# chenruduan/OAReactDiff

Measured on AMD Instinct MI355X. Metric: denoising_steps_per_sec, higher is better.
Workload: dtype f32; 1 GPU; EGNNDynamics.forward (LEFTNet H=196 R=96 L=6), B=64 reactions/GPU x 3 objects x 23 atoms, complete graph per reaction (N=4416, E=300288), T=1000 sampler step shape; batch_per_gpu=64, atoms_per_object=23, parallelism=replica x1 (no collective), launch=eager

## Files before the change

### oareactdiff_amd/_capi.py

```python
from __future__ import annotations

import ctypes as C
import os

from .build import LIB

OARD_MAX_OBJECTS = 8
ABI_VERSION = 2040
OARD_OK, OARD_EINVAL, OARD_ENOTCOMPLETE, OARD_EHIP, OARD_ENOMEM = 0, -1, -2, -3, -4
ERRORS = {OARD_EINVAL: "invalid argument / unsupported configuration", OARD_ENOTCOMPLETE: "topology is not complete-per-sample",
          OARD_EHIP: "HIP runtime error", OARD_ENOMEM: "workspace too small"}

PREC_GCL_BF16X3, PREC_EQUI_BF16X3, PREC_TRAIN_BF16X3 = 1, 2, 4
TAP_S, TAP_VEC, TAP_EDGE, TAP_POS_FRAME, TAP_DPOS, TAP_HOUT, TAP_LABELS, TAP_NE1 = 1, 2, 3, 4, 5, 6, 7, 8

EXPORTS = ["oard_version", "oard_supported", "oard_param_count", "oard_packed_bytes", "oard_pack_weights",
           "oard_topology_create", "oard_topology_destroy", "oard_topology_num_nodes", "oard_topology_num_edges",
           "oard_topology_num_inner_edges", "oard_topology_num_samples", "oard_topology_check_edge_index",
           "oard_workspace_bytes", "oard_forward", "oard_active_inner_edges", "oard_debug_lin3u_table", "oard_sampler_step", "oard_sampler_step_dev", "oard_tap", "oard_debug_stop_after", "oard_debug_option", "oard_timing_enable", "oard_timing_reset",
           "oard_timing_get",
           "oard_topology_create_parts", "oard_topology_export", "oard_tape_bytes", "oard_tape_entry", "oard_forward_train",
           "oard_packed_bwd_bytes", "oard_pack_weights_bwd", "oard_gcl_backward_dx", "oard_edge_node_sums",
           "oard_equi_backward_dx", "oard_scalarize_backward", "oard_equi_msg_backward", "oard_lin3u_forward", "oard_lin3u_backward", "oard_wgrad_scratch_bytes", "oard_wgrad",
           "oard_train_scratch_bytes", "oard_train_scratch_poison", "oard_train_scratch_entry", "oard_train_tail_backward",
           "oard_train_layer_backward", "oard_train_init_backward", "oard_train_stage_backward",
           "oard_loss_prepare", "oard_loss_terms", "oard_adamw_step", "oard_adamw_step_dev", "oard_nan_replace",
           "oard_graph_create", "oard_graph_destroy", "oard_graph_num_nodes", "oard_graph_num_edges", "oard_graph_object_rows",
           "oard_graph_is_complete", "oard_graph_workspace_bytes", "oard_graph_forward", "oard_library_stream"]
STAGE_RECOMPUTE, STAGE_UPDATE, STAGE_MESSAGE, STAGE_GCL_NODE, STAGE_NODE_PRE, STAGE_GCL_EDGE, STAGE_EQUI_EDGE = range(7)
SCRATCH_XH, SCRATCH_XQ, SCRATCH_CR, SCRATCH_DCD, SCRATCH_DCR = range(1, 6)

TOPO_NODE_REF, TOPO_NODE_OBJ, TOPO_NODE_ROW, TOPO_NODE_SAMPLE, TOPO_NODE_TIDX, TOPO_SAMPLE_PTR, TOPO_GROUP_PTR, \
    TOPO_INNER_SRC, TOPO_INNER_TGT, TOPO_ROW_SRC, TOPO_ROW_TGT = range(1, 12)
TAPE_HIN, TAPE_GEO, TAPE_RBF, TAPE_PP0, TAPE_X1 = 1, 2, 3, 4, 5
TAPE_S_IN, TAPE_VEC_IN, TAPE_EW, TAPE_AGG, TAPE_S_MID, TAPE_Z1, TAPE_Z2, TAPE_ATT, TAPE_Z3, TAPE_ZD1, TAPE_CD, TAPE_S_A, TAPE_VEC_A = range(16, 29)


class OardConfig(C.Structure):
    _fields_ = [
        ("hidden", C.c_int32), ("num_radial", C.c_int32), ("num_layers", C.c_int32), ("in_hidden", C.c_int32),
        ("n_obj", C.c_int32), ("node_nf", C.c_int32 * OARD_MAX_OBJECTS), ("enc_alias", C.c_int32 * OARD_MAX_OBJECTS),
        ("condition_nf", C.c_int32), ("condition_time", C.c_int32), ("pos_dim", C.c_int32), ("cutoff", C.c_float),
        ("reflect_equiv", C.c_int32), ("precision", C.c_int32),
    ]


class OardError(RuntimeError):
    pass


def check(rc: int, what: str) -> None:
    if rc != OARD_OK:
        raise OardError(f"{what} failed: {ERRORS.get(rc, rc)}")


def ptr_array(tensors, n=None):
    if tensors is None:
        return None
    ptrs = [None if t is None else t.data_ptr() for t in tensors]
    return (C.c_void_p * (len(ptrs) if n is None else n))(*ptrs)


_lib = None


def lib() -> C.CDLL:
    global _lib
    if _lib is not None:
        return _lib
    if not os.path.exists(LIB):
        raise OardError(f"{LIB} not found: build it with `python -m oareactdiff_amd.build` "
                        "(there is no CPU fallback for the HIP backend)")
    L = C.CDLL(LIB)
    vp, i32, i64, sz = C.c_void_p, C.c_int32, C.c_int64, C.c_size_t
    cfgp = C.POINTER(OardConfig)
    L.oard_version.restype = C.c_int
    got = L.oard_version()
    if got != ABI_VERSION:
        raise OardError(f"{LIB} has ABI version {got}, this package expects {ABI_VERSION}: rebuild it "
                        "(`python -m oareactdiff_amd.build --force`, or the script that made the OARD_LIB build)")
    L.oard_supported.argtypes = [cfgp]; L.oard_supported.restype = C.c_int
    L.oard_param_count.argtypes = [cfgp]; L.oard_param_count.restype = sz
    L.oard_packed_bytes.argtypes = [cfgp]; L.oard_packed_bytes.restype = sz
    L.oard_pack_weights.argtypes = [cfgp, C.POINTER(vp), sz, vp, sz, vp]; L.oard_pack_weights.restype = C.c_int
    L.oard_topology_create.argtypes = [cfgp, C.POINTER(i64), C.POINTER(i64), i64, C.POINTER(vp)]
    L.oard_topology_create.restype = C.c_int
    L.oard_topology_destroy.argtypes = [vp]; L.oard_topology_destroy.restype = None
    for f in ("oard_topology_num_nodes", "oard_topology_num_edges", "oard_topology_num_inner_edges",
              "oard_topology_num_samples"):
        getattr(L, f).argtypes = [vp]; getattr(L, f).restype = i64
    L.oard_topology_check_edge_index.argtypes = [vp, vp, i64, vp, vp]; L.oard_topology_check_edge_index.restype = C.c_int
    L.oard_workspace_bytes.argtypes = [cfgp, vp]; L.oard_workspace_bytes.restype = sz
    L.oard_forward.argtypes = [cfgp, vp, vp, C.POINTER(vp), vp, C.c_int, vp, C.POINTER(vp), vp, sz, vp, vp]
    L.oard_forward.restype = C.c_int
    L.oard_debug_lin3u_table.argtypes = [cfgp, vp, C.c_int, vp, vp]; L.oard_debug_lin3u_table.restype = C.c_int
    L.oard_active_inner_edges.argtypes = [cfgp, vp, vp, sz, C.POINTER(i64), vp]; L.oard_active_inner_edges.restype = C.c_int
    L.oard_sampler_step.argtypes = [cfgp, vp, C.c_int, C.POINTER(vp), C.POINTER(vp), C.POINTER(vp), C.POINTER(vp),
                                    C.c_float, C.c_float, C.c_float, C.c_int, C.POINTER(vp), vp]
    L.oard_sampler_step.restype = C.c_int
    L.oard_sampler_step_dev.argtypes = [cfgp, vp, C.c_int, C.POINTER(vp), C.POINTER(vp), C.POINTER(vp), C.POINTER(vp), vp, C.c_int,
                                        C.POINTER(vp), vp]
    L.oard_sampler_step_dev.restype = C.c_int
    L.oard_tap.argtypes = [cfgp, vp, vp, C.c_int, C.c_int, vp, vp]; L.oard_tap.restype = C.c_int
    ci = C.c_int
    L.oard_topology_create_parts.argtypes = [cfgp, C.POINTER(i64), C.POINTER(i64), i64, ci, C.POINTER(vp)]
    L.oard_topology_create_parts.restype = ci
    L.oard_topology_export.argtypes = [vp, ci, vp, i64, vp]; L.oard_topology_export.restype = ci
    L.oard_tape_bytes.argtypes = [cfgp, vp]; L.oard_tape_bytes.restype = sz
    L.oard_tape_entry.argtypes = [cfgp, vp, ci, ci, C.POINTER(sz), C.POINTER(i64), C.POINTER(i64)]; L.oard_tape_entry.restype = ci
    L.oard_forward_train.argtypes = [cfgp, vp, vp, C.POINTER(vp), vp, ci, vp, C.POINTER(vp), vp, sz, vp, sz, vp, vp]
    L.oard_forward_train.restype = ci
    L.oard_packed_bwd_bytes.argtypes = [cfgp]; L.oard_packed_bwd_bytes.restype = sz
    L.oard_pack_weights_bwd.argtypes = [cfgp, C.POINTER(vp), sz, vp, sz, vp]; L.oard_pack_weights_bwd.restype = ci
    L.oard_gcl_backward_dx.argtypes = [cfgp, vp, vp, ci, vp, vp, vp, vp, vp, vp, vp, vp, vp]; L.oard_gcl_backward_dx.restype = ci
    L.oard_edge_node_sums.argtypes = [cfgp, vp, vp, vp, vp, vp]; L.oard_edge_node_sums.restype = ci
    L.oard_equi_backward_dx.argtypes = [cfgp, vp, vp, ci, vp, vp, vp, vp, vp]; L.oard_equi_backward_dx.restype = ci
    L.oard_scalarize_backward.argtypes = [cfgp, vp, vp, vp, vp, ci, vp, vp, vp, vp]; L.oard_scalarize_backward.restype = ci
    L.oard_equi_msg_backward.argtypes = [cfgp, vp, vp, ci, vp, vp, vp, vp, vp, vp, vp, vp, vp]; L.oard_equi_msg_backward.restype = ci
    L.oard_lin3u_forward.argtypes = [cfgp, vp, ci, vp, i64, vp, vp]; L.oard_lin3u_forward.restype = ci
    L.oard_lin3u_backward.argtypes = [cfgp, vp, ci, vp, vp, i64, vp, vp, vp, vp, vp, vp, vp]; L.oard_lin3u_backward.restype = ci
    L.oard_wgrad_scratch_bytes.argtypes = [ci, ci, i64]; L.oard_wgrad_scratch_bytes.restype = sz
    L.oard_wgrad.argtypes = [vp, ci, ci, ci, ci, ci, vp, ci, ci, ci, ci, ci, ci, i64, vp, vp, vp, sz, vp]; L.oard_wgrad.restype = ci
    pvp = C.POINTER(vp)
    L.oard_train_scratch_bytes.argtypes = [cfgp, vp]; L.oard_train_scratch_bytes.restype = sz
    L.oard_train_scratch_poison.argtypes = [cfgp, vp, vp, sz, vp]; L.oard_train_scratch_poison.restype = ci
    L.oard_train_scratch_entry.argtypes = [cfgp, vp, ci, C.POINTER(sz), C.POINTER(i64), C.POINTER(i64)]; L.oard_train_scratch_entry.restype = ci
    L.oard_train_tail_backward.argtypes = [cfgp, vp, vp, vp, vp, pvp, vp, vp, pvp, pvp, vp, sz, vp]; L.oard_train_tail_backward.restype = ci
    L.oard_train_layer_backward.argtypes = [cfgp, vp, vp, vp, vp, ci, vp, vp, vp, pvp, pvp, vp, sz, vp]; L.oard_train_layer_backward.restype = ci
    L.oard_train_init_backward.argtypes = [cfgp, vp, vp, vp, vp, pvp, vp, vp, pvp, pvp, vp, sz, vp]; L.oard_train_init_backward.restype = ci
    L.oard_train_stage_backward.argtypes = [cfgp, vp, vp, vp, vp, ci, ci, vp, vp, vp, vp, vp, vp, pvp, pvp, vp, sz, vp]
    L.oard_train_stage_backward.restype = ci
    L.oard_nan_replace.argtypes = [cfgp, vp, vp, pvp, pvp, vp]; L.oard_nan_replace.restype = ci
    pf, cf = C.POINTER(C.c_float), C.c_float
    L.oard_loss_prepare.argtypes = [cfgp, vp, pvp, pvp, pvp, pvp, vp, vp, ci, pf, pf, ci, ci, pvp, pvp, vp]; L.oard_loss_prepare.restype = ci
    L.oard_loss_terms.argtypes = [cfgp, vp, pvp, pvp, pvp, pvp, pvp, vp, vp, ci, pf, pf, pf, ci, ci, vp, vp, pvp, vp]; L.oard_loss_terms.restype = ci
    cd = C.c_double
    L.oard_adamw_step.argtypes = [vp, vp, vp, vp, vp, i64, cd, cd, cd, cd, cd, i64, ci, cd, vp]; L.oard_adamw_step.restype = ci
    L.oard_adamw_step_dev.argtypes = [vp, vp, vp, vp, vp, i64, cd, cd, cd, cd, cd, ci, ci, vp, ci, vp, vp, vp, vp]; L.oard_adamw_step_dev.restype = ci
    L.oard_library_stream.argtypes = [ci, pvp]; L.oard_library_stream.restype = ci
    L.oard_graph_create.argtypes = [cfgp, vp, vp, i64, vp, i64, pvp]; L.oard_graph_create.restype = ci
    L.oard_graph_destroy.argtypes = [vp]; L.oard_graph_destroy.restype = None
    L.oard_graph_num_nodes.argtypes = [vp]; L.oard_graph_num_nodes.restype = i64
    L.oard_graph_num_edges.argtypes = [vp]; L.oard_graph_num_edges.restype = i64
    L.oard_graph_object_rows.argtypes = [vp, ci]; L.oard_graph_object_rows.restype = i64
    L.oard_graph_is_complete.argtypes = [vp]; L.oard_graph_is_complete.restype = ci
    L.oard_graph_workspace_bytes.argtypes = [cfgp, vp]; L.oard_graph_workspace_bytes.restype = sz
    L.oard_graph_forward.argtypes = [cfgp, vp, pvp, sz, pvp, vp, ci, vp, pvp, vp, sz, vp, vp]; L.oard_graph_forward.restype = ci
    L.oard_debug_stop_after.argtypes = [C.c_int]; L.oard_debug_stop_after.restype = C.c_int
    L.oard_debug_option.argtypes = [C.c_char_p, C.c_int]; L.oard_debug_option.restype = C.c_int
    L.oard_timing_enable.argtypes = [C.c_int]; L.oard_timing_enable.restype = C.c_int
    L.oard_timing_reset.argtypes = []; L.oard_timing_reset.restype = C.c_int
    L.oard_timing_get.argtypes = [C.c_char_p, C.POINTER(C.c_double), C.POINTER(i64)]; L.oard_timing_get.restype = C.c_int
    for env, opt in (("OARD_GCL_VARIANT", b"gcl_variant"), ("OARD_EQUI_VARIANT", b"equi_variant"),
                     ("OARD_NODE_VARIANT", b"node_variant"), ("OARD_GCL_SKIP", b"gcl_skip"), ("OARD_EQUI_SKIP", b"equi_skip"), ("OARD_EQUI_L0_SKIP", b"equi_l0_skip"), ("OARD_GCL_MSUM", b"gcl_msum"), ("OARD_GCL_PERSIST", b"gcl_persist"), ("OARD_GCL_GRID", b"gcl_grid"), ("OARD_PARTS", b"parts"), ("OARD_SEQUENTIAL", b"sequential"), ("OARD_POISON", b"poison"), ("OARD_AUTO_SMALL", b"auto_small"), ("OARD_AUTO_TINY", b"auto_tiny"), ("OARD_NPB", b"npb"),
                     ("OARD_WGRAD_WGS", b"wgrad_wgs"), ("OARD_WGRAD_LDS", b"wgrad_lds"), ("OARD_WGRAD_T16", b"wgrad_t16"), ("OARD_WGRAD_QUEUE", b"wgrad_queue"), ("OARD_GATE_FOLD", b"gate_fold"), ("OARD_WGRAD_SHAPES", b"wgrad_shapes"), ("OARD_TRAIN_DUAL", b"train_dual"), ("OARD_SMALL_SPLIT", b"small_split"),
                     ("OARD_SKIP_FAMILIES", b"skip_families")):
        if os.environ.get(env) not in (None, ""):
            check(L.oard_debug_option(opt, int(os.environ[env])), f"oard_debug_option({opt.decode()})")
    _lib = L
    return L


def timing_get(family: str):
    ms, n = C.c_double(0.0), C.c_int64(0)
    check(lib().oard_timing_get(family.encode(), C.byref(ms), C.byref(n)), "oard_timing_get")
    return ms.value, n.value
```

### oareactdiff_amd/csrc/oard_edge_v1.h

```cpp
#pragma once
#include "oard_kernels.h"

typedef __attribute__((address_space(3))) void* lds_ptr_t;
typedef const __attribute__((address_space(1))) void* gbl_ptr_t;
typedef int i4 __attribute__((ext_vector_type(4)));

OARD_DEV void glds16(const float* gsrc_lane, float* lds_chunk);
OARD_DEV void glds16u(const float* chunk_uniform, unsigned lane_byte_off, float* lds_chunk) {
    glds16(reinterpret_cast<const float*>(reinterpret_cast<const char*>(chunk_uniform) + lane_byte_off), lds_chunk);
}
OARD_DEV void glds16(const float* gsrc_lane, float* lds_chunk) {
#ifndef OARD_ABL_NODMA_INSTR
    __builtin_amdgcn_global_load_lds((gbl_ptr_t)gsrc_lane, (lds_ptr_t)lds_chunk, 16, 0, 0);
#else
    asm volatile("" :: "v"(gsrc_lane), "s"(lds_chunk));
#endif
}

OARD_DEV void phase_barrier() {
    asm volatile("s_waitcnt vmcnt(0)" ::: "memory");
#ifndef OARD_ABL_NOBARRIER
    __syncthreads();
#endif
}

#ifdef OARD_PHASE_PROBE
OARD_DEVVAR __device__ unsigned long long g_phase_probe[8];
#define PROBE_DECL long long pr_t0_ = clock64(), pr_wait_ = 0, pr_bar_ = 0, pr_n_ = 0;
#define PHASE_BARRIER() do { const long long a_ = clock64(); asm volatile("s_waitcnt vmcnt(0)" ::: "memory"); const long long b_ = clock64(); \
        __syncthreads(); const long long c_ = clock64(); pr_wait_ += b_ - a_; pr_bar_ += c_ - b_; ++pr_n_; } while (0)
#define PROBE_END(pf) do { if ((threadIdx.x & 63) == 0) { atomicAdd(&g_phase_probe[0], 1ull); atomicAdd(&g_phase_probe[1], (unsigned long long)(clock64() - pr_t0_)); \
        atomicAdd(&g_phase_probe[2], (unsigned long long)pr_wait_); atomicAdd(&g_phase_probe[3], (unsigned long long)pr_bar_); \
        atomicAdd(&g_phase_probe[4], (unsigned long long)(pf).dma_cyc); atomicAdd(&g_phase_probe[5], (unsigned long long)(pf).dma_n); \
        atomicAdd(&g_phase_probe[6], (unsigned long long)pr_n_); if ((threadIdx.x >> 6) < (blockDim.x >> 7)) atomicAdd(&g_phase_probe[7], (unsigned long long)pr_bar_); } } while (0)
#else
#define PROBE_DECL
#define PHASE_BARRIER() phase_barrier()
#define PROBE_END(pf) do {} while (0)
#endif

#ifdef OARD_TIMELINE
#define TL_MAX 1024
OARD_DEVVAR __device__ long long g_timeline[16][TL_MAX];
#define TL_DECL const bool tl_on_ = DO_S1 && DO_S3 && blockIdx.x == gridDim.x / 2 && (threadIdx.x & 63) == 0; int tl_n_ = 0;
#define TL(code) do { if (tl_on_ && tl_n_ < TL_MAX) g_timeline[threadIdx.x >> 6][tl_n_++] = (clock64() << 3) | (code); } while (0)
#define TL_END() do { if (tl_on_ && tl_n_ < TL_MAX) g_timeline[threadIdx.x >> 6][tl_n_] = 0; } while (0)
#else
#define TL_DECL
#define TL(code) do {} while (0)
#define TL_END() do {} while (0)
#endif

OARD_DEV void mma_pair(f4 a0, f4 b0, f4& c0, f4 a1, f4 b1, f4& c1) {
    c0 = __builtin_amdgcn_mfma_f32_16x16x4f32(a0.x, b0.x, c0, 0, 0, 0);
    c1 = __builtin_amdgcn_mfma_f32_16x16x4f32(a1.x, b1.x, c1, 0, 0, 0);
    c0 = __builtin_amdgcn_mfma_f32_16x16x4f32(a0.y, b0.y, c0, 0, 0, 0);
    c1 = __builtin_amdgcn_mfma_f32_16x16x4f32(a1.y, b1.y, c1, 0, 0, 0);
    c0 = __builtin_amdgcn_mfma_f32_16x16x4f32(a0.z, b0.z, c0, 0, 0, 0);
    c1 = __builtin_amdgcn_mfma_f32_16x16x4f32(a1.z, b1.z, c1, 0, 0, 0);
    c0 = __builtin_amdgcn_mfma_f32_16x16x4f32(a0.w, b0.w, c0, 0, 0, 0);
    c1 = __builtin_amdgcn_mfma_f32_16x16x4f32(a1.w, b1.w, c1, 0, 0, 0);
}

OARD_DEV void mma4_chunk(f4 a, f4 b, f4& c0, f4& c1) {
    c0 = __builtin_amdgcn_mfma_f32_4x4x1f32(a.x, b.x, c0, 0, 0, 0);
    c1 = __builtin_amdgcn_mfma_f32_4x4x1f32(a.y, b.y, c1, 0, 0, 0);
    c0 = __builtin_amdgcn_mfma_f32_4x4x1f32(a.z, b.z, c0, 0, 0, 0);
    c1 = __builtin_amdgcn_mfma_f32_4x4x1f32(a.w, b.w, c1, 0, 0, 0);
}
OARD_DEV f4 reduce_g(f4 v) {
    f4 r;
#pragma unroll
    for (int c = 0; c < 4; ++c) {
        float x = v[c];
        x += __shfl_xor(x, 16, 64);
        x += __shfl_xor(x, 32, 64);
        r[c] = x;
    }
    return r;
}

OARD_DEV f4 lds_a(const float* sl, int j) { return *reinterpret_cast<const f4*>(sl + j * 256); }

struct NoHook { OARD_DEV void operator()() const {} };
template <int KB, bool TAIL, class Hook>
OARD_DEV f4 chain_tile(const float* sl, int j0, const f4 (&in)[KB], f4 init, float tail, Hook hook) {
    static_assert(!TAIL || (KB & 1), "compact tail needs an odd number of chunks");
    f4 c0 = init, c1 = f4zero();
    f4 a0 = lds_a(sl, j0), a1 = KB > 1 ? lds_a(sl, j0 + 1) : f4zero();
#pragma unroll
    for (int b = 0; b + 1 < KB; b += 2) {
        f4 n0 = a0, n1 = a1;
        if (b + 2 < KB) n0 = lds_a(sl, j0 + b + 2);
        if (b + 3 < KB) n1 = lds_a(sl, j0 + b + 3);
        mma_pair(a0, in[b], c0, a1, in[b + 1], c1);
        hook();
        a0 = n0; a1 = n1;
    }
    if (KB & 1) {
        if (TAIL) c0 = __builtin_amdgcn_mfma_f32_16x16x4f32(a0.x, tail, c0, 0, 0, 0);
        else c0 = mma_chunk(a0, in[KB - 1], c0);
    }
    return c0 + c1;
}
template <int KB, class Hook = NoHook>
OARD_DEV f4 chain_tile(const float* sl, int j0, const f4 (&in)[KB], f4 init, Hook hook = Hook()) {
    return chain_tile<KB, false, Hook>(sl, j0, in, init, 0.f, hook);
}
template <int KB, class Hook = NoHook>
OARD_DEV f4 chain_tile4(const float* sl, int j0, const f4 (&in)[KB], f4 init, Hook hook = Hook()) {
    f4 c0 = init, c1 = f4zero();
    f4 a0 = lds_a(sl, j0), a1 = KB > 1 ? lds_a(sl, j0 + 1) : f4zero();
#pragma unroll
    for (int b = 0; b + 1 < KB; b += 2) {
        f4 n0 = a0, n1 = a1;
        if (b + 2 < KB) n0 = lds_a(sl, j0 + b + 2);
        if (b + 3 < KB) n1 = lds_a(sl, j0 + b + 3);
        mma4_chunk(a0, in[b], c0, c1);
        mma4_chunk(a1, in[b + 1], c0, c1);
        hook();
        a0 = n0; a1 = n1;
        __builtin_amdgcn_sched_barrier(0);
    }
    if (KB & 1) mma4_chunk(a0, in[KB - 1], c0, c1);
    return c0 + c1;
}
template <int MT, bool ROWS4, class Hook>
OARD_DEV void chain_kouter(const float* sl, int j0, f4 x, f4 (&acc)[MT], f4& extra, Hook hook) {
    static_assert(!ROWS4 || (MT & 1), "the 4-row tile must be the odd one");
    f4 a0 = lds_a(sl, j0), a1 = MT > 1 ? lds_a(sl, j0 + 1) : f4zero();
#pragma unroll
    for (int t = 0; t + 1 < MT; t += 2) {
        f4 n0 = a0, n1 = a1;
        if (t + 2 < MT) n0 = lds_a(sl, j0 + t + 2);
        if (t + 3 < MT) n1 = lds_a(sl, j0 + t + 3);
        mma_pair(a0, x, acc[t], a1, x, acc[t + 1]);
        hook();
        a0 = n0; a1 = n1;
    }
    if (MT & 1) {
        if (ROWS4) mma4_chunk(a0, x, acc[MT - 1], extra);
        else acc[MT - 1] = mma_chunk(a0, x, acc[MT - 1]);
    }
}
template <int MT, class Hook = NoHook>
OARD_DEV void chain_kouter(const float* sl, int j0, f4 x, f4 (&acc)[MT], Hook hook = Hook()) {
    f4 unused = f4zero();
    chain_kouter<MT, false, Hook>(sl, j0, x, acc, unused, hook);
}

#ifndef OARD_PF_HALF
#define OARD_PF_HALF 1
#endif
#ifndef OARD_PF_PERIOD
#define OARD_PF_PERIOD 1
#endif
template <int WAVES, int SLAB, int HALF = OARD_PF_HALF, int PERIOD = OARD_PF_PERIOD, int RING = 2>
struct SlabPrefetch {
    static constexpr int IW = (HALF && WAVES >= 8) ? WAVES / 2 : WAVES;
    static constexpr int KMAX = (SLAB + IW - 1) / IW;
    const float* src;
    float* dst;
    unsigned lane_off;
    int n, k, next, wave;
#ifdef OARD_PHASE_PROBE
    long long dma_cyc = 0, dma_n = 0;
#endif
    OARD_DEV void begin(const float* stream, float* smem, int phase, int first_chunk, int n_chunks) {
        src = stream + (size_t)first_chunk * 256;
        dst = smem + (size_t)(RING == 2 ? (phase & 1) : (phase % RING)) * SLAB * 256;
        n = wave < IW ? n_chunks : 0; k = 0; next = 1 + ((IW == WAVES && wave >= WAVES / 2) ? 1 : 0);
    }
    OARD_DEV void one() {
#ifdef OARD_ABL_NOHOOK
        k = KMAX;
        return;
#endif
        const int j = wave + k * IW;
#ifdef OARD_PHASE_PROBE
        if (j < n) { const long long a_ = clock64(); glds16u(src + (size_t)j * 256, lane_off, dst + j * 256); dma_cyc += clock64() - a_; ++dma_n; }
#else
        if (j < n) glds16u(src + (size_t)j * 256, lane_off, dst + j * 256);
#endif
        ++k;
    }
#ifdef OARD_ABL_BURST
    OARD_DEV void tick() {}
#else
#ifdef OARD_ABL_NOHOOK
    OARD_DEV void tick() {}
#else
    OARD_DEV void tick() { if (--next == 0) { one(); next = PERIOD; } }
#endif
#endif
    OARD_DEV void flush() { while (k < KMAX) one(); }
};

#ifdef OARD_ABL_NOEDGELOAD
OARD_DEV f4 ld_edge(const float* p) { return (f4){0.25f, -0.5f, 0.125f, 1.0f}; }
#else
OARD_DEV f4 ld_edge(const float* p) { return ld_f4(p); }
#endif

template <int CTRL>
OARD_DEV float dpp_row(float x) {
    return __builtin_bit_cast(float, __builtin_amdgcn_update_dpp(0, __builtin_bit_cast(int, x), CTRL, 0xf, 0xf, true));
}
template <int CTRL>
OARD_DEV int dpp_row_i(int x) { return __builtin_amdgcn_update_dpp(0, x, CTRL, 0xf, 0xf, true); }
struct SegLanes {
    float k1, k2, k4, k8;
    bool head;
};
OARD_DEV SegLanes seg_lanes(int key) {
    SegLanes s;
    s.k1 = dpp_row_i<0x101>(key) == key ? 1.f : 0.f; s.k2 = dpp_row_i<0x102>(key) == key ? 1.f : 0.f;
    s.k4 = dpp_row_i<0x104>(key) == key ? 1.f : 0.f; s.k8 = dpp_row_i<0x108>(key) == key ? 1.f : 0.f;
    const int prev = dpp_row_i<0x111>(key);
    s.head = key > 0 && prev != key;
    return s;
}
OARD_DEV f4 seg_sum(f4 v, const SegLanes& s) {
#define OARD_SEG_STEP(k, d) \
        "v_fmac_f32_dpp %0, %0, " k " row_shl:" d " row_mask:0xf bank_mask:0xf bound_ctrl:1\n\t" \
        "v_fmac_f32_dpp %1, %1, " k " row_shl:" d " row_mask:0xf bank_mask:0xf bound_ctrl:1\n\t" \
        "v_fmac_f32_dpp %2, %2, " k " row_shl:" d " row_mask:0xf bank_mask:0xf bound_ctrl:1\n\t" \
        "v_fmac_f32_dpp %3, %3, " k " row_shl:" d " row_mask:0xf bank_mask:0xf bound_ctrl:1\n\t"
    asm volatile("s_nop 4\n\t" OARD_SEG_STEP("%4", "1") OARD_SEG_STEP("%5", "2") OARD_SEG_STEP("%6", "4") OARD_SEG_STEP("%7", "8")
                 : "+v"(v.x), "+v"(v.y), "+v"(v.z), "+v"(v.w) : "v"(s.k1), "v"(s.k2), "v"(s.k4), "v"(s.k8));
#undef OARD_SEG_STEP
    return v;
}
template <class D>
OARD_DEV void st_msum(float* __restrict__ msum, long long col, int key, const f4 (&m)[D::HT], int lane) {
    const SegLanes s = seg_lanes(key);
#pragma unroll
    for (int t = 0; t < D::HT; ++t) {
        const f4 v = seg_sum(m[t], s);
        if (s.head) st_blk(msum, (size_t)col, D::HP, t, lane, v);
    }
}

template <class D, int GP>
struct GclStream {
    static constexpr int HT = D::HT, WB = D::WB, G1 = HT, G2 = HT + 1, NG2 = HT + 1;
    static constexpr bool TAIL1 = (D::H % 16) >= 1 && (D::H % 16) <= 4 && HT >= 3 && (HT & 1);
    static constexpr bool ROWS4 = TAIL1;
    static constexpr int SLAB = GP * G2;
    static constexpr int NP1 = (WB + GP - 1) / GP, NP2 = (NG2 + GP - 1) / GP, NP3 = NP1, NPH = NP1 + NP2 + NP3;
    static constexpr int C1 = WB * G1, C2 = NG2 * G2, C3 = WB * G2, CHUNKS = C1 + C2 + C3;
    static constexpr size_t LDS_BYTES = (size_t)2 * SLAB * 1024;
};

struct GclTape {
    float* z1;
    float* z2;
    float* att;
    float* z3;
};

OARD_DEV float tail_compact(f4 v, int lane) {
    const int e = lane & 15, g = lane >> 4;
    const float t0 = __shfl(v.x, e, 64), t1 = __shfl(v.y, e, 64), t2 = __shfl(v.z, e, 64), t3 = __shfl(v.w, e, 64);
// ... 201 lines not shown
            pf_begin(p + DIST);
            if (p3 + 1 < S::NP3) {
#pragma unroll
                for (int gg = 0; gg < GP; ++gg) {
                    const int t = (p3 + 1) * GP + gg;
                    if (t < WB)
                        onext[gg] = DO_S1 ? ld_edge(erow + 16 * t) : ld_f4(c0 + 16 * t + 4 * g);
                }
            }
        };
        auto hook = [&]() { if (RING == 3 && bar_left > 0 && --bar_left == 0) { PHASE_BARRIER(); post(); } pf.tick(); };
        if (RING == 2) { PHASE_BARRIER(); post(); } else bar_left = BAR_AT;
#pragma unroll
        for (int gg = 0; gg < GP; ++gg) {
            const int t = p3 * GP + gg;
            if (t < WB) {
                TL(2);
                const f4 z = chain_tile<HT, TAIL1>(SL(p), gg * G2 + 1, m, A(p, gg * G2), m_tail, hook);
                TL(3);
                if (TRAIN) pendz[gg] = z;
                pend[gg] = o[gg] + silu4(z);
            }
        }
        TL(4);
        if (RING == 3 && bar_left > 0) { bar_left = 0; PHASE_BARRIER(); post(); }
        if (MSUM && p3 == 0) st_msum<D>(mbuf, c, key, m, lane);
        pf.flush();
        ++p;
    };
    {
        int p3 = 0;
        for (; p3 + 1 < S::NP3; p3 += 2) { s3_phase(p3, on, om); s3_phase(p3 + 1, om, on); }
        if (p3 < S::NP3) s3_phase(p3, on, om);
    }
#pragma unroll
    for (int gg = 0; gg < GP; ++gg) {
        const int t = (S::NP3 - 1) * GP + gg;
        if (t < WB) {
            st_f4(orow + 16 * t, pend[gg]);
            if (TRAIN) st_f4(tape.z3 + e * D::WP + 4 * g + 16 * t, pendz[gg]);
        }
    }
    PROBE_END(pf);
    TL_END();
}

template <class D>
struct EquiStream {
    static constexpr int WB = D::WB, D1T = D::D1T, RB = D::RB, HT = D::HT;
    static constexpr int G1 = D1T, G2 = 1 + D1T + RB, NG2 = 3 * HT;
    static constexpr bool ROWS4 = (D::H % 16) >= 1 && (D::H % 16) <= 4;
    static constexpr int SLAB = G2 > G1 ? G2 : G1;
    static constexpr int NPH = WB + NG2;
    static constexpr int C1 = WB * G1, CHUNKS = C1 + NG2 * G2;
    static constexpr size_t LDS_BYTES = (size_t)2 * SLAB * 1024;
};

template <class D, int WAVES, bool TRAIN>
__global__ __launch_bounds__(WAVES * 64) void k_equi_edge_v1(TopoDev tp, const float* __restrict__ stream,
                                                             const float* __restrict__ dp0b,
                                                             const float* __restrict__ ew, const float* __restrict__ rbuf,
                                                             float* __restrict__ qbuf, float* __restrict__ zd1,
                                                             float* __restrict__ cdbuf, ActList al, int skip_mid) {
    extern __shared__ __attribute__((aligned(16))) float smem[];
    using S = EquiStream<D>;
    constexpr int WB = D::WB, D1T = D::D1T, RB = D::RB, HT = D::HT, G1 = S::G1, G2 = S::G2;
    const int lane = threadIdx.x & 63, g = lane >> 4;
    const int wave = __builtin_amdgcn_readfirstlane(threadIdx.x >> 6);

    SlabPrefetch<WAVES, S::SLAB, 0, 3> pf;
    pf.wave = wave;
    pf.lane_off = (unsigned)lane * 16u;
    const bool skip = !TRAIN && skip_mid != 0;
    auto pf_begin = [&](int ph) {
        pf.begin(stream, smem, ph, ph * G1, G1);
    };
    auto pf_begin_t2 = [&](int ph, int slot) {
        pf.begin(stream, smem, ph, S::C1 + slot * G2, slot < S::NG2 ? G2 : 0);
    };
    auto next_slot = [&](int i) -> int { return i + ((skip && i % 3 == 0) ? 2 : 1); };
    auto hook = [&]() { pf.tick(); };
    auto A = [&](int p, int j) -> f4 {
        return *reinterpret_cast<const f4*>(smem + ((size_t)(p & 1) * S::SLAB + j) * 256 + lane * 4);
    };
    auto SL = [&](int p) -> const float* { return smem + (size_t)(p & 1) * S::SLAB * 256 + lane * 4; };

    const long long n_cols = al.n != nullptr ? (long long)*al.n : tp.A;
    if ((long long)blockIdx.x * WAVES * 16 >= n_cols) return;
    const long long c = ((long long)blockIdx.x * WAVES + wave) * 16 + (lane & 15);
    const bool live = c < n_cols;
    const size_t a = (size_t)(live ? (al.rows != nullptr ? (long long)al.rows[c] : c) : tp.A);
    const float* erow = ew + (live ? a : (size_t)tp.E) * D::WP + 4 * g;
    f4 d1[D1T];
#pragma unroll
    for (int t = 0; t < D1T; ++t) d1[t] = ld_vec(dp0b, t, lane);
    f4 rb[RB];
#pragma unroll
    for (int b = 0; b < RB; ++b) rb[b] = ld_blk(rbuf, a, D::RP, b, lane);
    f4 xn = ld_f4(erow);
    pf_begin(0);
    pf.flush();

    int p = 0;
    for (int b = 0; b < WB; ++b, ++p) {
        phase_barrier();
        const f4 x = xn;
        if (b + 1 < WB) pf_begin(p + 1); else pf_begin_t2(p + 1, 0);
        if (b + 1 < WB) xn = ld_f4(erow + 16 * (b + 1));
        chain_kouter<D1T>(SL(p), 0, x, d1, hook);
        pf.flush();
    }
    if (TRAIN) {
#pragma unroll
        for (int t = 0; t < D1T; ++t) st_blk(zd1, a, D::D1P, t, lane, d1[t]);
    }
#pragma unroll
    for (int t = 0; t < D1T; ++t) d1[t] = silu4(d1[t]);

    float* qrow = qbuf + a * (size_t)(3 * D::HP) + 4 * g;
    float* cdrow = TRAIN ? cdbuf + a * (size_t)(3 * D::HP) + 4 * g : nullptr;
    f4 pend = f4zero(), pendc = f4zero();
    int pend_off = 0;
    auto t2_phase = [&](int i, auto rows4) {
        phase_barrier();
        if (i > 0) {
            st_f4(qrow + pend_off, pend);
            if (TRAIN) st_f4(cdrow + pend_off, pendc);
        }
        pf_begin_t2(p + 1, next_slot(i));
        const int tt = i / 3, th = i - 3 * tt;
        f4 cd, cr;
        if (decltype(rows4)::value) {
            cd = reduce_g(chain_tile4<D1T>(SL(p), 1, d1, A(p, 0), hook));
            cr = reduce_g(chain_tile4<RB>(SL(p), 1 + D1T, rb, f4zero(), hook));
            if (g != 0) { cd = f4zero(); cr = f4zero(); }
        } else {
            cd = chain_tile<D1T>(SL(p), 1, d1, A(p, 0), hook);
            cr = chain_tile<RB>(SL(p), 1 + D1T, rb, f4zero(), hook);
        }
        pf.flush();
        pend = cd * cr;
        if (TRAIN) pendc = cd;
        pend_off = th * D::HP + 16 * tt;
        ++p;
    };
    constexpr int N_FULL = S::ROWS4 ? S::NG2 - 3 : S::NG2;
    for (int i = 0; i < N_FULL; i = next_slot(i)) t2_phase(i, std::false_type{});
    for (int i = N_FULL; i < S::NG2; i = next_slot(i)) t2_phase(i, std::true_type{});
    st_f4(qrow + pend_off, pend);
    if (TRAIN) st_f4(cdrow + pend_off, pendc);
}

template <class D>
__global__ __launch_bounds__(256) void k_equi_agg_v1(TopoDev tp, const float* __restrict__ wb, LayerOff lo,
                                                     const float* __restrict__ qbuf, const float* __restrict__ xq,
                                                     const float* __restrict__ geo, const float* __restrict__ x1,
                                                     float* __restrict__ s, const float* __restrict__ vec_in,
                                                     float* __restrict__ vec_out, float* __restrict__ v2buf,
                                                     float* __restrict__ scal, float* __restrict__ vdot) {
    bool live; const ColId id = col_id(tp.N, live);
    if (!live) return;
    const int n = id.col, a0 = tp.act_ptr[n], cnt = tp.act_ptr[n + 1] - a0;
    const int mx = wave_max(cnt);
    const float inv_sqrt2 = 0.70710678118654752f, inv_sqrt3 = 0.57735026918962576f,
                inv_sqrt_h = 1.0f / sqrtf((float)D::H);
    f4 vx[3][D::HT], dx[D::HT];
#pragma unroll
    for (int t = 0; t < D::HT; ++t) { dx[t] = f4zero(); vx[0][t] = f4zero(); vx[1][t] = f4zero(); vx[2][t] = f4zero(); }
    for (int k = 0; k < mx; ++k)
        if (k < cnt) {
            const size_t a = (size_t)a0 + k;
            const int m = tp.act_src[a];
            const float* g = geo + a * GEO_STRIDE;
            const float ux = g[2], uy = g[3], uz = g[4];
            const float xc = lo.xcross ? 1.0f : 0.0f, cx = xc * g[5], cy = xc * g[6], cz = xc * g[7];
#pragma unroll
            for (int t = 0; t < D::HT; ++t) {
                const f4 q0 = ld_blk(qbuf, a, 3 * D::HP, t, id.lane);
                const f4 q1 = ld_blk(qbuf, a, 3 * D::HP, D::HT + t, id.lane);
                const f4 q2 = ld_blk(qbuf, a, 3 * D::HP, 2 * D::HT + t, id.lane);
                const f4 xs0 = ld_blk(xq, m, 3 * D::HP, t, id.lane) + ld_blk(xq, n, 3 * D::HP, t, id.lane);
                const f4 xs1 = ld_blk(xq, m, 3 * D::HP, D::HT + t, id.lane) + ld_blk(xq, n, 3 * D::HP, D::HT + t, id.lane);
                const f4 xs2 = ld_blk(xq, m, 3 * D::HP, 2 * D::HT + t, id.lane) + ld_blk(xq, n, 3 * D::HP, 2 * D::HT + t, id.lane);
                const f4 xm = xs0 * q0;
                dx[t] += xm;
                const f4 a2 = xs1 * q1 * inv_sqrt3, a3 = xs2 * q2;
                vx[0][t] += (ld_blk(vec_in, (size_t)m * 3 + 0, D::HP, t, id.lane) * a2 + a3 * ux + xm * cx) * inv_sqrt_h;
                vx[1][t] += (ld_blk(vec_in, (size_t)m * 3 + 1, D::HP, t, id.lane) * a2 + a3 * uy + xm * cy) * inv_sqrt_h;
                vx[2][t] += (ld_blk(vec_in, (size_t)m * 3 + 2, D::HP, t, id.lane) * a2 + a3 * uz + xm * cz) * inv_sqrt_h;
            }
        }
#pragma unroll
    for (int t = 0; t < D::HT; ++t) {
        const f4 sn = (ld_blk(s, n, D::HP, t, id.lane) + dx[t]) * inv_sqrt2;
        if (id.valid) st_blk(s, n, D::HP, t, id.lane, sn);
#pragma unroll
        for (int x = 0; x < 3; ++x) {
            vx[x][t] += ld_blk(vec_in, (size_t)n * 3 + x, D::HP, t, id.lane);
            if (id.valid) st_blk(vec_out, (size_t)n * 3 + x, D::HP, t, id.lane, vx[x][t]);
        }
    }
    const float fx = x1[n * 3], fy = x1[n * 3 + 1], fz = x1[n * 3 + 2];
    const float* l3 = wb + lo.l3u;
    for (int t = 0; t < D::HT; ++t) {
        f4 v1[3] = {f4zero(), f4zero(), f4zero()}, v2[3] = {f4zero(), f4zero(), f4zero()};
        const float* w1 = wb + lo.vp + ((size_t)t * D::HT * 64 + id.lane) * 4;
        const float* w2 = wb + lo.vp + ((size_t)(D::HT + t) * D::HT * 64 + id.lane) * 4;
#pragma unroll
        for (int b = 0; b < D::HT; ++b) {
            const f4 c1 = ld_f4(w1 + (size_t)b * 256), c2 = ld_f4(w2 + (size_t)b * 256);
#pragma unroll
            for (int x = 0; x < 3; ++x) {
                v1[x] = mma_chunk(c1, vx[x][b], v1[x]);
                v2[x] = mma_chunk(c2, vx[x][b], v2[x]);
            }
        }
        const f4 sc = v1[0] * fx + v1[1] * fy + v1[2] * fz;
        const f4 vd = (v1[0] * v2[0] + v1[1] * v2[1] + v1[2] * v2[2]) * inv_sqrt_h;
        f4 sca;
        const int f0 = 16 * t + 4 * id.g;
        sca.x = f0 + 0 < D::H ? lin3u(l3, sc.x) : 0.f;
        sca.y = f0 + 1 < D::H ? lin3u(l3, sc.y) : 0.f;
        sca.z = f0 + 2 < D::H ? lin3u(l3, sc.z) : 0.f;
        sca.w = f0 + 3 < D::H ? lin3u(l3, sc.w) : 0.f;
        if (id.valid) {
            st_blk(scal, n, D::HP, t, id.lane, sca);
            st_blk(vdot, n, D::HP, t, id.lane, vd);
            st_blk(v2buf, (size_t)n * 3 + 0, D::HP, t, id.lane, v2[0]);
            st_blk(v2buf, (size_t)n * 3 + 1, D::HP, t, id.lane, v2[1]);
            st_blk(v2buf, (size_t)n * 3 + 2, D::HP, t, id.lane, v2[2]);
        }
    }
}
```

### oareactdiff_amd/csrc/oard_hip.hip

```cpp
#include <algorithm>
#include <cmath>
#include <cstdio>
#include <cstring>
#include <map>
#include <string>
#include <vector>
#include <mutex>
#include <chrono>
#include <utility>

#include "oard_kernels.h"
#include "oard_edge_v1.h"
#include "oard_edge_p.h"
#include "oard_wgrad_t16.h"
#include "oard_edge_b3.h"
#ifdef OARD_EXPERIMENTS
#include "oard_edge_fp.h"
#endif
#include "oard_node_v1.h"
#include "oard_edge_small.h"
#include "oard_edge_bwd.h"
#include "oard_node_bwd.h"
#include "oard_rows.h"
#include "oard_inst.h"

#define OARD_VERSION 2040
#ifdef OARD_EXPERIMENTS
static constexpr bool kV0 = true;
#else
static constexpr bool kV0 = false;
#endif

#define HIP_TRY(x) do { hipError_t e_ = (x); if (e_ != hipSuccess) { \
    fprintf(stderr, "liboard_hip: %s failed: %s (%s:%d)\n", #x, hipGetErrorString(e_), __FILE__, __LINE__); \
    return OARD_EHIP; } } while (0)

namespace {
enum Family { F_GCL_EDGE = 0, F_EQUI_EDGE, F_NODE, F_INIT, F_OTHER, F_GCL_BWD, F_EQUI_BWD, F_WGRAD, F_COUNT };
const char* kFamilyNames[F_COUNT] = {"gcl_edge", "equi_edge", "node", "init", "other", "gcl_edge_bwd", "equi_edge_bwd", "wgrad"};
struct TimingRec { hipEvent_t a, b; int fam; };
struct Timing {
    bool on = false;
    std::vector<TimingRec> recs;
    std::vector<hipEvent_t> pool;
    double total_ms[F_COUNT] = {0};
    long long launches[F_COUNT] = {0};
    hipEvent_t get() {
        if (!pool.empty()) { hipEvent_t e = pool.back(); pool.pop_back(); return e; }
        hipEvent_t e; (void)hipEventCreate(&e); return e;
    }
    void flush() {
        for (auto& r : recs) {
            (void)hipEventSynchronize(r.b);
            float ms = 0.f;
            (void)hipEventElapsedTime(&ms, r.a, r.b);
            total_ms[r.fam] += ms; launches[r.fam] += 1;
            pool.push_back(r.a); pool.push_back(r.b);
        }
        recs.clear();
    }
} g_timing;
int g_stop_after = 0;
int g_gcl_variant = 2;
int g_equi_variant = 2;
int g_sequential = 0;
int g_auto_tiny = 8;
int g_auto_small = 4;
int g_npb = 0;
int g_poison = 0;
int g_equi_l0_skip = 1;
int g_gcl_msum = 1;
int g_gcl_msum_taken = 0;
int g_equi_l0_taken = 0;
int g_parts = 0;
int g_small_split = 128;
int g_wgrad_shapes = 3;
int g_wgrad_t16 = 256;
int g_wgrad_lds = 256;
int g_wgrad_wgs = 512;
int g_gcl_persist = 1;
int g_gcl_grid = 0;
int g_equi_skip = 1;
int g_gcl_skip = 1;
int g_node_variant = 1;
int g_skip_families = 0;

struct ScopedLaunch {
    hipStream_t st; hipEvent_t a; int fam; bool on;
    ScopedLaunch(int f, hipStream_t s) : st(s), fam(f), on(g_timing.on) {
        if (on) { a = g_timing.get(); (void)hipEventRecord(a, st); }
    }
    ~ScopedLaunch() {
        if (on) { hipEvent_t b = g_timing.get(); (void)hipEventRecord(b, st); g_timing.recs.push_back({a, b, fam}); }
    }
};
#define LAUNCH(fam, kern, grid, block, stream, ...) do { ScopedLaunch sl_(fam, stream); if (!((g_skip_families >> (fam)) & 1)) \
    hipLaunchKernelGGL(kern, dim3((unsigned)(grid)), dim3(block), 0, stream, __VA_ARGS__); } while (0)
#define LAUNCH2(fam, kern, gx, gy, block, stream, ...) do { ScopedLaunch sl_(fam, stream); if (!((g_skip_families >> (fam)) & 1)) \
    hipLaunchKernelGGL(kern, dim3((unsigned)(gx), (unsigned)(gy)), dim3(block), 0, stream, __VA_ARGS__); } while (0)

#ifndef OARD_DIMS_LIST
#define OARD_DIMS_LIST X(196, 96) X(32, 8) X(32, 32)
#endif

inline size_t align_up(size_t x, size_t a) { return (x + a - 1) / a * a; }
inline long long cdiv(long long a, long long b) { return (a + b - 1) / b; }

bool config_ok(const oard_config* c) {
    if (!c) return false;
    bool dims = false;
#define X(h, r) dims = dims || (c->hidden == (h) && c->num_radial == (r));
    OARD_DIMS_LIST
#undef X
    if (!dims) return false;
    if (c->num_layers < 1 || c->num_layers > OARD_MAX_LAYERS) return false;
    if (c->in_hidden < 1 || c->in_hidden > 16) return false;
    if (c->n_obj < 1 || c->n_obj > OARD_MAX_OBJECTS) return false;
    if (c->pos_dim != 3 || (c->reflect_equiv != 0 && c->reflect_equiv != 1)) return false;
    if (c->precision & ~(OARD_PREC_GCL_BF16X3 | OARD_PREC_EQUI_BF16X3 | OARD_PREC_TRAIN_BF16X3)) return false;
    const int emb = c->in_hidden - (c->condition_time ? 1 : 0) - (c->condition_nf > 0 ? c->condition_nf : 0);
    if (emb < 1) return false;
    for (int k = 0; k < c->n_obj; ++k) {
        const int d = c->node_nf[k] - 3;
        if (d < 1 || d > 16) return false;
        const int a = c->enc_alias[k];
        if (a < 0 || a >= c->n_obj || c->node_nf[a] != c->node_nf[k]) return false;
    }
    return true;
}
int embed_dim(const oard_config* c) {
    return c->in_hidden - (c->condition_time ? 1 : 0) - (c->condition_nf > 0 ? c->condition_nf : 0);
}

PackOff make_layout(const oard_config* c) {
    const RDims d(c->hidden, c->num_radial);
    PackOff po;
    memset(&po, 0, sizeof(po));
    size_t cur = 0;
    auto take = [&](size_t n) { size_t o = cur; cur = align_up(cur + n, 64); return o; };
    auto mat = [&](int MT, int KB) { return take((size_t)MT * KB * 256); };
    const int emb = embed_dim(c);
    po.emb = mat(d.HT, 1); po.emb_b = take(d.HP);
    po.nbemb = mat(d.HT, 1); po.nbemb_b = take(d.HP);
    po.s2v = mat(d.HT, d.HT); po.s2v_b = take(d.HP);
    po.rl0 = mat(d.HT, d.RB); po.rl0_b = take(d.HP);
    po.rl2 = mat(d.HT, d.HT); po.rl2_b = take(d.HP);
    po.lin3 = take((size_t)d.H4 * 5 + 1);
    po.pe0 = take((size_t)d.H2 * 3);
    po.pe1 = mat(d.HT, d.PB);
    po.embout = mat(1, d.HT); po.embout_b = take(16);
    po.v1p = mat(d.HT, d.HT); po.v2p = take(d.HP);
    po.un0 = mat(d.HT, 2 * d.HT); po.un0_b = take(d.HP);
    po.un2 = mat(1, d.HT); po.un2_b = take(16);
    po.c0row = take(d.WP);
    po.u0 = take(d.HP);
    po.rbf_means = take(d.RP); po.rbf_betas = take(d.RP);
    for (int k = 0; k < c->n_obj; ++k) {
        const int dd = c->node_nf[k] - 3;
        po.enc[k] = take((size_t)2 * dd * dd + 2 * dd + (size_t)emb * 2 * dd + emb);
        po.dec[k] = take((size_t)2 * dd * emb + 2 * dd + (size_t)dd * 2 * dd + dd);
    }
    for (int l = 0; l < c->num_layers; ++l) {
        LayerOff& lo = po.layer[l];
        lo.ln_g_w = take(d.HP); lo.ln_g_b = take(d.HP);
        lo.W1a = mat(d.HT, d.HT); lo.b1 = take(d.HP);
        lo.W1b = mat(d.HT, d.HT);
        lo.W1c = mat(d.HT, d.WB);
        lo.W2 = mat(d.HT, d.HT); lo.b2 = take(d.HP);
        lo.watt = take(d.HP); lo.batt = take(1);
        lo.W3 = mat(d.WB, d.HT); lo.b3 = take(d.WP);
        lo.nm0 = mat(d.HT, 2 * d.HT); lo.nm0b = take(d.HP);
        lo.nm1 = mat(d.HT, d.HT); lo.nm1b = take(d.HP);
        lo.ln_q_w = take(d.HP); lo.ln_q_b = take(d.HP);
        lo.xp0 = mat(d.HT, d.HT);
        lo.xp2 = mat(3 * d.HT, d.HT);
        lo.dp0 = mat(d.D1T, d.WB); lo.dp0b = take(d.D1P);
        lo.dp2 = mat(3 * d.HT, d.D1T); lo.dp2b = take(3 * d.HP);
        lo.rbfp = mat(3 * d.HT, d.RB);
        lo.vp = mat(2 * d.HT, d.HT);
        lo.xv0 = mat(d.HT, 2 * d.HT);
        lo.xv2 = mat(3 * d.HT, d.HT);
        lo.l3u = take(593);
        lo.l3t = take(L3T_FLOATS);
        lo.gcl_stream = take((size_t)(d.WB * d.HT + (d.HT + 1) * (d.HT + 1) + d.WB * (d.HT + 1)) * 256);
        lo.equi_stream = take((size_t)(d.WB * d.D1T + 3 * d.HT * (1 + d.D1T + d.RB)) * 256);
        {
            const int nbh = (d.HT + 1) / 2, nbw = (d.WB + 1) / 2;
            lo.gcl_b3 = take((size_t)(nbw * 3 * d.HT + (d.HT + 1) * (1 + 3 * nbh) + d.WB * (1 + 3 * nbh)) * 256);
            lo.equi_b3 = take((size_t)(nbw * 3 * d.D1T + ((d.RB + 1) / 2 + (d.D1T + 1) / 2) * 9 * d.HT) * 256);
        }
    }
    po.total = cur;
    po.signed_scal = c->reflect_equiv ? 0 : 1;
    for (int l = 0; l < c->num_layers; ++l) po.layer[l].xcross = c->reflect_equiv ? 0 : 1;
    return po;
}

struct ParamIdx {
    int emb_w, emb_b, embout_w, embout_b, means, betas, nbemb_w, nbemb_b, s2v_w, s2v_b, rl0_w, rl0_b, rl2_w, rl2_b,
        lin30_w, lin30_b, lin32_w, lin32_b, pe0_w, pe1_w;
    int gcl0, msg0, upd0, out0, enc0, dec0, count;
    explicit ParamIdx(const oard_config* c) {
        int i = 0;
        emb_w = i++; emb_b = i++; embout_w = i++; embout_b = i++; means = i++; betas = i++;
        nbemb_w = i++; nbemb_b = i++; s2v_w = i++; s2v_b = i++; rl0_w = i++; rl0_b = i++; rl2_w = i++; rl2_b = i++;
        lin30_w = i++; lin30_b = i++; lin32_w = i++; lin32_b = i++; pe0_w = i++; pe1_w = i++;
        i += 2;
        gcl0 = i; i += 14 * c->num_layers;
        msg0 = i; i += 9 * c->num_layers;
        upd0 = i; i += 9 * c->num_layers;
        i += 2;
        out0 = i; i += 6;
        enc0 = i; i += 4 * c->n_obj;
        dec0 = i; i += 4 * c->n_obj;
        count = i;
    }
};

struct Packer {
    const float* const* p; float* blob; hipStream_t st;
    std::vector<GenJob> jobs;
    long long blocks = 0;
    void push(GenJob j, size_t work) {
        j.block0 = blocks;
        blocks += cdiv((long long)std::max<size_t>(work, 1), 256);
        jobs.push_back(j);
    }
    void matrix(int src, int src_ld, int col_off, int msl, int msp, int ms, int ksl, int ksp, int ks, int MT, int KB,
                size_t dst, size_t tstride = 0, size_t bstride = 256, int perm_ht = 0, int transpose = 0, int tail_compact = 0,
                int rows4 = 0) {
        if (tstride == 0) tstride = (size_t)KB * 256;
        GenJob j;
        memset(&j, 0, sizeof(j));
        j.type = 0;
        j.m = PackJob{p[src], src_ld, col_off, msl, msp, ms, ksl, ksp, ks, MT, KB, dst, tstride, bstride, perm_ht, transpose, rows4, tail_compact};
        push(j, (size_t)MT * KB * 256);
    }
    void nat(int src, int src_ld, int col_off, int M, int K, int MT, int KB, size_t dst) {
        matrix(src, src_ld, col_off, M, MT * 16, 1, K, KB * 16, 1, MT, KB, dst);
    }
    void vec(int src, int sect_len, int sect_pad, int sects, int n_dst, size_t dst) {
        GenJob j;
        memset(&j, 0, sizeof(j));
        j.type = 1; j.src = src >= 0 ? p[src] : nullptr; j.dst = dst; j.sect_len = sect_len; j.sect_pad = sect_pad; j.sects = sects; j.n = n_dst;
        push(j, (size_t)n_dst);
    }
    void bias_chunks(int src, int sect_len, int sect_pad, int sects, int n_tiles, size_t dst, size_t tstride,
                     int perm_ht = 0) {
        GenJob j;
        memset(&j, 0, sizeof(j));
        j.type = 2; j.src = p[src]; j.dst = dst; j.sect_len = sect_len; j.sect_pad = sect_pad; j.sects = sects; j.n = n_tiles * 256;
        j.tstride = tstride; j.perm_ht = perm_ht;
        push(j, (size_t)n_tiles * 256);
    }
    void raw(int src, int n, size_t dst) {
        GenJob j;
        memset(&j, 0, sizeof(j));
        j.type = 3; j.src = p[src]; j.dst = dst; j.n = n;
        push(j, (size_t)n);
    }
    int flush() {
        if (jobs.empty()) return OARD_OK;
        struct Cached { std::vector<GenJob> host; GenJob* dev = nullptr; size_t cap = 0; };
        static std::mutex mu;
        static std::map<std::pair<const void*, int>, Cached> cache;
        int devid = 0;
        (void)hipGetDevice(&devid);
        const GenJob* table = nullptr;
        {
            std::lock_guard<std::mutex> lk(mu);
            Cached& c = cache[{(const void*)blob, devid}];
            const bool same = c.host.size() == jobs.size() && memcmp(c.host.data(), jobs.data(), jobs.size() * sizeof(GenJob)) == 0;
            if (!same) {
                HIP_TRY(hipStreamSynchronize(st));
                if (c.cap < jobs.size()) {
                    if (c.dev) (void)hipFree(c.dev);
                    HIP_TRY(hipMalloc((void**)&c.dev, jobs.size() * sizeof(GenJob)));
                    c.cap = jobs.size();
                }
                HIP_TRY(hipMemcpy(c.dev, jobs.data(), jobs.size() * sizeof(GenJob), hipMemcpyHostToDevice));
                c.host = jobs;
            }
            table = c.dev;
        }
        hipLaunchKernelGGL(k_pack_all, dim3((unsigned)blocks), dim3(256), 0, st, table, (int)jobs.size(), blob);
        jobs.clear();
        blocks = 0;
        return OARD_OK;
    }
};
#define OARD_SMALL_MAX_EDGES (512 * 16 * 16)
struct SmallScratch { float* a; float* b; };
static thread_local SmallScratch t_small = {nullptr, nullptr};
static WsOff make_ws(const oard_config* c, const TopoDev& td) {
    const RDims d(c->hidden, c->num_radial);
    const size_t N = td.N, E = td.E + 1, A = td.A + 1;
    WsOff w;
    size_t cur = 0;
    auto take = [&](size_t bytes) { size_t o = cur; cur = align_up(cur + bytes, 256); return o; };
    w.pos = take(N * 3 * 4); w.pf64 = take(N * 3 * 8); w.pf32 = take(N * 3 * 4); w.x1 = take(N * 3 * 4);
    w.pp0 = take(N * 4); w.labels = take(N * 4); w.hin = take(N * 16 * 4);
    w.zemb = take(N * d.HP * 4); w.nb = take(N * d.HP * 4); w.s = take(N * d.HP * 4); w.s1 = take(N * d.HP * 4);
    w.ne1 = take(N * 3 * d.HP * 4); w.xh = take(N * d.HP * 4); w.P = take(N * d.HP * 4); w.Q = take(N * d.HP * 4);
    w.xq = take(N * 3 * d.HP * 4); w.vec = take(N * 3 * d.HP * 4); w.vec2 = take(N * 3 * d.HP * 4); w.v2buf = take(N * 3 * d.HP * 4);
    w.sc0 = take(N * d.HP * 4); w.vdot = take(N * d.HP * 4);
    w.geo = take(A * GEO_STRIDE * 4); w.d64 = take(A * 8); w.rbuf = take(A * d.RP * 4);
    w.ew = take(E * d.WP * 4); w.mbuf = take(std::max(E, (size_t)(td.CI + td.CX) + 1) * d.HP * 4);
    w.xmsg = take(A * d.HP * 4); w.vmsg = take(A * 3 * d.HP * 4);
    w.dpos = take(N * 3 * 4); w.hout = take(N * 16 * 4);
    w.al_rows = take(A * 4); w.al_src = take(A * 4); w.al_pre = take(A * 4); w.al_cnt = take((size_t)cdiv((long long)td.A, 256) * 4 + 4); w.al_n = take(4);
    w.d1s = take((size_t)cdiv((long long)td.A, 128) * 8 * d.D1T * 1024);
    w.small_a = w.small_b = 0;
    if (E <= (size_t)OARD_SMALL_MAX_EDGES) {
        w.small_a = take(A * d.D1P * 4);
    }
    w.total = cur;
    return w;
}



template <class K>
int set_lds(K kernel, size_t bytes) {
    HIP_TRY(hipFuncSetAttribute((const void*)kernel, hipFuncAttributeMaxDynamicSharedMemorySize, (int)bytes));
    return OARD_OK;
}

#define LAUNCH_LDS(fam, kern, grid, block, lds, stream, ...) do { \
    static bool attr_done_[64] = {}; \
    int dev_ = 0; (void)hipGetDevice(&dev_); dev_ &= 63; \
    if (!attr_done_[dev_]) { int rc_ = set_lds(kern, lds); if (rc_ != OARD_OK) return rc_; attr_done_[dev_] = true; } \
    ScopedLaunch sl_(fam, stream); if (!((g_skip_families >> (fam)) & 1)) \
    hipLaunchKernelGGL(kern, dim3((unsigned)(grid)), dim3(block), lds, stream, __VA_ARGS__); } while (0)

#define GCL_CASE(id, WV_, GP_) case id: { \
        LAUNCH_LDS(F_GCL_EDGE, (k_gcl_edge_v1<D, WV_, GP_, S1, S3, false>), cdiv(r1 - r0, 16 * WV_), WV_ * 64, \
                   (GclStream<D, GP_>::LDS_BYTES), st, tp, stream, P, Q, u0, c0, r0, r1, ew_in, ew_out, mbuf, GclTape{}); return OARD_OK; }
#define GCL_RING3(TRAIN_, tape_) do { \
        LAUNCH_LDS(F_GCL_EDGE, (k_gcl_edge_v1<D, 8, 2, S1, S3, TRAIN_, false, 2, 3>), cdiv(r1 - r0, 16 * 8), 8 * 64, \
                   (GclStream<D, 2>::LDS_BYTES / 2 * 3), st, tp, stream, P, Q, u0, c0, r0, r1, ew_in, ew_out, mbuf, tape_); return OARD_OK; } while (0)
static int device_cus() {
    static int cus[64] = {};
    int d = 0;
    (void)hipGetDevice(&d);
    d &= 63;
    if (!cus[d]) {
        int n = 0;
        if (hipDeviceGetAttribute(&n, hipDeviceAttributeMultiprocessorCount, d) != hipSuccess || n < 1) { (void)hipGetLastError(); n = 256; }
        cus[d] = n;
    }
    return cus[d];
}
static bool gcl_v1_throughput(int prec, int variant, int conc, long long cols) {
    if (variant == 2 && cdiv(cols, 16) * conc <= 1024LL * g_auto_small) variant = 3;
    if ((variant == 2 || variant == 3) && cdiv(cols, 16) * conc <= 512LL * g_auto_tiny) variant = 6;
    return variant == 2 && !(prec & OARD_PREC_GCL_BF16X3);
}
template <class D, bool S1, bool S3>
int launch_gcl_v1s(int prec, int variant, int conc, const TopoDev& tp, const float* wb, const LayerOff& lo, const float* stream, const float* P, const float* Q, const float* u0,
                   const float* c0, long long r0, long long r1, const float* ew_in, float* ew_out, float* mbuf, const GclTape* tape, hipStream_t st,
                   bool msum = false) {
    if (r1 <= r0) return OARD_OK;
    if (msum && (tape || !gcl_v1_throughput(prec, variant, conc, r1 - r0))) return OARD_EINVAL;
    if (tape && (prec & OARD_PREC_TRAIN_BF16X3)) {
        LAUNCH_LDS(F_GCL_EDGE, (k_gcl_edge_b3<D, S1, S3, true>), cdiv(r1 - r0, 16 * 8), 8 * 64, (GclB3Stream<D>::LDS_BYTES), st, tp,
                   wb + lo.gcl_b3, P, Q, u0, c0, r0, r1, ew_in, ew_out, mbuf, *tape);
        return OARD_OK;
    }
    if (tape) {
#ifdef OARD_EXPERIMENTS
        if (variant == 7) {
            LAUNCH_LDS(F_GCL_EDGE, (k_gcl_edge_v1<D, 8, 2, S1, S3, true>), cdiv(r1 - r0, 16 * 8), 8 * 64,
                       (GclStream<D, 2>::LDS_BYTES), st, tp, stream, P, Q, u0, c0, r0, r1, ew_in, ew_out, mbuf, *tape);
            return OARD_OK;
        }
#endif
        if (g_gcl_persist) {
            const long long nhalf = cdiv(cdiv(r1 - r0, 16), 4);
            const long long want = g_gcl_grid > 0 ? g_gcl_grid : (g_gcl_grid < 0 ? cdiv(nhalf, 2LL * -g_gcl_grid) : device_cus());
            LAUNCH_LDS(F_GCL_EDGE, (k_gcl_edge_p<D, S1, S3, true>), std::min(nhalf, want), 8 * 64, (GclStream<D, 2>::LDS_BYTES / 2 * 3), st,
                       tp, stream, P, Q, u0, c0, r0, r1, ew_in, ew_out, mbuf, *tape);
            return OARD_OK;
        }
        GCL_RING3(true, *tape);
    }
    if (variant == 2 && cdiv(r1 - r0, 16) * conc <= 1024LL * g_auto_small) variant = 3;
    if ((variant == 2 || variant == 3) && cdiv(r1 - r0, 16) * conc <= 512LL * g_auto_tiny) variant = 6;
    if (variant == 6) {
        LAUNCH_LDS(F_GCL_EDGE, (k_gcl_edge_small<D, 8, S1, S3>), cdiv(r1 - r0, 16), 512, (GclSmall<D>::LDS_BYTES), st,
                   tp, wb, lo, P, Q, u0, c0, r0, r1, ew_out, mbuf);
        return OARD_OK;
    }
    switch (variant) {
        case 2:
            if (prec & OARD_PREC_GCL_BF16X3) {
                LAUNCH_LDS(F_GCL_EDGE, (k_gcl_edge_b3<D, S1, S3>), cdiv(r1 - r0, 16 * 8), 8 * 64, (GclB3Stream<D>::LDS_BYTES), st, tp,
                           wb + lo.gcl_b3, P, Q, u0, c0, r0, r1, ew_in, ew_out, mbuf, GclTape{});
                return OARD_OK;
            }
            if (g_gcl_persist > 1 || (g_gcl_persist == 1 && conc == 1)) {
                const long long nhalf = cdiv(cdiv(r1 - r0, 16), 4);
                const long long want = g_gcl_grid > 0 ? g_gcl_grid : (g_gcl_grid < 0 ? cdiv(nhalf, 2LL * -g_gcl_grid) : (conc > 1 ? std::max(1, device_cus() / 2) : device_cus()));
                if (msum) {
                    LAUNCH_LDS(F_GCL_EDGE, (k_gcl_edge_p<D, S1, S3, false, true>), std::min(nhalf, want), 8 * 64, (GclStream<D, 2>::LDS_BYTES / 2 * 3), st,
                               tp, stream, P, Q, u0, c0, r0, r1, ew_in, ew_out, mbuf, GclTape{});
                    return OARD_OK;
                }
                LAUNCH_LDS(F_GCL_EDGE, (k_gcl_edge_p<D, S1, S3>), std::min(nhalf, want), 8 * 64, (GclStream<D, 2>::LDS_BYTES / 2 * 3), st,
                           tp, stream, P, Q, u0, c0, r0, r1, ew_in, ew_out, mbuf, GclTape{});
                return OARD_OK;
            }
            if (msum) {
                LAUNCH_LDS(F_GCL_EDGE, (k_gcl_edge_v1<D, 8, 2, S1, S3, false, true, 2, 3>), cdiv(r1 - r0, 16 * 8), 8 * 64,
                           (GclStream<D, 2>::LDS_BYTES / 2 * 3), st, tp, stream, P, Q, u0, c0, r0, r1, ew_in, ew_out, mbuf, GclTape{});
                return OARD_OK;
            }
            GCL_RING3(false, GclTape{});
        GCL_CASE(3, 4, 2)
#ifdef OARD_EXPERIMENTS
        GCL_CASE(7, 8, 2)
        case 4: {
            LAUNCH_LDS(F_GCL_EDGE, (k_gcl_edge_fp<D, 8, 2, S1, S3, false>), cdiv(r1 - r0, 16 * 8), 8 * 64,
                       (GclRing<D, 2, 4>::LDS_BYTES), st, tp, stream, P, Q, u0, c0, r0, r1, ew_in, ew_out, mbuf, GclTape{}); return OARD_OK; }
        case 5: {
            LAUNCH_LDS(F_GCL_EDGE, (k_gcl_edge_fp<D, 8, 2, S1, S3, false, 3>), cdiv(r1 - r0, 16 * 8), 8 * 64,
                       (GclRing<D, 2, 3>::LDS_BYTES), st, tp, stream, P, Q, u0, c0, r0, r1, ew_in, ew_out, mbuf, GclTape{}); return OARD_OK; }
        GCL_CASE(8, 8, 3)
        GCL_CASE(9, 8, 4)
        case 10: { LAUNCH_LDS(F_GCL_EDGE, (k_gcl_edge_v1<D, 12, 1, S1, S3, false, false, 3>), cdiv(r1 - r0, 16 * 12), 12 * 64,
                              (GclStream<D, 1>::LDS_BYTES), st, tp, stream, P, Q, u0, c0, r0, r1, ew_in, ew_out, mbuf, GclTape{}); return OARD_OK; }
        case 11: { LAUNCH_LDS(F_GCL_EDGE, (k_gcl_edge_v1<D, 12, 2, S1, S3, false, false, 3>), cdiv(r1 - r0, 16 * 12), 12 * 64,
                              (GclStream<D, 2>::LDS_BYTES), st, tp, stream, P, Q, u0, c0, r0, r1, ew_in, ew_out, mbuf, GclTape{}); return OARD_OK; }
        case 12: { LAUNCH_LDS(F_GCL_EDGE, (k_gcl_edge_v1<D, 4, 1, S1, S3, false, false, 3>), cdiv(r1 - r0, 16 * 4), 4 * 64,
                              (GclStream<D, 1>::LDS_BYTES), st, tp, stream, P, Q, u0, c0, r0, r1, ew_in, ew_out, mbuf, GclTape{}); return OARD_OK; }
#endif
        default: return OARD_EINVAL;
    }
}
template <class D>
int launch_gcl_v1(int prec, int variant, int conc, const TopoDev& tp, const float* wb, const LayerOff& lo, const float* stream, const float* P, const float* Q, const float* u0,
                  const float* c0, bool first, bool last, const float* ew_in, float* ew_out, float* mbuf, const GclTape* tape, hipStream_t st,
                  bool msum = false) {
    const long long A = tp.A, E = tp.E;
    int rc;
    const bool skip = g_gcl_skip || tape;
    if (msum) {
        const long long c_in = tp.CI, c_all = tp.CI + tp.CX;
        const bool s1 = !(skip && first), s3 = !(skip && last);
        if (s1 && s3) return launch_gcl_v1s<D, true, true>(prec, variant, conc, tp, wb, lo, stream, P, Q, u0, c0, 0, c_all, ew_in, ew_out, mbuf, tape, st, true);
        rc = launch_gcl_v1s<D, true, true>(prec, variant, conc, tp, wb, lo, stream, P, Q, u0, c0, 0, c_in, ew_in, ew_out, mbuf, tape, st, true);
        if (rc != OARD_OK) return rc;
        if (s1) return launch_gcl_v1s<D, true, false>(prec, variant, conc, tp, wb, lo, stream, P, Q, u0, c0, c_in, c_all, ew_in, ew_out, mbuf, tape, st, true);
        if (s3) return launch_gcl_v1s<D, false, true>(prec, variant, conc, tp, wb, lo, stream, P, Q, u0, c0, c_in, c_all, ew_in, ew_out, mbuf, tape, st, true);
        return launch_gcl_v1s<D, false, false>(prec, variant, conc, tp, wb, lo, stream, P, Q, u0, c0, c_in, c_all, ew_in, ew_out, mbuf, tape, st, true);
    }
    if (!skip || (!first && !last)) return launch_gcl_v1s<D, true, true>(prec, variant, conc, tp, wb, lo, stream, P, Q, u0, c0, 0, E, ew_in, ew_out, mbuf, tape, st);
    rc = launch_gcl_v1s<D, true, true>(prec, variant, conc, tp, wb, lo, stream, P, Q, u0, c0, 0, A, ew_in, ew_out, mbuf, tape, st);
    if (rc != OARD_OK) return rc;
    if (first && last) return launch_gcl_v1s<D, false, false>(prec, variant, conc, tp, wb, lo, stream, P, Q, u0, c0, A, E, ew_in, ew_out, mbuf, tape, st);
    if (first) return launch_gcl_v1s<D, false, true>(prec, variant, conc, tp, wb, lo, stream, P, Q, u0, c0, A, E, ew_in, ew_out, mbuf, tape, st);
    return launch_gcl_v1s<D, true, false>(prec, variant, conc, tp, wb, lo, stream, P, Q, u0, c0, A, E, ew_in, ew_out, mbuf, tape, st);
}
static int equi_v1_shape(int prec, int variant, int conc, long long A, const float* d1s) {
    if (variant == 2 && cdiv(A, 16) * conc <= 512LL * g_auto_small) variant = 1;
    if ((variant == 2 || variant == 1) && cdiv(A, 16) * conc <= 512LL * g_auto_tiny) variant = 4;
    if (variant == 2 && (prec & OARD_PREC_EQUI_BF16X3) && d1s) variant = 5;
    return variant;
}
#define EQUI_CASE(id, WV_, SKIP_) case id: { \
        LAUNCH_LDS(F_EQUI_EDGE, (k_equi_edge_v1<D, WV_, false>), cdiv(tp.A, 16 * WV_), WV_ * 64, (EquiStream<D>::LDS_BYTES), st, \
                   tp, stream, dp0b, ew, rbuf, qbuf, nullptr, nullptr, al, SKIP_); return OARD_OK; }
template <class D>
int launch_equi_v1(int prec, int variant, int conc, const TopoDev& tp, const float* wb, const LayerOff& lo, const float* stream, const float* dp0b, const float* ew,
                   const float* rbuf, float* qbuf, float* zd1, float* cd, hipStream_t st, float* d1s = nullptr, ActList al = ActList{}, bool skip_mid = false) {
    if (zd1 && (prec & OARD_PREC_TRAIN_BF16X3) && d1s) {
        LAUNCH_LDS(F_EQUI_EDGE, (k_equi_edge_b3<D, true>), cdiv(tp.A, 16 * 8), 8 * 64, (EquiB3Stream<D>::LDS_BYTES), st, tp, wb + lo.equi_b3,
                   dp0b, wb + lo.dp2b, ew, rbuf, qbuf, d1s, zd1, cd, ActList{});
        return OARD_OK;
    }
    if (zd1) {
        LAUNCH_LDS(F_EQUI_EDGE, (k_equi_edge_v1<D, 8, true>), cdiv(tp.A, 16 * 8), 8 * 64, (EquiStream<D>::LDS_BYTES), st,
                   tp, stream, dp0b, ew, rbuf, qbuf, zd1, cd, ActList{}, 0);
        return OARD_OK;
    }
    variant = equi_v1_shape(prec, variant, conc, tp.A, d1s);
    if (skip_mid && variant != 2) return OARD_EINVAL;
    if (variant == 4) {
        if (t_small.a && cdiv(tp.A, 16) * conc <= g_small_split) {
            const long long tiles = cdiv(tp.A, 16);
            LAUNCH_LDS(F_EQUI_EDGE, (k_equi_small_s1<D, 8>), tiles * cdiv(D::D1T, 8), 512, (size_t)D::WB * 1024, st,
                       tp, wb, lo, ew, t_small.a);
            LAUNCH_LDS(F_EQUI_EDGE, (k_equi_small_s2<D, 8>), tiles * cdiv(3 * D::HT, 8), 512, (size_t)(D::D1T + D::RB) * 1024, st,
                       tp, wb, lo, (const float*)t_small.a, rbuf, qbuf);
            return OARD_OK;
        }
        LAUNCH_LDS(F_EQUI_EDGE, (k_equi_edge_small<D, 8>), cdiv(tp.A, 16), 512, (EquiSmall<D>::LDS_BYTES), st,
                   tp, wb, lo, ew, rbuf, qbuf);
        return OARD_OK;
    }
    if (variant == 5) {
        LAUNCH_LDS(F_EQUI_EDGE, (k_equi_edge_b3<D>), cdiv(tp.A, 16 * 8), 8 * 64, (EquiB3Stream<D>::LDS_BYTES), st, tp, wb + lo.equi_b3,
                   dp0b, wb + lo.dp2b, ew, rbuf, qbuf, d1s, nullptr, nullptr, al);
        return OARD_OK;
    }
    switch (variant) {
        EQUI_CASE(1, 4, 0)
        EQUI_CASE(2, 8, skip_mid ? 1 : 0)
        default: return OARD_EINVAL;
    }
}

struct TapeOff {
    size_t hin, geo, rbuf, pp0, x1;
    size_t s_in[OARD_MAX_LAYERS + 1], vec_in[OARD_MAX_LAYERS + 1];
    size_t agg[OARD_MAX_LAYERS], s_mid[OARD_MAX_LAYERS];
    size_t s_a[OARD_MAX_LAYERS], vec_a[OARD_MAX_LAYERS];
    size_t ew[OARD_MAX_LAYERS + 1];
    size_t z1[OARD_MAX_LAYERS], z2[OARD_MAX_LAYERS], att[OARD_MAX_LAYERS], z3[OARD_MAX_LAYERS];
    size_t zd1[OARD_MAX_LAYERS], cd[OARD_MAX_LAYERS];
    size_t total;
};
static TapeOff make_tape(const oard_config* c, const TopoDev& td) {
    const RDims d(c->hidden, c->num_radial);
    const size_t N = td.N, E = td.E + 1, A = td.A + 1;
    TapeOff t;
    memset(&t, 0, sizeof(t));
    size_t cur = 0;
    auto take = [&](size_t bytes) { size_t o = cur; cur = align_up(cur + bytes, 256); return o; };
    t.hin = take(N * 16 * 4); t.geo = take(A * GEO_STRIDE * 4); t.rbuf = take(A * d.RP * 4); t.pp0 = take(N * 4); t.x1 = take(N * 3 * 4);
    for (int l = 0; l <= c->num_layers; ++l) {
        t.s_in[l] = take(N * d.HP * 4); t.vec_in[l] = take(N * 3 * d.HP * 4); t.ew[l] = take(E * d.WP * 4);
        if (l == c->num_layers) break;
        t.agg[l] = take(N * d.HP * 4); t.s_mid[l] = take(N * d.HP * 4);
        t.s_a[l] = take(N * d.HP * 4); t.vec_a[l] = take(N * 3 * d.HP * 4);
        t.z1[l] = take(E * d.HP * 4); t.z2[l] = take(E * d.HP * 4); t.att[l] = take(E * 4); t.z3[l] = take(E * d.WP * 4);
        t.zd1[l] = take(A * d.D1P * 4); t.cd[l] = take(A * 3 * d.HP * 4);
    }
    t.total = cur;
    return t;
}

template <class D>
static int forward_impl(const oard_config* c, const TopoPart* topo, const float* wb, const float* const* xh,
                        const float* t, int t_scalar, const float* cond, float* const* out, char* ws, char* tape,
                        int* status, hipStream_t st) {
    const TopoDev& tp = topo->d;
    const PackOff po = make_layout(c);
    const WsOff w = make_ws(c, tp);
    const bool train = tape != nullptr;
    const TapeOff to = train ? make_tape(c, tp) : TapeOff{};
    const int emb = embed_dim(c);
    float* pos = (float*)(ws + w.pos); double* pf64 = (double*)(ws + w.pf64); float* pf32 = (float*)(ws + w.pf32);
    auto slot = [&](size_t ws_off, size_t tape_off) -> float* { return train ? (float*)(tape + tape_off) : (float*)(ws + ws_off); };
    float* x1 = slot(w.x1, to.x1); float* pp0 = slot(w.pp0, to.pp0); int* labels = (int*)(ws + w.labels);
    float* hin = slot(w.hin, to.hin); float* zemb = (float*)(ws + w.zemb); float* nb = (float*)(ws + w.nb);
    float* s = (float*)(ws + w.s); float* s1 = (float*)(ws + w.s1); float* ne1 = (float*)(ws + w.ne1);
    float* xhb = (float*)(ws + w.xh); float* P = (float*)(ws + w.P); float* Q = (float*)(ws + w.Q);
    float* xq = (float*)(ws + w.xq); float* vec = slot(w.vec, to.vec_in[0]); float* v2buf = (float*)(ws + w.v2buf);
    float* scal = (float*)(ws + w.sc0); float* vdot = (float*)(ws + w.vdot);
    float* geo = slot(w.geo, to.geo); double* d64 = (double*)(ws + w.d64); float* rbuf = slot(w.rbuf, to.rbuf);
    float* mbuf = (float*)(ws + w.mbuf); float* xmsg = (float*)(ws + w.xmsg);
    float* vmsg = (float*)(ws + w.vmsg); float* dpos = (float*)(ws + w.dpos); float* hout = (float*)(ws + w.hout);
    t_small = (w.small_a && !train) ? SmallScratch{(float*)(ws + w.small_a), (float*)(ws + w.small_b)} : SmallScratch{nullptr, nullptr};
    auto ew_at = [&](int l) -> float* { return train ? (float*)(tape + to.ew[l]) : (float*)(ws + w.ew); };
    float* ew = ew_at(0);
    auto s_at = [&](int l) -> float* { return train ? (float*)(tape + to.s_in[l]) : s; };
    auto s_mid_at = [&](int l) -> float* { return train ? (float*)(tape + to.s_mid[l]) : s; };

    ObjPtrs op;
    memset(&op, 0, sizeof(op));
    for (int k = 0; k < c->n_obj; ++k) {
        op.xh[k] = xh[k]; op.out[k] = out[k]; op.node_nf[k] = c->node_nf[k]; op.enc[k] = po.enc[k]; op.dec[k] = po.dec[k];
    }
    const long long N = tp.N, E = tp.E, A = tp.A;
    const unsigned gN = (unsigned)cdiv(N, 64), gE = (unsigned)cdiv(E, 64), gA = (unsigned)cdiv(A, 64);
    const double cutoff = (double)c->cutoff;
    const int gcl_variant = train ? 2 : g_gcl_variant, equi_variant = train ? 2 : g_equi_variant;
    const int node_variant = train ? 1 : g_node_variant;
    const bool gcl_skip = train || g_gcl_skip;
    const int stop_after = train ? 0 : g_stop_after;
    const bool use_al = !train && g_equi_skip && A > 0 && equi_variant != 0 && node_variant == 1;
    int* al_cnt = (int*)(ws + w.al_cnt);
    const ActList al = use_al ? ActList{(const int*)(ws + w.al_rows), (const int*)(ws + w.al_src), (const int*)(ws + w.al_pre), (const int*)(ws + w.al_n)}
                              : ActList{nullptr, nullptr, nullptr, nullptr};
    if (!use_al) HIP_TRY(hipMemsetAsync(ws + w.al_n, 0xff, sizeof(int), st));
    LAUNCH(F_OTHER, k_prep, cdiv(N, 128), 128, st, tp, op, wb, pos, hin, t, t_scalar, cond,
           c->condition_nf > 0 ? c->condition_nf : 0, c->condition_time, emb);
    LAUNCH(F_INIT, k_geom, tp.n_groups, 64, st, tp, (const float*)pos, cutoff, pf64, pf32, x1, pp0, labels);
    if (!(gcl_skip && gcl_variant != 0) || stop_after == 1)
        LAUNCH(F_INIT, k_fill_edges, std::min<long long>(cdiv((E - A + 1) * (D::WP / 4), 256), 8192), 256, st,
               wb + po.c0row, ew + (size_t)A * D::WP, E - A + 1, D::WP);
    if (A > 0) {
        LAUNCH(F_INIT, k_edge_geo, cdiv(A, 256), 256, st, tp, (const float*)pos, (const double*)pf64, cutoff, geo, d64, use_al ? al_cnt : nullptr);
        if (use_al) LAUNCH(F_INIT, k_active_list, cdiv(A, 256), 256, st, tp, (const float*)geo, (const int*)al_cnt, (int*)al.rows, (int*)al.src, (int*)al.pre, (int*)al.n);
        LAUNCH(F_INIT, k_rbf, cdiv(A * D::RP, 256), 256, st, tp, (const double*)d64, (const float*)geo,
               wb + po.rbf_means, wb + po.rbf_betas, cutoff, rbuf, ew, D::R, D::RP, D::H, D::WP);
    }
    LAUNCH(F_INIT, (k_node_embed<D>), gN, 256, st, tp, wb, po, (const float*)hin, zemb, nb);
    if (A > 0) LAUNCH(F_INIT, (k_radial_lin<D>), gA, 256, st, tp, wb, po, (const float*)rbuf, (const float*)geo, ew);
    constexpr int NW = D::HT <= 16 ? D::HT : 8;
    const unsigned gNb = (unsigned)cdiv(N, tp.npb);
    if (node_variant >= 1) {
        LAUNCH(F_INIT, (k_neighbor_v1<D, NW>), gNb, NW * 64, st, tp, wb, po, (const float*)zemb, (const float*)nb, (const float*)ew, s_at(0), s1);
        LAUNCH(F_INIT, (k_s2v_agg_v1<D, NW>), gNb, NW * 64, st, tp, (const float*)s1, (const float*)ew, (const float*)geo, ne1);
    } else if constexpr (kV0) {
        LAUNCH(F_INIT, (k_neighbor<D>), gN, 256, st, tp, wb, po, (const float*)zemb, (const float*)nb, (const float*)ew, s_at(0), s1);
        LAUNCH(F_INIT, (k_s2v_agg<D>), gN, 256, st, tp, (const float*)s1, (const float*)ew, (const float*)geo, ne1);
    } else return OARD_EINVAL;
    if (A > 0) LAUNCH2(F_INIT, (k_scalarize<D>), gA, (gA * topo->conc <= 2048 ? D::HT : 1), 256, st, tp, wb, po, (const float*)ne1, (const float*)geo, ew);
    HIP_TRY(hipMemsetAsync(vec, 0, (size_t)N * 3 * D::HP * sizeof(float), st));
    if (stop_after == 1) return OARD_OK;

    float* vec2 = (float*)(ws + w.vec2);
    float* vcur = vec;
    float* vnext = vec2;
    const bool msum = !train && g_gcl_msum && E > 0 && gcl_variant == 2 && node_variant == 1 && equi_variant != 0 && tp.npb > 4 &&
                      (tp.CI == 0 || gcl_v1_throughput(c->precision, gcl_variant, topo->conc, tp.CI)) &&
                      (tp.CX == 0 || gcl_v1_throughput(c->precision, gcl_variant, topo->conc, tp.CX));
    g_gcl_msum_taken = msum;
    for (int l = 0; l < c->num_layers; ++l) {
        const LayerOff lo = po.layer[l];
        const bool nv1 = node_variant == 1 && equi_variant != 0;
        const unsigned gN16 = (unsigned)cdiv(N, tp.npb);
        float* ew_in = ew_at(l);
        float* ew_out = ew_at(l + 1);
        if (train) vnext = (float*)(tape + to.vec_in[l + 1]);

        if (nv1) LAUNCH(F_NODE, (k_node_pre_v1<D, NW>), gN16, NW * 64, st, tp, wb, po, lo, (const float*)s_at(l), (const float*)pp0, xhb, P, Q);
        else if constexpr (kV0) LAUNCH(F_NODE, (k_node_pre<D>), gN, 256, st, tp, wb, po, lo, (const float*)s, (const float*)pp0, xhb, P, Q);
        else return OARD_EINVAL;
        if (E > 0) {
            if (gcl_variant == 0) {
                if constexpr (kV0) LAUNCH(F_GCL_EDGE, (k_gcl_edge<D>), gE, 256, st, tp, wb, lo, (const float*)P, (const float*)Q, ew_in, mbuf);
                else return OARD_EINVAL;
            } else {
                GclTape gt{};
                if (train) gt = GclTape{(float*)(tape + to.z1[l]), (float*)(tape + to.z2[l]), (float*)(tape + to.att[l]), (float*)(tape + to.z3[l])};
                int rc = launch_gcl_v1<D>(c->precision, gcl_variant, topo->conc, tp, wb, lo, wb + lo.gcl_stream, P, Q, wb + po.u0, wb + po.c0row, l == 0,
                                          l == c->num_layers - 1, ew_in, ew_out, mbuf, train ? &gt : nullptr, st, msum);
                if (rc != OARD_OK) return rc;
            }
        }
        const bool rows = tp.npb <= 4;
        if (nv1 && rows) LAUNCH(F_NODE, (k_gcl_node_v1<D, NW, true>), gN16, NW * 64, st, tp, wb, lo, (const float*)xhb, (const float*)mbuf, s_mid_at(l), xq,
                                train ? (float*)(tape + to.agg[l]) : nullptr);
        else if (nv1 && msum) LAUNCH(F_NODE, (k_gcl_node_v1<D, NW, false, true>), gN16, NW * 64, st, tp, wb, lo, (const float*)xhb, (const float*)mbuf, s_mid_at(l), xq,
                                     (float*)nullptr);
        else if (nv1) LAUNCH(F_NODE, (k_gcl_node_v1<D, NW, false>), gN16, NW * 64, st, tp, wb, lo, (const float*)xhb, (const float*)mbuf, s_mid_at(l), xq,
                             train ? (float*)(tape + to.agg[l]) : nullptr);
        else if constexpr (kV0) LAUNCH(F_NODE, (k_gcl_node<D>), gN, 256, st, tp, wb, lo, (const float*)xhb, (const float*)mbuf, s, xq);
        else return OARD_EINVAL;
        if (stop_after == 100 + 10 * l + 1) { topo->vec_final = (size_t)((char*)vcur - ws); return OARD_OK; }
        if (equi_variant == 0) {
            if constexpr (kV0) {
                if (A > 0) LAUNCH(F_EQUI_EDGE, (k_equi_edge<D>), gA, 256, st, tp, wb, lo, (const float*)ew_out, (const float*)rbuf,
                                  (const float*)geo, (const float*)xq, (const float*)vcur, xmsg, vmsg);
                LAUNCH(F_NODE, (k_equi_agg<D>), gN, 256, st, tp, wb, lo, (const float*)xmsg, (const float*)vmsg, (const float*)x1,
                       s, vcur, v2buf, scal, vdot);
            } else return OARD_EINVAL;
        } else {
            const bool l0_skip = l == 0 && !train && g_equi_l0_skip && A > 0 && nv1 && !rows &&
                                 equi_v1_shape(c->precision, equi_variant, topo->conc, A, (const float*)(ws + w.d1s)) == 2;
            if (l == 0) g_equi_l0_taken = l0_skip;
            if (A > 0) {
                int rc = launch_equi_v1<D>(c->precision, equi_variant, topo->conc, tp, wb, lo, wb + lo.equi_stream, wb + lo.dp0b, ew_out, rbuf, vmsg,
                                           train ? (float*)(tape + to.zd1[l]) : nullptr, train ? (float*)(tape + to.cd[l]) : nullptr, st,
                                           (float*)(ws + w.d1s), al, l0_skip);
                if (rc != OARD_OK) return rc;
            }
#define EQUI_NODE_V1(D_, ROWS_, XC_) LAUNCH(F_NODE, (k_equi_node_v1<D_, NW, ROWS_, XC_>), gN16, NW * 64, st, tp, wb, lo, (const float*)vmsg, \
                       (const float*)xq, (const float*)geo, (const float*)x1, (const float*)s_mid_at(l), s_at(l + 1), (const float*)vcur, vnext, \
                       train ? (float*)(tape + to.s_a[l]) : nullptr, train ? (float*)(tape + to.vec_a[l]) : nullptr, al)
            if (nv1 && rows) {
                if (lo.xcross) EQUI_NODE_V1(D, true, true); else EQUI_NODE_V1(D, true, false);
            } else if (nv1 && l0_skip) {
                if (lo.xcross) EQUI_NODE_V1(Layer0<D>, false, true); else EQUI_NODE_V1(Layer0<D>, false, false);
            } else if (nv1) {
                if (lo.xcross) EQUI_NODE_V1(D, false, true); else EQUI_NODE_V1(D, false, false);
            } else if constexpr (kV0) {
                LAUNCH(F_NODE, (k_equi_agg_v1<D>), gN, 256, st, tp, wb, lo, (const float*)vmsg, (const float*)xq,
                       (const float*)geo, (const float*)x1, s, (const float*)vcur, vnext, v2buf, scal, vdot);
            } else return OARD_EINVAL;
            std::swap(vcur, vnext);
        }
        if constexpr (kV0) {
            if (!nv1) LAUNCH(F_NODE, (k_equi_upd<D>), gN, 256, st, tp, wb, lo, (const float*)scal, (const float*)vdot,
                             (const float*)v2buf, s, vcur);
        }
        if (stop_after == 100 + 10 * l + 2) { topo->vec_final = (size_t)((char*)vcur - ws); return OARD_OK; }
    }
    if (!train) topo->vec_final = (size_t)((char*)vcur - ws);
    if (train) {
        ZeroRows z;
        z.count = 0;
        auto add = [&](size_t off, size_t row, int ld) {
            if (z.count == 64) { LAUNCH(F_OTHER, k_zero_rows, 64, 256, st, z); z.count = 0; }
            z.p[z.count] = (float*)(tape + off) + row * (size_t)ld; z.n[z.count] = ld; ++z.count;
        };
        for (int l = 0; l <= c->num_layers; ++l) {
            add(to.ew[l], (size_t)E, D::WP);
            if (l == c->num_layers) break;
            add(to.z1[l], (size_t)E, D::HP); add(to.z2[l], (size_t)E, D::HP); add(to.att[l], (size_t)E, 1); add(to.z3[l], (size_t)E, D::WP);
            add(to.zd1[l], (size_t)A, D::D1P); add(to.cd[l], (size_t)A, 3 * D::HP);
        }
        add(to.geo, (size_t)A, GEO_STRIDE); add(to.rbuf, (size_t)A, D::RP);
        if (z.count > 0) LAUNCH(F_OTHER, k_zero_rows, z.count, 256, st, z);
    }
    if (node_variant >= 1)
        LAUNCH(F_NODE, (k_out_v1<D, NW>), gNb, NW * 64, st, tp, wb, po, (const float*)s_at(c->num_layers), (const float*)vcur, dpos, hout, status);
    else if constexpr (kV0)
        LAUNCH(F_NODE, (k_out<D>), gN, 256, st, tp, wb, po, (const float*)s, (const float*)vcur, dpos, hout, status);
    else return OARD_EINVAL;
    LAUNCH(F_OTHER, k_post, cdiv(N, 128), 128, st, tp, op, wb, (const float*)dpos, (const float*)hout, emb);
    HIP_TRY(hipGetLastError());
    return OARD_OK;
}

template <class F> static int dispatch_dims(const oard_config* c, F&& f) {
#define X(h, r) if (c->hidden == (h) && c->num_radial == (r)) { f(Dims<(h), (r)>{}); return 0; }
    OARD_DIMS_LIST
#undef X
    return OARD_EINVAL;
}
#define DISPATCH_DIMS(c, CALL)                                                                         \
    do {                                                                                               \
        if (dispatch_dims((c), [&](auto d_) { using D = decltype(d_); CALL; }) != 0) return OARD_EINVAL; \
    } while (0)

struct BwdLayerOff { size_t gcl, equi, watt; };
struct BwdOff { BwdLayerOff layer[OARD_MAX_LAYERS]; size_t total; };
static BwdOff make_bwd_layout(const oard_config* c) {
    const RDims d(c->hidden, c->num_radial);
    BwdOff b;
    memset(&b, 0, sizeof(b));
    size_t cur = 0;
    auto take = [&](size_t n) { size_t o = cur; cur = align_up(cur + n, 64); return o; };
    for (int l = 0; l < c->num_layers; ++l) {
        b.layer[l].gcl = take((size_t)(2 * d.WB * d.HT + d.HT * d.HT) * 256);
        b.layer[l].equi = take((size_t)(3 * d.HT * d.D1T + d.WB * d.D1T) * 256);
        b.layer[l].watt = take(d.HP);
    }
    b.total = cur;
    return b;
}
template <class D>
static int gcl_backward_impl(const oard_config* c, const TopoDev& tp, const float* pb, const BwdLayerOff& bl, int layer,
                             const char* tape, const TapeOff& to, const float* dagg, float* dew, float* dz3, float* mout,
                             float* dz2, float* da, float* dz1, hipStream_t st, float* gate_part = nullptr, long long* gate_rows = nullptr) {
    GclBwdArgs a;
    a.gate_part = gate_part;
    a.z1 = (const float*)(tape + to.z1[layer]); a.z2 = (const float*)(tape + to.z2[layer]);
    a.att = (const float*)(tape + to.att[layer]); a.z3 = (const float*)(tape + to.z3[layer]);
    a.dagg = dagg; a.watt = pb + bl.watt; a.dew = dew; a.dz3 = dz3; a.mout = mout; a.dz2 = dz2; a.da = da; a.dz1 = dz1;
    const float* stream = pb + bl.gcl;
    const bool last = layer == c->num_layers - 1;
    const long long r_full = last ? tp.A : tp.E;
    long long rows = 0;
    if (r_full > 0) {
        LAUNCH_LDS(F_GCL_BWD, (k_gcl_edge_bwd<D, 8, 2, true>), cdiv(r_full, 128), 512, (GclBwdStream<D, 2>::LDS_BYTES), st,
                   tp, stream, 0LL, r_full, a);
        rows += cdiv(r_full, 128) * 8;
    }
    if (last && tp.E > tp.A) {
        if (a.gate_part) a.gate_part += (size_t)rows * D::HP;
        LAUNCH_LDS(F_GCL_BWD, (k_gcl_edge_bwd<D, 8, 2, false>), cdiv(tp.E - tp.A, 128), 512, (GclBwdStream<D, 2>::LDS_BYTES), st,
                   tp, stream, tp.A, tp.E, a);
        rows += cdiv(tp.E - tp.A, 128) * 8;
    }
    if (gate_rows) *gate_rows = rows;
    HIP_TRY(hipGetLastError());
    return OARD_OK;
}

template <class D>
static int equi_backward_impl(const TopoDev& tp, const float* stream, const float* dcd, const float* zd1, float* dew,
                              float* dzd1, hipStream_t st) {
    LAUNCH_LDS(F_EQUI_BWD, (k_equi_edge_bwd<D, 8>), cdiv(tp.A, 128), 512, (EquiBwdStream<D>::LDS_BYTES), st, tp, stream, dcd,
               zd1, dew, dzd1);
    HIP_TRY(hipGetLastError());
    return OARD_OK;
}

#ifndef OARD_SCAL_BWD_WAVES
#define OARD_SCAL_BWD_WAVES 2
#endif
template <class D>
static int scalarize_backward_impl(const oard_config* c, const TopoDev& tp, const float* wb, const char* tape, const TapeOff& to,
                                   const float* ne1, int ld, const float* dew, float* dne1, float* part, hipStream_t st) {
    const PackOff po = make_layout(c);
    constexpr int NW = OARD_SCAL_BWD_WAVES;
    if (po.signed_scal)
        LAUNCH(F_INIT, (k_scalarize_bwd<D, NW, true>), tp.N, NW * 64, st, tp, wb + po.lin3, ne1, ld, (const float*)(tape + to.geo), dew, dne1, part);
    else
        LAUNCH(F_INIT, (k_scalarize_bwd<D, NW, false>), tp.N, NW * 64, st, tp, wb + po.lin3, ne1, ld, (const float*)(tape + to.geo), dew, dne1, part);
    HIP_TRY(hipGetLastError());
    return OARD_OK;
}

template <class D>
static int equi_msg_backward_impl(const oard_config* c, const TopoDev& tp, const char* tape, const TapeOff& to, int layer, const float* xq, const float* cr,
                                  const float* gs, const float* gv, float* dcd, float* dcr, float* dxq, float* dvec, hipStream_t st) {
    const Strided3 xq3{xq, 3 * D::H, D::H}, vec3{(const float*)(tape + to.vec_in[layer]), 3 * D::HP, D::HP}, cr3{cr, 3 * D::H, D::H},
        gv3{gv, 3 * D::H, D::H};
    LAUNCH(F_NODE, (k_equi_msg_bwd<D>), tp.N, 256, st, tp, (const float*)(tape + to.geo), xq3, vec3, (const float*)(tape + to.cd[layer]), cr3,
           gs, D::H, gv3, dcd, dcr, dxq, dvec, D::H, c->reflect_equiv ? 0 : 1);
    HIP_TRY(hipGetLastError());
    return OARD_OK;
}

struct WgradPlan { int transposed, NT, nPB, nQG, PP, QP, gy; long long rpc; int n_chunks; int lds, PBW, QGW; };
struct WglShape { int NT, PBW, QGW; };
static const WglShape kWglShapes[2] = {{7, 4, 2}, {8, 4, 2}};
static WgradPlan wgrad_plan(int ncY, int ncX, long long rows) {
    WgradPlan p;
    p.transposed = ncX > ncY ? 1 : 0;
    const int ncP = p.transposed ? ncX : ncY, ncQ = p.transposed ? ncY : ncX;
    const int nQT = (int)cdiv(ncQ, 16);
    p.NT = (cdiv(nQT, 7) * 7 <= cdiv(nQT, 8) * 8) ? 7 : 8;
    p.nPB = (int)cdiv(ncP, 64); p.nQG = (int)cdiv(nQT, p.NT);
    p.PP = p.nPB * 64; p.QP = p.nQG * p.NT * 16;
    p.gy = (int)cdiv((long long)p.nPB * p.nQG, 4);
    long long want = std::max<long long>(1, g_wgrad_wgs / p.gy);
    want = std::min(want, std::max<long long>(1, cdiv(rows, rows < 16384 ? 128 : 64)));
    p.rpc = align_up((size_t)cdiv(std::max<long long>(rows, 1), want), 4 * OARD_WG_PD);
    p.n_chunks = (int)cdiv(std::max<long long>(rows, 1), p.rpc);
    p.lds = 0; p.PBW = 4; p.QGW = 2;
// ... 273 lines not shown
        fl.erase(fl.begin());
    }
    void* p = nullptr;
    *cap = align_up(bytes + bytes / 8, (size_t)1 << 16);
    const hipError_t e = kind == 0 ? hipMalloc(&p, *cap) : hipHostMalloc(&p, *cap, hipHostMallocDefault);
    if (e != hipSuccess) { (void)hipGetLastError(); return nullptr; }
    return p;
}
static void pool_release(void* p, size_t cap, const hipStream_t* streams, int n_streams, bool sync_device, int kind = 0) {
    if (!p) return;
    TablePool& tp = table_pool();
    std::lock_guard<std::mutex> lk(tp.m);
    if (sync_device) { (void)hipDeviceSynchronize(); tp.free_[kind].push_back({p, cap}); return; }
    TablePool::Pending q{p, cap, {}, 0, kind};
    hipStream_t all[5] = {device_streams()[2]};
    int n = 1;
    for (int k = 0; k < n_streams && k < 4; ++k) if (streams[k] != all[0]) all[n++] = streams[k];
    for (int k = 0; k < n && q.n_ev < 4; ++k) {
        hipEvent_t e = nullptr;
        if (!tp.spare_events.empty()) { e = tp.spare_events.back(); tp.spare_events.pop_back(); }
        else if (hipEventCreateWithFlags(&e, hipEventDisableTiming) != hipSuccess) { (void)hipDeviceSynchronize(); tp.free_[kind].push_back({p, cap}); return; }
        (void)hipEventRecord(e, all[k]);
        q.ev[q.n_ev++] = e;
    }
    if (n > 4) { (void)hipDeviceSynchronize(); }
    tp.pending.push_back(q);
}
struct UploadItem { const void* src; size_t bytes; size_t off; };
static int pool_upload(void* dev, const std::vector<UploadItem>& items, size_t total, void** stage_out, size_t* stage_cap) {
    char* stage = (char*)pool_alloc(total, stage_cap, 1);
    if (!stage) return OARD_EHIP;
    for (const UploadItem& it : items) memcpy(stage + it.off, it.src, it.bytes);
    if (hipMemcpyAsync(dev, stage, total, hipMemcpyHostToDevice, device_streams()[2]) != hipSuccess) {
        (void)hipGetLastError();
        pool_release(stage, *stage_cap, nullptr, 0, true, 1);
        return OARD_EHIP;
    }
    *stage_out = stage;
    return OARD_OK;
}
static void topo_touch(const oard_topology* tp, hipStream_t st) {
    if (!tp) return;
    for (int i = 0; i < tp->n_used; ++i) if (tp->used_on[i] == st) return;
    if (tp->ready) (void)hipStreamWaitEvent(st, tp->ready, 0);
    if (tp->n_used < 4) tp->used_on[tp->n_used++] = st; else tp->used_many = true;
}

static int build_part(const oard_config* c, const int64_t* cm, const int64_t* nfs, int N_all, const std::vector<int>& obj_start,
                      const std::vector<int>& dense, const std::vector<long long>& ref_ptr_ref, int lo, int hi,
                      TopoPart& part, int& max_group, int& max_ns) {
    const int n_obj = c->n_obj, B = hi - lo;
    std::vector<int> order;
    for (int i = 0; i < N_all; ++i) if (dense[i] >= lo && dense[i] < hi) order.push_back(i);
    std::stable_sort(order.begin(), order.end(), [&](int a, int b) {
        if (dense[a] != dense[b]) return dense[a] < dense[b];
        return nfs[a] < nfs[b];
    });
    const int N = (int)order.size();
    if (N < 1) return OARD_EINVAL;
    std::vector<int> node_obj(N), node_row(N), node_ref(N), node_tidx(N), node_sample(N), sample_ptr(B + 1, 0),
        grp_ptr((size_t)B * n_obj + 1, 0), edge_ptr(N), act_ptr(N + 1, 0);
    for (int n = 0; n < N; ++n) {
        const int r = order[n], sb = dense[r] - lo;
        node_ref[n] = r; node_obj[n] = (int)nfs[r]; node_row[n] = r - obj_start[nfs[r]];
        node_tidx[n] = (int)cm[r]; node_sample[n] = sb;
        sample_ptr[sb + 1]++;
        grp_ptr[(size_t)sb * n_obj + nfs[r] + 1]++;
    }
    for (int b = 0; b < B; ++b) sample_ptr[b + 1] += sample_ptr[b];
    for (size_t q = 0; q < (size_t)B * n_obj; ++q) grp_ptr[q + 1] += grp_ptr[q];
    long long E = 0, A = 0;
    for (int b = 0; b < B; ++b) {
        const long long ns = sample_ptr[b + 1] - sample_ptr[b];
        max_ns = std::max(max_ns, (int)ns);
        for (int n = sample_ptr[b]; n < sample_ptr[b + 1]; ++n) { edge_ptr[n] = (int)E; E += ns - 1; }
        if (E > 0x7fffffffLL) return OARD_EINVAL;
    }
    for (size_t q = 0; q < (size_t)B * n_obj; ++q) {
        const long long ng = grp_ptr[q + 1] - grp_ptr[q];
        max_group = std::max(max_group, (int)ng);
        A += ng * (ng - 1);
    }
    if (max_group > OARD_MAX_GROUP || A > 0x7fffffffLL) return OARD_EINVAL;
    std::vector<int> edge_src((size_t)E + 1, 0), edge_tgt((size_t)E + 1, 0);
    for (int b = 0; b < B; ++b) {
        const int s0 = sample_ptr[b], s1 = sample_ptr[b + 1];
        for (int n = s0; n < s1; ++n) {
            size_t e = (size_t)edge_ptr[n];
            for (int m = s0; m < s1; ++m) if (m != n) { edge_src[e] = n; edge_tgt[e] = m; ++e; }
        }
    }
    std::vector<int> act_src((size_t)A + 1, 0), act_tgt((size_t)A + 1, 0), act_edge((size_t)A + 1, (int)E);
    {
        size_t a = 0;
        for (int n = 0; n < N; ++n) {
            const int q = node_sample[n] * n_obj + node_obj[n];
            const int g0 = grp_ptr[q], g1 = grp_ptr[q + 1], s0 = sample_ptr[node_sample[n]];
            act_ptr[n] = (int)a;
            for (int m = g0; m < g1; ++m) if (m != n) {
                act_src[a] = m; act_tgt[a] = n;
                act_edge[a] = edge_ptr[m] + (n - s0) - (n > m ? 1 : 0);
                ++a;
            }
        }
        act_ptr[N] = (int)a;
    }
    std::vector<int> edge_row((size_t)std::max<long long>(E, 1), -1), row_src((size_t)E + 1, 0), row_tgt((size_t)E + 1, 0),
        row_eid((size_t)E + 1, (int)E);
    {
        for (long long a = 0; a < A; ++a) {
            edge_row[act_edge[a]] = (int)a; row_src[a] = act_src[a]; row_tgt[a] = act_tgt[a]; row_eid[a] = act_edge[a];
        }
        long long r = A;
        for (long long e = 0; e < E; ++e)
            if (edge_row[e] < 0) { edge_row[e] = (int)r; row_src[r] = edge_src[e]; row_tgt[r] = edge_tgt[e]; row_eid[r] = (int)e; ++r; }
    }
    std::vector<long long> ref_edge_ptr(N);
    for (int n = 0; n < N; ++n) ref_edge_ptr[n] = ref_ptr_ref[node_ref[n]];
    std::vector<int> col_row, col_info, node_cols((size_t)N * 4, 0);
    long long CI = 0, CX = 0;
    {
        auto pad16 = [&]() { while (col_row.size() % 16) col_row.push_back((int)E); };
        for (int b = 0; b < B; ++b) {
            for (int n = sample_ptr[b]; n < sample_ptr[b + 1]; ++n) {
                const int q = node_sample[n] * n_obj + node_obj[n];
                const int g0 = grp_ptr[q], g1 = grp_ptr[q + 1];
                node_cols[4 * (size_t)n + 0] = (int)col_row.size();
                for (int m = g0; m < g1; ++m) if (m != n) col_row.push_back(act_ptr[m] + (n - g0) - (n > m ? 1 : 0));
                node_cols[4 * (size_t)n + 1] = (int)col_row.size();
            }
            pad16();
        }
        CI = (long long)col_row.size();
        for (int b = 0; b < B; ++b) {
            const int ns = sample_ptr[b + 1] - sample_ptr[b];
            for (int n = sample_ptr[b]; n < sample_ptr[b + 1]; ++n) {
                node_cols[4 * (size_t)n + 2] = (int)col_row.size();
                for (long long e = edge_ptr[n]; e < (long long)edge_ptr[n] + ns - 1; ++e) if (edge_row[e] >= A) col_row.push_back(edge_row[e]);
                node_cols[4 * (size_t)n + 3] = (int)col_row.size();
            }
            pad16();
        }
        CX = (long long)col_row.size() - CI;
        if (CI + CX > 0x7fffffffLL - 256) return OARD_EINVAL;
        if (col_row.empty()) col_row.push_back((int)E);
        col_info.resize(col_row.size() * 4);
        for (size_t k = 0; k < col_row.size(); ++k) {
            const int r = col_row[k];
            col_info[4 * k] = r; col_info[4 * k + 1] = row_src[r]; col_info[4 * k + 2] = row_tgt[r];
            col_info[4 * k + 3] = r == (int)E ? -1 : row_src[r] + 1;
        }
    }

    std::vector<UploadItem> items;
    size_t cur = 0;
    auto add = [&](const void* p, size_t bytes) { UploadItem it{p, bytes, cur}; cur = align_up(cur + bytes, 256); items.push_back(it); return it.off; };
    const size_t o_obj = add(node_obj.data(), N * 4), o_row = add(node_row.data(), N * 4), o_ref = add(node_ref.data(), N * 4),
                 o_tidx = add(node_tidx.data(), N * 4), o_smp = add(node_sample.data(), N * 4),
                 o_sptr = add(sample_ptr.data(), (B + 1) * 4), o_eptr = add(edge_ptr.data(), N * 4),
                 o_esrc = add(edge_src.data(), edge_src.size() * 4), o_etgt = add(edge_tgt.data(), edge_tgt.size() * 4),
                 o_gptr = add(grp_ptr.data(), grp_ptr.size() * 4), o_aptr = add(act_ptr.data(), (N + 1) * 4),
                 o_asrc = add(act_src.data(), act_src.size() * 4), o_atgt = add(act_tgt.data(), act_tgt.size() * 4),
                 o_aedge = add(act_edge.data(), act_edge.size() * 4), o_rptr = add(ref_edge_ptr.data(), N * 8),
                 o_erow = add(edge_row.data(), edge_row.size() * 4), o_rsrc = add(row_src.data(), row_src.size() * 4),
                 o_rtgt = add(row_tgt.data(), row_tgt.size() * 4), o_reid = add(row_eid.data(), row_eid.size() * 4),
                 o_crow = add(col_info.data(), col_info.size() * 4), o_ncol = add(node_cols.data(), node_cols.size() * 4);
    size_t cap = 0;
    char* dev = (char*)pool_alloc(cur, &cap);
    if (!dev) return OARD_EHIP;
    if (int rc = pool_upload(dev, items, cur, &part.stage, &part.stage_cap)) { pool_release(dev, cap, nullptr, 0, false); return rc; }
    part.dev_cap = cap;
    part.dev_block = dev;
    TopoDev& d = part.d;
    d.N = N; d.B = B; d.n_obj = n_obj; d.n_groups = B * n_obj; d.E = E; d.A = A;
    d.node_obj = (const int*)(dev + o_obj); d.node_row = (const int*)(dev + o_row); d.node_ref = (const int*)(dev + o_ref);
    d.node_tidx = (const int*)(dev + o_tidx); d.node_sample = (const int*)(dev + o_smp); d.sample_ptr = (const int*)(dev + o_sptr);
    d.edge_ptr = (const int*)(dev + o_eptr); d.edge_src = (const int*)(dev + o_esrc); d.edge_tgt = (const int*)(dev + o_etgt);
    d.grp_ptr = (const int*)(dev + o_gptr); d.act_ptr = (const int*)(dev + o_aptr); d.act_src = (const int*)(dev + o_asrc);
    d.act_tgt = (const int*)(dev + o_atgt); d.act_edge = (const int*)(dev + o_aedge);
    d.ref_edge_ptr = (const long long*)(dev + o_rptr);
    d.edge_row = (const int*)(dev + o_erow); d.row_src = (const int*)(dev + o_rsrc); d.row_tgt = (const int*)(dev + o_rtgt);
    d.row_eid = (const int*)(dev + o_reid);
    d.CI = CI; d.CX = CX; d.col_info = (const int*)(dev + o_crow); d.node_cols = (const int*)(dev + o_ncol);
    return OARD_OK;
}

int oard_topology_create(const oard_config* c, const int64_t* cm, const int64_t* nfs, int64_t n_nodes,
                         oard_topology** out) {
    return oard_topology_create_parts(c, cm, nfs, n_nodes, g_parts, out);
}

int oard_topology_create_parts(const oard_config* c, const int64_t* cm, const int64_t* nfs, int64_t n_nodes,
                               int parts, oard_topology** out) {
    if (!config_ok(c) || !cm || !nfs || !out || n_nodes < 1 || n_nodes > (1 << 24)) return OARD_EINVAL;
    const int N = (int)n_nodes, n_obj = c->n_obj;
    std::vector<int> obj_start(n_obj + 1, 0);
    for (int i = 0; i < N; ++i) {
        if (nfs[i] < 0 || nfs[i] >= n_obj) return OARD_EINVAL;
        if (i > 0 && nfs[i] < nfs[i - 1]) return OARD_EINVAL;
        obj_start[nfs[i] + 1]++;
    }
    for (int k = 0; k < n_obj; ++k) obj_start[k + 1] += obj_start[k];
    std::vector<int64_t> samples(cm, cm + N);
    std::sort(samples.begin(), samples.end());
    samples.erase(std::unique(samples.begin(), samples.end()), samples.end());
    const int B = (int)samples.size();
    if (samples.front() < 0 || samples.back() > (1 << 30)) return OARD_EINVAL;
    std::vector<int> dense(N), ns_of(B, 0);
    for (int i = 0; i < N; ++i) {
        dense[i] = (int)(std::lower_bound(samples.begin(), samples.end(), cm[i]) - samples.begin());
        ns_of[dense[i]]++;
    }
    std::vector<long long> ref_ptr_ref(N);
    long long E_all = 0;
    for (int r = 0; r < N; ++r) { ref_ptr_ref[r] = E_all; E_all += ns_of[dense[r]] - 1; }

    int n_parts = parts > 0 ? parts : (B >= 32 ? 4 : (B >= 16 ? 2 : 1));
    n_parts = std::max(1, std::min(std::min(n_parts, OARD_MAX_PARTS), B));
    oard_topology* tp = new oard_topology();
    (void)hipGetDevice(&tp->device);
    tp->n_obj = n_obj; tp->B = B; tp->n_parts = n_parts;
    {
        std::vector<int> tab(2 * (size_t)N), seen(B, 0);
        for (int r = 0; r < N; ++r) { tab[r] = dense[r]; tab[(size_t)N + r] = seen[dense[r]]++; }
        const size_t b_int = 2 * (size_t)N * sizeof(int), b_all = align_up(b_int, 8) + (size_t)N * sizeof(long long);
        tp->ref_block = pool_alloc(b_all, &tp->ref_cap);
        if (!tp->ref_block) { delete tp; return OARD_EHIP; }
        const std::vector<UploadItem> ref_items = {{tab.data(), b_int, 0}, {ref_ptr_ref.data(), (size_t)N * sizeof(long long), align_up(b_int, 8)}};
        if (int rc = pool_upload(tp->ref_block, ref_items, b_all, &tp->ref_stage, &tp->ref_stage_cap)) { oard_topology_destroy(tp); return rc; }
        tp->ref_sample = (const int*)tp->ref_block; tp->ref_rank = tp->ref_sample + N;
        tp->ref_ptr = (const long long*)((char*)tp->ref_block + align_up(b_int, 8));
        tp->N_ref = N;
    }
    for (int k = 0; k <= n_obj && k <= OARD_MAX_OBJECTS; ++k) tp->obj_start[k] = obj_start[k];
    for (int p = 0; p < n_parts; ++p) {
        const int lo = (int)((long long)B * p / n_parts), hi = (int)((long long)B * (p + 1) / n_parts);
        int rc = build_part(c, cm, nfs, N, obj_start, dense, ref_ptr_ref, lo, hi, tp->parts[p], tp->max_group, tp->max_ns);
        if (rc != OARD_OK) { oard_topology_destroy(tp); return rc; }
        tp->N += tp->parts[p].d.N; tp->E += tp->parts[p].d.E; tp->A += tp->parts[p].d.A;
        tp->parts[p].conc = n_parts;
    }
    {
        const int npb = g_npb > 0 ? g_npb : (int)std::max<long long>(1, std::min<long long>(16, cdiv(tp->N, 256)));
        for (int p = 0; p < n_parts; ++p) tp->parts[p].d.npb = npb;
    }
    if (n_parts > 1) {
        HIP_TRY(hipEventCreateWithFlags(&tp->ev_fork, hipEventDisableTiming));
        for (int p = 1; p < n_parts; ++p) {
            tp->side[p] = device_streams()[(p - 1) % 3];
            if (!tp->side[p]) { oard_topology_destroy(tp); return OARD_EHIP; }
            HIP_TRY(hipEventCreateWithFlags(&tp->ev_join[p], hipEventDisableTiming));
        }
    }
    HIP_TRY(hipEventCreateWithFlags(&tp->ready, hipEventDisableTiming));
    HIP_TRY(hipEventRecord(tp->ready, device_streams()[2]));
    *out = tp;
    return OARD_OK;
}

void oard_topology_destroy(oard_topology* tp) {
    if (!tp) return;
    int cur = tp->device;
    (void)hipGetDevice(&cur);
    if (cur != tp->device) (void)hipSetDevice(tp->device);
    struct Restore { int cur, dev; ~Restore() { if (cur != dev) (void)hipSetDevice(cur); } } restore_{cur, tp->device};
    for (int p = 0; p < OARD_MAX_PARTS; ++p) {
        pool_release(tp->parts[p].dev_block, tp->parts[p].dev_cap, tp->used_on, tp->n_used, tp->used_many);
        pool_release(tp->parts[p].stage, tp->parts[p].stage_cap, nullptr, 0, false, 1);
        if (tp->ev_join[p]) (void)hipEventDestroy(tp->ev_join[p]);
    }
    if (tp->ev_fork) (void)hipEventDestroy(tp->ev_fork);
    pool_release(tp->ref_block, tp->ref_cap, tp->used_on, tp->n_used, tp->used_many);
    pool_release(tp->ref_stage, tp->ref_stage_cap, nullptr, 0, false, 1);
    if (tp->ready) (void)hipEventDestroy(tp->ready);
    delete tp;
}
int64_t oard_topology_num_nodes(const oard_topology* tp) { return tp ? tp->N : 0; }
int64_t oard_topology_num_edges(const oard_topology* tp) { return tp ? tp->E : 0; }
int64_t oard_topology_num_inner_edges(const oard_topology* tp) { return tp ? tp->A : 0; }
int64_t oard_topology_num_samples(const oard_topology* tp) { return tp ? tp->B : 0; }

int oard_topology_check_edge_index(const oard_topology* tp, const int64_t* ei, int64_t n_edges, int32_t* ok,
                                   oard_stream_t stream) {
    topo_touch(tp, (hipStream_t)stream);
    if (!tp || !ok) return OARD_EINVAL;
    hipStream_t st = (hipStream_t)stream;
    const int one = (n_edges == tp->E) ? 1 : 0;
    HIP_TRY(hipMemcpyAsync(ok, &one, sizeof(int), hipMemcpyHostToDevice, st));
    HIP_TRY(hipStreamSynchronize(st));
    if (one && tp->E > 0) {
        if (!ei) return OARD_EINVAL;
        unsigned* bitmap = nullptr;
        const size_t words = (size_t)cdiv(tp->E, 32);
        HIP_TRY(hipMalloc(&bitmap, words * sizeof(unsigned)));
        hipError_t e1 = hipMemsetAsync(bitmap, 0, words * sizeof(unsigned), st);
        if (e1 == hipSuccess) {
            hipLaunchKernelGGL(k_check_edge_set, dim3((unsigned)cdiv(n_edges, 256)), dim3(256), 0, st, tp->ref_sample, tp->ref_rank,
                               tp->ref_ptr, tp->N_ref, (const long long*)ei, (long long)n_edges, bitmap, (int*)ok);
            e1 = hipGetLastError();
        }
        const hipError_t e2 = hipStreamSynchronize(st);
        (void)hipFree(bitmap);
        HIP_TRY(e1);
        HIP_TRY(e2);
    }
    return OARD_OK;
}

static size_t ws_total(const oard_config* c, const oard_topology* tp) {
    size_t cur = 0;
    for (int p = 0; p < tp->n_parts; ++p) {
        const_cast<TopoPart&>(tp->parts[p]).ws_off = cur;
        cur = align_up(cur + make_ws(c, tp->parts[p].d).total, 4096);
    }
    return cur;
}
size_t oard_workspace_bytes(const oard_config* c, const oard_topology* tp) {
    if (!config_ok(c) || !tp) return 0;
    return ws_total(c, tp);
}

int oard_debug_lin3u_table(const oard_config* c, const void* packed, int layer, float* out, oard_stream_t stream) {
    static_assert(OARD_L3T_FLOATS == L3T_FLOATS, "include/oard.h and csrc/oard_layout.h disagree on the table size");
    if (!config_ok(c) || !packed || !out || layer < 0 || layer >= c->num_layers) return OARD_EINVAL;
    const PackOff po = make_layout(c);
    HIP_TRY(hipMemcpyAsync(out, (const float*)packed + po.layer[layer].l3t, (size_t)L3T_FLOATS * sizeof(float), hipMemcpyDeviceToDevice,
                           (hipStream_t)stream));
    return OARD_OK;
}

int oard_active_inner_edges(const oard_config* c, const oard_topology* topo, const void* ws, size_t ws_bytes, int64_t* n_active,
                            oard_stream_t stream) {
    if (!config_ok(c) || !topo || !ws || !n_active) return OARD_EINVAL;
    if (ws_bytes < ws_total(c, topo)) return OARD_ENOMEM;
    hipStream_t st = (hipStream_t)stream;
    long long total = 0;
// ... 652 lines not shown
    NanPtrs np;
    memset(&np, 0, sizeof(np));
    for (int k = 0; k < c->n_obj; ++k) { np.noise[k] = noise[k]; np.out[k] = out[k]; np.node_nf[k] = c->node_nf[k]; }
    for (int p = 0; p < topo->n_parts; ++p)
        LAUNCH(F_OTHER, k_nan_replace, cdiv(topo->parts[p].d.N, 128), 128, (hipStream_t)stream, topo->parts[p].d, np, (const int*)status);
    HIP_TRY(hipGetLastError());
    return OARD_OK;
}

static LossCfg make_loss_cfg(const oard_config* c, const float* norm_values, const float* norm_biases, const float* scales, int pos_only,
                             int fixed_mask, int T) {
    LossCfg lc;
    memset(&lc, 0, sizeof(lc));
    for (int i = 0; i < 3; ++i) { lc.norm_value[i] = norm_values ? norm_values[i] : 1.0f; lc.norm_bias[i] = norm_biases ? norm_biases[i] : 0.0f; }
    for (int k = 0; k < c->n_obj; ++k) lc.scale[k] = scales ? scales[k] : 1.0f;
    lc.pos_only = pos_only; lc.fixed_mask = fixed_mask; lc.T = T;
    return lc;
}
int oard_loss_prepare(const oard_config* c, const oard_topology* topo, const float* const* pos, const int64_t* const* one_hot,
                      const int64_t* const* charge, const float* const* noise, const float* t_int, const float* gamma, int T,
                      const float* norm_values, const float* norm_biases, int pos_only, int fixed_mask, float* const* z,
                      float* const* eps, oard_stream_t stream) {
    topo_touch(topo, (hipStream_t)stream);
    if (!config_ok(c) || !topo || topo->n_parts != 1 || !pos || !one_hot || !charge || !noise || !t_int || !gamma || !z || !eps)
        return OARD_EINVAL;
    LossPtrs lp;
    memset(&lp, 0, sizeof(lp));
    for (int k = 0; k < c->n_obj; ++k) {
        if (c->node_nf[k] < 5 || c->node_nf[k] - 4 > 16) return OARD_EINVAL;
        lp.pos[k] = pos[k]; lp.one_hot[k] = (const long long*)one_hot[k]; lp.charge[k] = (const long long*)charge[k];
        lp.noise[k] = noise[k]; lp.z[k] = z[k]; lp.eps[k] = eps[k]; lp.node_nf[k] = c->node_nf[k];
    }
    const TopoDev& tp = topo->parts[0].d;
    LAUNCH(F_OTHER, k_loss_prep, cdiv(tp.N, 128), 128, (hipStream_t)stream, tp, lp,
           make_loss_cfg(c, norm_values, norm_biases, nullptr, pos_only, fixed_mask, T), t_int, gamma);
    HIP_TRY(hipGetLastError());
    return OARD_OK;
}
int oard_loss_terms(const oard_config* c, const oard_topology* topo, const float* const* eps, const float* const* net,
                    const float* const* z, const int64_t* const* one_hot, const int64_t* const* charge, const float* t_int,
                    const float* gamma, int T, const float* norm_values, const float* norm_biases, const float* scales, int pos_only,
                    int B, float* nll, float* terms, float* const* dnet, oard_stream_t stream) {
    topo_touch(topo, (hipStream_t)stream);
    if (!config_ok(c) || !topo || topo->n_parts != 1 || !eps || !net || !z || !one_hot || !charge || !t_int || !gamma || !nll || !terms ||
        !dnet || B < 1)
        return OARD_EINVAL;
    LossPtrs lp;
    memset(&lp, 0, sizeof(lp));
    for (int k = 0; k < c->n_obj; ++k) {
        if (c->node_nf[k] < 5 || c->node_nf[k] - 4 > 16) return OARD_EINVAL;
        lp.eps[k] = (float*)eps[k]; lp.net[k] = net[k]; lp.z[k] = (float*)z[k]; lp.one_hot[k] = (const long long*)one_hot[k];
        lp.charge[k] = (const long long*)charge[k]; lp.dnet[k] = dnet[k]; lp.node_nf[k] = c->node_nf[k];
    }
    const TopoDev& tp = topo->parts[0].d;
    LAUNCH(F_OTHER, k_loss_terms, tp.B, 64, (hipStream_t)stream, tp, lp, make_loss_cfg(c, norm_values, norm_biases, scales, pos_only, 0, T),
           t_int, gamma, B, nll, terms);
    HIP_TRY(hipGetLastError());
    return OARD_OK;
}
int oard_adamw_step(float* param, const float* grad, float* exp_avg, float* exp_avg_sq, float* max_exp_avg_sq, int64_t n, double lr,
                    double beta1, double beta2, double eps, double weight_decay, int64_t step, int amsgrad, double grad_scale,
                    oard_stream_t stream) {
    if (!param || !grad || !exp_avg || !exp_avg_sq || (amsgrad && !max_exp_avg_sq) || n < 0 || step < 1) return OARD_EINVAL;
    if (n == 0) return OARD_OK;
    const double bc1 = 1.0 - pow(beta1, (double)step), bc2 = 1.0 - pow(beta2, (double)step);
    LAUNCH(F_OTHER, k_adamw, cdiv(n, 256), 256, (hipStream_t)stream, param, grad, exp_avg, exp_avg_sq, max_exp_avg_sq, (long long)n,
           (float)(1.0 - lr * weight_decay), (float)(1.0 - beta1), (float)beta2, (float)(1.0 - beta2), (float)eps, (float)(lr / bc1),
           (float)(1.0 / sqrt(bc2)), amsgrad, (float)grad_scale);
    HIP_TRY(hipGetLastError());
    return OARD_OK;
}

int oard_adamw_step_dev(float* param, const float* grad, float* exp_avg, float* exp_avg_sq, float* max_exp_avg_sq, int64_t n, double lr,
                        double beta1, double beta2, double eps, double weight_decay, int amsgrad, int clip, double* clip_state,
                        int capacity, const float* grad_norm, const float* flag, float* out4, oard_stream_t stream) {
    if (!param || !grad || !exp_avg || !exp_avg_sq || (amsgrad && !max_exp_avg_sq) || n < 0 || !clip_state || capacity < 1 || capacity > 64 ||
        !grad_norm || !flag || !out4)
        return OARD_EINVAL;
    LAUNCH(F_OTHER, k_clip_decide, 1, 64, (hipStream_t)stream, clip_state, capacity, grad_norm, flag, clip, lr, beta1, beta2, eps, weight_decay, out4);
    if (n > 0)
        LAUNCH(F_OTHER, k_adamw_dev, cdiv(n, 256), 256, (hipStream_t)stream, param, grad, exp_avg, exp_avg_sq, max_exp_avg_sq, (long long)n, amsgrad,
               reinterpret_cast<const AdamScal*>(clip_state + 4 + capacity));
    HIP_TRY(hipGetLastError());
    return OARD_OK;
}

int oard_train_scratch_entry(const oard_config* c, const oard_topology* topo, int which, size_t* offset_bytes, int64_t* rows,
                             int64_t* row_floats) {
    if (!config_ok(c) || !topo || topo->n_parts != 1 || !offset_bytes || !rows || !row_floats) return OARD_EINVAL;
    const TopoDev& d = topo->parts[0].d;
    const TrainWs w = make_train_ws(c, d);
    const RDims r(c->hidden, c->num_radial);
    switch (which) {
        case OARD_SCRATCH_XH: *offset_bytes = w.xh; *rows = d.N; *row_floats = r.HP; break;
        case OARD_SCRATCH_XQ: *offset_bytes = w.xq; *rows = d.N; *row_floats = 3 * r.HP; break;
        case OARD_SCRATCH_CR: *offset_bytes = w.cr; *rows = d.A + 1; *row_floats = 3 * r.HP; break;
        case OARD_SCRATCH_DCD: *offset_bytes = w.dcd; *rows = d.A + 1; *row_floats = 3 * r.HP; break;
        case OARD_SCRATCH_DCR: *offset_bytes = w.dcr; *rows = d.A + 1; *row_floats = 3 * r.HP; break;
        default: return OARD_EINVAL;
    }
    return OARD_OK;
}

int oard_tap(const oard_config* c, const oard_topology* topo, const void* ws_, int which, int layer, float* dst,
             oard_stream_t stream) {
    topo_touch(topo, (hipStream_t)stream);
    if (!config_ok(c) || !topo || !ws_ || !dst || layer != 0) return OARD_EINVAL;
    const RDims d(c->hidden, c->num_radial);
    ws_total(c, topo);
    hipStream_t st = (hipStream_t)stream;
    for (int p = 0; p < topo->n_parts; ++p) {
        const TopoDev& tp = topo->parts[p].d;
        const WsOff w = make_ws(c, tp);
        const char* ws = (const char*)ws_ + topo->parts[p].ws_off;
        auto nodes = [&](const float* src, int ld, int sections, int sect_pad, int sect_len) {
            const long long tot = (long long)tp.N * sections * sect_len;
            hipLaunchKernelGGL(k_tap_nodes, dim3((unsigned)cdiv(tot, 256)), dim3(256), 0, st, tp, src, ld, sections, sect_pad, sect_len, dst);
        };
        switch (which) {
            case OARD_TAP_S: nodes((const float*)(ws + w.s), d.HP, 1, d.HP, d.H); break;
            case OARD_TAP_VEC: nodes((const float*)(ws + topo->parts[p].vec_final), 3 * d.HP, 3, d.HP, d.H); break;
            case OARD_TAP_NE1: nodes((const float*)(ws + w.ne1), 3 * d.HP, 3, d.HP, d.H); break;
            case OARD_TAP_POS_FRAME: nodes((const float*)(ws + w.pf32), 3, 1, 3, 3); break;
            case OARD_TAP_DPOS: nodes((const float*)(ws + w.dpos), 3, 1, 3, 3); break;
            case OARD_TAP_HOUT: nodes((const float*)(ws + w.hout), 16, 1, 16, c->in_hidden); break;
            case OARD_TAP_LABELS:
                hipLaunchKernelGGL(k_tap_labels, dim3((unsigned)cdiv(tp.N, 256)), dim3(256), 0, st, tp, (const int*)(ws + w.labels), dst);
                break;
            case OARD_TAP_EDGE:
                if (tp.E > 0)
                    hipLaunchKernelGGL(k_tap_edges, dim3((unsigned)cdiv(tp.E * d.W, 256)), dim3(256), 0, st, tp,
                                       (const float*)(ws + w.ew), d.WP, d.W, dst);
                break;
            default: return OARD_EINVAL;
        }
    }
    HIP_TRY(hipGetLastError());
    return OARD_OK;
}

int oard_debug_stop_after(int code) { g_stop_after = code; return OARD_OK; }
int oard_debug_option(const char* name, int value) {
    if (!name) return OARD_EINVAL;
    if (!kV0 && value == 0 && (strcmp(name, "gcl_variant") == 0 || strcmp(name, "equi_variant") == 0 || strcmp(name, "node_variant") == 0))
        return OARD_EINVAL;
    if (strcmp(name, "gcl_variant") == 0) { g_gcl_variant = value; return OARD_OK; }
    if (strcmp(name, "equi_variant") == 0) { g_equi_variant = value; return OARD_OK; }
    if (strcmp(name, "node_variant") == 0) { g_node_variant = value; return OARD_OK; }
    if (strcmp(name, "experiments") == 0) return kV0 ? OARD_OK : OARD_EINVAL;
    if (strcmp(name, "gcl_skip") == 0) { g_gcl_skip = value; return OARD_OK; }
    if (strcmp(name, "equi_skip") == 0) { g_equi_skip = value; return OARD_OK; }
    if (strcmp(name, "equi_l0_skip") == 0) { g_equi_l0_skip = value; return OARD_OK; }
    if (strcmp(name, "gcl_msum") == 0) { g_gcl_msum = value; return OARD_OK; }
    if (strcmp(name, "gcl_msum_taken") == 0) return g_gcl_msum_taken ? OARD_OK : OARD_EINVAL;
    if (strcmp(name, "equi_l0_taken") == 0) return g_equi_l0_taken ? OARD_OK : OARD_EINVAL;
    if (strcmp(name, "gcl_persist") == 0) { g_gcl_persist = value; return OARD_OK; }
    if (strcmp(name, "gcl_grid") == 0) { g_gcl_grid = value; return OARD_OK; }
    if (strcmp(name, "skip_families") == 0) { g_skip_families = value; return OARD_OK; }
    if (strcmp(name, "parts") == 0) { g_parts = value; return OARD_OK; }
    if (strcmp(name, "sequential") == 0) { g_sequential = value; return OARD_OK; }
    if (strcmp(name, "poison") == 0) { g_poison = value; return OARD_OK; }
    if (strcmp(name, "auto_small") == 0) { g_auto_small = value; return OARD_OK; }
    if (strcmp(name, "auto_tiny") == 0) { g_auto_tiny = value; return OARD_OK; }
    if (strcmp(name, "npb") == 0) { g_npb = value; return OARD_OK; }
    if (strcmp(name, "wgrad_wgs") == 0) { g_wgrad_wgs = value; return OARD_OK; }
    if (strcmp(name, "wgrad_t16") == 0) { g_wgrad_t16 = value; return OARD_OK; }
    if (strcmp(name, "wgrad_queue") == 0) { g_wgrad_queue = value; return OARD_OK; }
    if (strcmp(name, "gate_fold") == 0) { g_gate_fold = value; return OARD_OK; }
    if (strcmp(name, "wgrad_lds") == 0) { g_wgrad_lds = value; return OARD_OK; }
    if (strcmp(name, "wgrad_shapes") == 0) { g_wgrad_shapes = value & 3; return OARD_OK; }
    if (strcmp(name, "train_dual") == 0) { g_train_dual = value; return OARD_OK; }
    if (strcmp(name, "small_split") == 0) { g_small_split = value; return OARD_OK; }
    return OARD_EINVAL;
}
#ifdef OARD_PHASE_PROBE
int oard_debug_probe_read(unsigned long long* out8) {
    if (!out8) return OARD_EINVAL;
    HIP_TRY(hipDeviceSynchronize());
    HIP_TRY(hipMemcpyFromSymbol(out8, HIP_SYMBOL(g_phase_probe), 8 * sizeof(unsigned long long)));
    unsigned long long z[8] = {};
    HIP_TRY(hipMemcpyToSymbol(HIP_SYMBOL(g_phase_probe), z, sizeof(z)));
    return OARD_OK;
}
#endif
#ifdef OARD_TIMELINE
int oard_debug_timeline_read(long long* out, int waves) {
    if (!out || waves < 1 || waves > 16) return OARD_EINVAL;
    HIP_TRY(hipDeviceSynchronize());
    HIP_TRY(hipMemcpyFromSymbol(out, HIP_SYMBOL(g_timeline), (size_t)waves * TL_MAX * sizeof(long long)));
    return OARD_OK;
}
#endif
#ifdef OARD_EXPERIMENTS
int oard_debug_fp_timeouts(unsigned int* out) {
    if (!out) return OARD_EINVAL;
    HIP_TRY(hipDeviceSynchronize());
    HIP_TRY(hipMemcpyFromSymbol(out, HIP_SYMBOL(g_fp_timeouts), sizeof(unsigned int)));
    return OARD_OK;
}
#endif
int oard_timing_enable(int on) { g_timing.on = on != 0; return OARD_OK; }
int oard_timing_reset(void) {
    g_timing.flush();
    for (int f = 0; f < F_COUNT; ++f) { g_timing.total_ms[f] = 0; g_timing.launches[f] = 0; }
    return OARD_OK;
}
int oard_timing_get(const char* family, double* total_ms, int64_t* launches) {
    if (!family || !total_ms || !launches) return OARD_EINVAL;
    g_timing.flush();
    for (int f = 0; f < F_COUNT; ++f)
        if (strcmp(family, kFamilyNames[f]) == 0) { *total_ms = g_timing.total_ms[f]; *launches = g_timing.launches[f]; return OARD_OK; }
    return OARD_EINVAL;
}

}
```

### oareactdiff_amd/csrc/oard_inst.h

```cpp
#pragma once
#if !defined(OARD_EXPERIMENTS) && !defined(OARD_SINGLE_TU)

#define OARD_UNPAREN(...) __VA_ARGS__
#ifdef OARD_INST_DEFINE
#define OARD_INST(K, ARGS) template __global__ void OARD_UNPAREN K ARGS;
#else
#define OARD_INST(K, ARGS) extern template __global__ void OARD_UNPAREN K ARGS;
#endif
#ifndef OARD_DIMS_LIST
#define OARD_DIMS_LIST X(196, 96) X(32, 8) X(32, 32)
#endif
#define OARD_BOOL4(M, D) M(D, true, true) M(D, false, true) M(D, true, false) M(D, false, false)

#define OARD_NW(h) (((h) + 15) / 16 <= 16 ? ((h) + 15) / 16 : 8)
#define OARD_A_GCL (TopoDev, const float*, const float*, const float*, const float*, const float*, long long, long long, const float*, float*, float*, GclTape)

#if !defined(OARD_INST_DEFINE) || defined(OARD_INST_UNIT_GCL_P)
#define OARD_I_GCL_P(D, S1, S3) OARD_INST((k_gcl_edge_p<OARD_UNPAREN D, S1, S3, false>), OARD_A_GCL) OARD_INST((k_gcl_edge_p<OARD_UNPAREN D, S1, S3, true>), OARD_A_GCL) \
    OARD_INST((k_gcl_edge_p<OARD_UNPAREN D, S1, S3, false, true>), OARD_A_GCL)
#define X(h, r) OARD_BOOL4(OARD_I_GCL_P, (Dims<h, r>))
OARD_DIMS_LIST
#undef X
#endif

#if !defined(OARD_INST_DEFINE) || defined(OARD_INST_UNIT_GCL_V1)
#define OARD_I_GCL_V1(D, S1, S3) \
    OARD_INST((k_gcl_edge_v1<OARD_UNPAREN D, 8, 2, S1, S3, false, false, 2, 3>), OARD_A_GCL) OARD_INST((k_gcl_edge_v1<OARD_UNPAREN D, 8, 2, S1, S3, true, false, 2, 3>), OARD_A_GCL) \
    OARD_INST((k_gcl_edge_v1<OARD_UNPAREN D, 8, 2, S1, S3, false, true, 2, 3>), OARD_A_GCL) \
    OARD_INST((k_gcl_edge_v1<OARD_UNPAREN D, 4, 2, S1, S3, false, false, 2, 2>), OARD_A_GCL) \
    OARD_INST((k_gcl_edge_small<OARD_UNPAREN D, 8, S1, S3>), (TopoDev, const float*, LayerOff, const float*, const float*, const float*, const float*, long long, long long, float*, float*))
#define X(h, r) OARD_BOOL4(OARD_I_GCL_V1, (Dims<h, r>))
OARD_DIMS_LIST
#undef X
#endif

#if !defined(OARD_INST_DEFINE) || defined(OARD_INST_UNIT_B3)
#define OARD_A_EQUI_B3 (TopoDev, const float*, const float*, const float*, const float*, const float*, float*, float*, float*, float*, ActList)
#define OARD_I_GCL_B3(D, S1, S3) OARD_INST((k_gcl_edge_b3<OARD_UNPAREN D, S1, S3, false>), OARD_A_GCL) OARD_INST((k_gcl_edge_b3<OARD_UNPAREN D, S1, S3, true>), OARD_A_GCL)
#define X(h, r) OARD_BOOL4(OARD_I_GCL_B3, (Dims<h, r>)) OARD_INST((k_equi_edge_b3<Dims<h, r>, false>), OARD_A_EQUI_B3) OARD_INST((k_equi_edge_b3<Dims<h, r>, true>), OARD_A_EQUI_B3)
OARD_DIMS_LIST
#undef X
#endif

#if !defined(OARD_INST_DEFINE) || defined(OARD_INST_UNIT_EQUI)
#define OARD_A_EQUI (TopoDev, const float*, const float*, const float*, const float*, float*, float*, float*, ActList, int)
#define OARD_A_EQUI_NODE (TopoDev, const float*, LayerOff, const float*, const float*, const float*, const float*, const float*, float*, const float*, float*, float*, float*, ActList)
#define X(h, r) \
    OARD_INST((k_equi_edge_v1<Dims<h, r>, 8, false>), OARD_A_EQUI) OARD_INST((k_equi_edge_v1<Dims<h, r>, 8, true>), OARD_A_EQUI) \
    OARD_INST((k_equi_edge_v1<Dims<h, r>, 4, false>), OARD_A_EQUI) \
    OARD_INST((k_equi_node_v1<Dims<h, r>, OARD_NW(h), false, false>), OARD_A_EQUI_NODE) OARD_INST((k_equi_node_v1<Dims<h, r>, OARD_NW(h), false, true>), OARD_A_EQUI_NODE) \
    OARD_INST((k_equi_node_v1<Dims<h, r>, OARD_NW(h), true, false>), OARD_A_EQUI_NODE) OARD_INST((k_equi_node_v1<Dims<h, r>, OARD_NW(h), true, true>), OARD_A_EQUI_NODE) \
    OARD_INST((k_equi_node_v1<Layer0<Dims<h, r> >, OARD_NW(h), false, false>), OARD_A_EQUI_NODE) OARD_INST((k_equi_node_v1<Layer0<Dims<h, r> >, OARD_NW(h), false, true>), OARD_A_EQUI_NODE) \
    OARD_INST((k_gcl_edge_bwd<Dims<h, r>, 8, 2, true>), (TopoDev, const float*, long long, long long, GclBwdArgs)) \
    OARD_INST((k_gcl_edge_bwd<Dims<h, r>, 8, 2, false>), (TopoDev, const float*, long long, long long, GclBwdArgs)) \
    OARD_INST((k_equi_edge_bwd<Dims<h, r>, 8>), (TopoDev, const float*, const float*, const float*, float*, float*))
OARD_DIMS_LIST
#undef X
#endif

#if !defined(OARD_INST_DEFINE) || defined(OARD_INST_UNIT_NODE)
#define OARD_A_GCL_NODE (TopoDev, const float*, LayerOff, const float*, const float*, float*, float*, float*)
#define OARD_A_OUT (TopoDev, const float*, PackOff, const float*, const float*, float*, float*, int*)
#define OARD_A_SCAL_BWD (TopoDev, const float*, const float*, int, const float*, const float*, float*, float*)
#define OARD_A_MSG_BWD (TopoDev, const float*, Strided3, Strided3, const float*, Strided3, const float*, int, Strided3, float*, float*, float*, float*, int, int, int)
#define X(h, r) \
    OARD_INST((k_gcl_node_v1<Dims<h, r>, OARD_NW(h), false>), OARD_A_GCL_NODE) OARD_INST((k_gcl_node_v1<Dims<h, r>, OARD_NW(h), true>), OARD_A_GCL_NODE) \
    OARD_INST((k_gcl_node_v1<Dims<h, r>, OARD_NW(h), false, true>), OARD_A_GCL_NODE) \
    OARD_INST((k_out_v1<Dims<h, r>, OARD_NW(h)>), OARD_A_OUT) \
    OARD_INST((k_scalarize_bwd<Dims<h, r>, 2, false>), OARD_A_SCAL_BWD) OARD_INST((k_scalarize_bwd<Dims<h, r>, 2, true>), OARD_A_SCAL_BWD) \
    OARD_INST((k_equi_msg_bwd<Dims<h, r> >), OARD_A_MSG_BWD)
OARD_DIMS_LIST
#undef X
OARD_INST((k_lin3u_bwd_fused<4>), (const float*, const float*, const float*, long long, float*, float*))
#define OARD_I_ROWS(KB, EPI) OARD_INST((k_rows_dense<KB, EPI, 8>), (RowsDense)) OARD_INST((k_rows_dense_long<KB, EPI, 8, 4>), (RowsDense))
OARD_I_ROWS(13, 0) OARD_I_ROWS(13, 2) OARD_I_ROWS(13, 3) OARD_I_ROWS(7, 3) OARD_I_ROWS(6, 0) OARD_I_ROWS(6, 1) OARD_I_ROWS(4, 1) OARD_I_ROWS(4, 3)
OARD_INST((k_rows_dense<26, 1, 8>), (RowsDense)) OARD_INST((k_rows_dense<26, 3, 8>), (RowsDense))
OARD_INST((k_rows_dense2<13, 1, 8, 13>), (RowsDense2)) OARD_INST((k_rows_dense2<13, 2, 8, 13>), (RowsDense2))
OARD_INST((k_rows_dense2<26, 1, 8, 13>), (RowsDense2)) OARD_INST((k_rows_dense2<39, 2, 8, 13>), (RowsDense2))
#endif

#if !defined(OARD_INST_DEFINE) || defined(OARD_INST_UNIT_WGRAD)
#define OARD_A_WG (const float*, int, int, const float*, int, int, long long, long long, long long, int, int, float*, float*, float*)
OARD_INST((k_wgrad_t16<4, 7, false>), (WgtArgs)) OARD_INST((k_wgrad_t16<4, 7, true>), (WgtArgs)) OARD_INST((k_wgrad_t16<5, 3, false>), (WgtArgs))
OARD_INST((k_wgrad_t16<5, 5, true>), (WgtArgs)) OARD_INST((k_wgrad_t16<5, 7, true>), (WgtArgs)) OARD_INST((k_wgrad_t16<6, 5, false>), (WgtArgs))
OARD_INST((k_wgrad_t16<6, 7, false>), (WgtArgs))
OARD_INST((k_wgrad<false, 7>), OARD_A_WG) OARD_INST((k_wgrad<false, 8>), OARD_A_WG) OARD_INST((k_wgrad<true, 7>), OARD_A_WG) OARD_INST((k_wgrad<true, 8>), OARD_A_WG)
OARD_INST((k_wgrad_lds<false, 7, 4, 2>), OARD_A_WG) OARD_INST((k_wgrad_lds<false, 8, 4, 2>), OARD_A_WG)
OARD_INST((k_wgrad_lds<true, 7, 4, 2>), OARD_A_WG) OARD_INST((k_wgrad_lds<true, 8, 4, 2>), OARD_A_WG)
#endif

#endif
```

### oareactdiff_amd/csrc/oard_layout.h

```cpp
#pragma once
#include <hip/hip_runtime.h>
#include <stdint.h>
#include <stddef.h>
#include "../../include/oard.h"

#define OARD_MAX_LAYERS 16
#define OARD_MAX_GROUP 1024

template <int H_, int R_>
struct Dims {
    static constexpr int H = H_, R = R_;
    static constexpr int HT = (H + 15) / 16, HP = HT * 16;
    static constexpr int W = 3 * H + R, WB = (W + 15) / 16, WP = WB * 16;
    static constexpr int RB = (R + 15) / 16, RP = RB * 16;
    static constexpr int H2 = H / 2, PB = (H2 + 15) / 16, PP = PB * 16;
    static constexpr int D1T = (3 * H + 15) / 16, D1P = D1T * 16;
    static constexpr int H4 = H / 4;
    static_assert(H % 4 == 0 && R % 4 == 0, "feature widths must be multiples of 4");
};

struct RDims {
    int H, R, HT, HP, W, WB, WP, RB, RP, H2, PB, PP, D1T, D1P, H4;
    explicit RDims(int h, int r) {
        H = h; R = r; HT = (H + 15) / 16; HP = HT * 16; W = 3 * H + R; WB = (W + 15) / 16; WP = WB * 16;
        RB = (R + 15) / 16; RP = RB * 16; H2 = H / 2; PB = (H2 + 15) / 16; PP = PB * 16;
        D1T = (3 * H + 15) / 16; D1P = D1T * 16; H4 = H / 4;
    }
};

#define L3T_X 16.0f
#define L3T_H 0.03125f
#define L3T_N 1024
#define L3T_FLOATS (2 * (L3T_N + 1) + 4)

struct LayerOff {
    size_t ln_g_w, ln_g_b, W1a, b1, W1b, W1c, W2, b2, watt, batt, W3, b3, nm0, nm0b, nm1, nm1b;
    size_t ln_q_w, ln_q_b, xp0, xp2, dp0, dp0b, dp2, dp2b, rbfp;
    size_t vp, xv0, xv2, l3u;
    size_t l3t;
    size_t gcl_stream, equi_stream;
    size_t gcl_b3, equi_b3;
    int xcross;
};
struct PackOff {
    size_t emb, emb_b, nbemb, nbemb_b, s2v, s2v_b, rl0, rl0_b, rl2, rl2_b;
    size_t lin3;
    size_t pe0;
    size_t pe1, embout, embout_b, v1p, v2p, un0, un0_b, un2, un2_b;
    size_t c0row;
    size_t u0;
    size_t rbf_means, rbf_betas;
    size_t enc[OARD_MAX_OBJECTS], dec[OARD_MAX_OBJECTS];
    LayerOff layer[OARD_MAX_LAYERS];
    size_t total;
    int signed_scal;
};

struct TopoDev {
    int N, B, n_obj, n_groups;
    int npb;
    long long E, A;
    const int *node_obj, *node_row, *node_ref, *node_tidx, *node_sample, *sample_ptr;
    const int *edge_ptr, *edge_src, *edge_tgt;
    const int *edge_row;
    const int *row_src, *row_tgt;
    const int *row_eid;
    const int *grp_ptr;
    const int *act_ptr, *act_src, *act_tgt, *act_edge;
    const long long *ref_edge_ptr;
    long long CI, CX;
    const int *col_info;
    const int *node_cols;
};

struct ActList {
    const int* rows;
    const int* src;
    const int* pre;
    const int* n;
};

#define OARD_MAX_PARTS 8
struct TopoPart {
    TopoDev d;
    void* dev_block = nullptr;
    size_t dev_cap = 0;
    void* stage = nullptr;
    size_t stage_cap = 0;
    size_t ws_off = 0;
    int conc = 1;
    mutable size_t vec_final = 0;
};
struct oard_topology {
    int device = 0;
    int n_parts = 0;
    TopoPart parts[OARD_MAX_PARTS];
    int n_obj = 0, B = 0;
    long long N = 0, E = 0, A = 0;
    int max_group = 0, max_ns = 0;
    int obj_start[OARD_MAX_OBJECTS + 1] = {};
    hipStream_t side[OARD_MAX_PARTS] = {};
    hipEvent_t ev_fork = nullptr, ev_join[OARD_MAX_PARTS] = {};
    void* ref_block = nullptr;
    size_t ref_cap = 0;
    void* ref_stage = nullptr;
    size_t ref_stage_cap = 0;
    hipEvent_t ready = nullptr;
    mutable hipStream_t used_on[4] = {};
    mutable int n_used = 0;
    mutable bool used_many = false;
    const int *ref_sample = nullptr, *ref_rank = nullptr;
    const long long* ref_ptr = nullptr;
    int N_ref = 0;
};

struct WsOff {
    size_t pos, pf64, pf32, x1, pp0, labels, hin, zemb, nb, s, s1, ne1, xh, P, Q, xq, vec, vec2, v2buf, sc0, vdot,
        geo, d64, rbuf, ew, mbuf, xmsg, vmsg, dpos, hout, total;
    size_t al_rows, al_src, al_pre, al_cnt, al_n;
    size_t d1s;
    size_t small_a, small_b;
};
```

### oareactdiff_amd/csrc/oard_node_v1.h

```cpp
#pragma once
#include "oard_kernels.h"

OARD_DEV f4 lds_blk(const float* v, int b, int lane) { return *reinterpret_cast<const f4*>(v + b * 256 + lane * 4); }
OARD_DEV void lds_st(float* v, int t, int lane, f4 x) { *reinterpret_cast<f4*>(v + t * 256 + lane * 4) = x; }

#ifndef OARD_NODE_PF
#define OARD_NODE_PF 13
#endif
template <int KB>
OARD_DEV f4 dense_tile_lds(const float* __restrict__ wp, int t, const float* in, int lane, f4 init) {
    const float* base = wp + ((size_t)t * KB * 64 + lane) * 4;
    f4 c0 = init, c1 = f4zero();
    constexpr int G = OARD_NODE_PF;
#pragma unroll
    for (int b0 = 0; b0 < KB; b0 += G) {
        f4 a[G];
#pragma unroll
        for (int i = 0; i < G; ++i)
            if (b0 + i < KB) a[i] = ld_f4(base + (size_t)(b0 + i) * 256);
        __builtin_amdgcn_sched_barrier(0);
#pragma unroll
        for (int i = 0; i < G; ++i)
            if (b0 + i < KB) {
                const f4 x = lds_blk(in, b0 + i, lane);
// ... 296 lines not shown
        if (ROWS) {
            const RowLanes rl = row_lanes(tp.N, tp.npb, nb.lane);
            const int nn = min(blockIdx.x * tp.npb + rl.node, tp.N - 1);
            const int smp2 = tp.node_sample[nn];
            const int deg2 = rl.live ? tp.sample_ptr[smp2 + 1] - tp.sample_ptr[smp2] - 1 : 0;
            const size_t e2 = (size_t)tp.edge_ptr[nn];
            const int mx2 = wave_max(deg2), last2 = max(deg2 - 1, 0);
            for (int k = 0; k < mx2; k += 2 * rl.L) {
                const int k0 = k + rl.slot, k1 = k0 + rl.L;
                const f4 r0 = ld_blk(mbuf, e2 + min(k0, last2), D::HP, t, nb.lane), r1 = ld_blk(mbuf, e2 + min(k1, last2), D::HP, t, nb.lane);
                if (k0 < deg2) a0 += r0;
                if (k1 < deg2) a1 += r1;
            }
            a0 = rows_total4(a0 + a1, rl, nb.lane);
            a1 = f4zero();
        }
        const int last = max(deg - 1, 0);
        for (int k = 0; MSUM && k < mxp; k += 8) {
            f4 r[8];
#pragma unroll
            for (int i = 0; i < 8; ++i) r[i] = ld_blk(mbuf, pc(min(k + i, max(cnt - 1, 0))), D::HP, t, nb.lane);
#pragma unroll
            for (int i = 0; i < 8; ++i) {
                const f4 v = k + i < cnt ? r[i] : f4zero();
                if (i & 1) a1 += v; else a0 += v;
            }
        }
        for (int k = 0; !ROWS && !MSUM && k < mx; k += 8) {
            f4 r[8];
#pragma unroll
            for (int i = 0; i < 8; ++i) r[i] = ld_blk(mbuf, e0 + min(k + i, last), D::HP, t, nb.lane);
#pragma unroll
            for (int i = 0; i < 8; ++i) {
                const f4 v = k + i < deg ? r[i] : f4zero();
                if (i & 1) a1 += v; else a0 += v;
            }
        }
        lds_st(in, D::HT + t, nb.lane, (a0 + a1) * inv);
        if (agg_out != nullptr && nb.valid) st_blk(agg_out, nb.n, D::HP, t, nb.lane, (a0 + a1) * inv);
    }
    __syncthreads();
    constexpr int TPW = (D::HT + WAVES - 1) / WAVES, TPW3 = (3 * D::HT + WAVES - 1) / WAVES;
    int tw[TPW];
#pragma unroll
    for (int i = 0; i < TPW; ++i) tw[i] = min(nb.wave + i * WAVES, D::HT - 1);
    {
        TileJob job[TPW];
        f4 acc[TPW];
#pragma unroll
        for (int i = 0; i < TPW; ++i) { job[i] = tile_job<2 * D::HT>(wb + lo.nm0, tw[i], in); acc[i] = ld_vec(wb + lo.nm0b, tw[i], nb.lane); }
        dense_seq<2 * D::HT, TPW, OARD_GCL_NODE_G>(job, nb.lane, acc);
#pragma unroll
        for (int i = 0; i < TPW; ++i)
            if (nb.wave + i * WAVES < D::HT) lds_st(hm, tw[i], nb.lane, silu4(acc[i]));
    }
    __syncthreads();
    {
        TileJob job[TPW];
        f4 acc[TPW];
#pragma unroll
        for (int i = 0; i < TPW; ++i) { job[i] = tile_job<D::HT>(wb + lo.nm1, tw[i], hm); acc[i] = ld_vec(wb + lo.nm1b, tw[i], nb.lane); }
        dense_seq<D::HT, TPW, OARD_GCL_NODE_G>(job, nb.lane, acc);
#pragma unroll
        for (int i = 0; i < TPW; ++i)
            if (nb.wave + i * WAVES < D::HT) {
                const f4 v = lds_blk(in, tw[i], nb.lane) + acc[i];
                lds_st(sv, tw[i], nb.lane, v);
                if (nb.valid) st_blk(s, nb.n, D::HP, tw[i], nb.lane, v);
            }
    }
    __syncthreads();
    float mean, rstd;
    ln_stats_lds<D::HT, D::H>(sv, nb.lane, mean, rstd);
    float* xln = in;
    float* hq = in + D::HT * 256;
    for (int t = nb.wave; t < D::HT; t += WAVES)
        lds_st(xln, t, nb.lane, ln_apply<D::H>(lds_blk(sv, t, nb.lane), mean, rstd, wb + lo.ln_q_w, wb + lo.ln_q_b, t, nb.lane));
    __syncthreads();
    {
        TileJob job[TPW];
        f4 acc[TPW];
#pragma unroll
        for (int i = 0; i < TPW; ++i) { job[i] = tile_job<D::HT>(wb + lo.xp0, tw[i], xln); acc[i] = f4zero(); }
        dense_seq<D::HT, TPW, OARD_GCL_NODE_G>(job, nb.lane, acc);
#pragma unroll
        for (int i = 0; i < TPW; ++i)
            if (nb.wave + i * WAVES < D::HT) lds_st(hq, tw[i], nb.lane, silu4(acc[i]));
    }
    __syncthreads();
    {
        TileJob job[TPW3];
        f4 acc[TPW3];
#pragma unroll
        for (int i = 0; i < TPW3; ++i) {
            job[i] = tile_job<D::HT>(wb + lo.xp2, min(nb.wave + i * WAVES, 3 * D::HT - 1), hq);
            acc[i] = f4zero();
        }
        dense_seq<D::HT, TPW3, OARD_GCL_NODE_G>(job, nb.lane, acc);
#pragma unroll
        for (int i = 0; i < TPW3; ++i)
            if (nb.wave + i * WAVES < 3 * D::HT && nb.valid) st_blk(xq, nb.n, 3 * D::HP, nb.wave + i * WAVES, nb.lane, acc[i]);
    }
}

OARD_DEV void lin3u_stage(const float* __restrict__ p, float* l3s, int tid, int nthreads) {
    for (int i = tid; i < 48 * 12; i += nthreads) {
        const int k = i / 12, j = i % 12;
        l3s[i] = j < 8 ? p[192 + j * 48 + k] : (j == 8 ? p[3 * k] : (j == 9 ? p[144 + k] : 0.f));
    }
}
OARD_DEV f4 lin3u4(const float* l3s, const float* __restrict__ p, f4 x) {
    const float* b2 = p + 576;
    const float* w4 = p + 584;
    f4 h2[8];
#pragma unroll
    for (int j = 0; j < 8; ++j) h2[j] = (f4){b2[j], b2[j], b2[j], b2[j]};
#pragma unroll 4
    for (int k = 0; k < 48; ++k) {
        const f4 wa = *reinterpret_cast<const f4*>(l3s + 12 * k), wc = *reinterpret_cast<const f4*>(l3s + 12 * k + 4);
        const float w0 = l3s[12 * k + 8], b0 = l3s[12 * k + 9];
        const f4 h = silu4(x * w0 + b0);
        h2[0] += h * wa.x; h2[1] += h * wa.y; h2[2] += h * wa.z; h2[3] += h * wa.w;
        h2[4] += h * wc.x; h2[5] += h * wc.y; h2[6] += h * wc.z; h2[7] += h * wc.w;
    }
    const float b4 = p[592];
    f4 o = (f4){b4, b4, b4, b4};
#pragma unroll
    for (int j = 0; j < 8; ++j) o += silu4(h2[j]) * w4[j];
    return o;
}

OARD_DEV float lin3u1(const float* l3s, const float* __restrict__ p, float x) {
    const float* b2 = p + 576;
    const float* w4 = p + 584;
    float h2[8];
#pragma unroll
    for (int j = 0; j < 8; ++j) h2[j] = b2[j];
#pragma unroll 4
    for (int k = 0; k < 48; ++k) {
        const f4 wa = *reinterpret_cast<const f4*>(l3s + 12 * k), wc = *reinterpret_cast<const f4*>(l3s + 12 * k + 4);
        const float h = silu1(x * l3s[12 * k + 8] + l3s[12 * k + 9]);
        h2[0] += h * wa.x; h2[1] += h * wa.y; h2[2] += h * wa.z; h2[3] += h * wa.w;
        h2[4] += h * wc.x; h2[5] += h * wc.y; h2[6] += h * wc.z; h2[7] += h * wc.w;
    }
    float o = p[592];
#pragma unroll
    for (int j = 0; j < 8; ++j) o += silu1(h2[j]) * w4[j];
    return o;
}

template <class D> struct Layer0 : D {};
template <class D> struct is_layer0 { static constexpr bool value = false; };
template <class D> struct is_layer0<Layer0<D> > { static constexpr bool value = true; };
template <class D, int WAVES, bool ROWS = false, bool XC = false>
__global__ __launch_bounds__(WAVES * 64) void k_equi_node_v1(TopoDev tp, const float* __restrict__ wb, LayerOff lo,
                                                             const float* __restrict__ qbuf, const float* __restrict__ xq,
                                                             const float* __restrict__ geo, const float* __restrict__ x1,
                                                             const float* s, float* s_out, const float* __restrict__ vec_in,
                                                             float* __restrict__ vec_out,
                                                             float* __restrict__ sa_out, float* __restrict__ va_out ,
                                                             ActList al ) {
    constexpr bool L0 = is_layer0<D>::value;
    static_assert(!(L0 && ROWS), "the layer-0 form exists for the large-batch gather only");
    constexpr int HT = D::HT;
    constexpr int TPW = (HT + WAVES - 1) / WAVES;
    __shared__ __attribute__((aligned(16))) float sm[6 * HT * 256 + 48 * 12 + L3T_FLOATS];
    float* l3s = sm + 6 * HT * 256;
    float* l3t = l3s + 48 * 12;
#ifdef OARD_NO_L3T
    const bool l3t_ok = false;
#else
    const bool l3t_ok = tp.npb > 4 && (wb + lo.l3t)[2 * (L3T_N + 1)] > 0.5f;
#endif
    if (l3t_ok)
        for (int i = threadIdx.x; i < 2 * (L3T_N + 1) / 4; i += WAVES * 64)
            reinterpret_cast<f4*>(l3t)[i] = ld_f4(wb + lo.l3t + 4 * i);
    if (l3t_ok && threadIdx.x < 2) l3t[2 * (L3T_N + 1) - 2 + threadIdx.x] = (wb + lo.l3t)[2 * (L3T_N + 1) - 2 + threadIdx.x];
#ifdef OARD_TIMELINE
    const bool tl_on_ = blockIdx.x == gridDim.x / 2 && (threadIdx.x & 63) == 0; int tl_n_ = 0;
#endif
    TL(1);
    lin3u_stage(wb + lo.l3u, l3s, threadIdx.x, WAVES * 64);
    float* vx = sm;
    float* in = sm + 3 * HT * 256;
    float* hx = sm + 5 * HT * 256;
    const NodeBlk nb = node_blk(tp.N, tp.npb);
    const int n = nb.n;
    const bool listed = al.pre != nullptr && (long long)__builtin_amdgcn_readfirstlane(*al.n) != tp.A;
    const int a0 = listed ? al.pre[tp.act_ptr[n]] : tp.act_ptr[n];
    const int cnt = nb.valid ? (listed ? al.pre[tp.act_ptr[n + 1]] : tp.act_ptr[n + 1]) - a0 : 0;
    const int mx = wave_max(cnt);
    auto row_of = [&](int k) -> int { return listed ? al.rows[k] : k; };
    auto src_of = [&](int k) -> int { return listed ? al.src[k] : tp.act_src[k]; };
    const float inv_sqrt2 = 0.70710678118654752f, inv_sqrt3 = 0.57735026918962576f,
                inv_sqrt_h = 1.0f / sqrtf((float)D::H);

    for (int t = nb.wave; t < HT; t += WAVES) {
        f4 dx = f4zero(), v0 = f4zero(), v1 = f4zero(), v2 = f4zero();
        const f4 xn0 = ld_blk(xq, n, 3 * D::HP, t, nb.lane), xn1 = ld_blk(xq, n, 3 * D::HP, HT + t, nb.lane),
                 xn2 = ld_blk(xq, n, 3 * D::HP, 2 * HT + t, nb.lane);
        const int a_hi = (int)max(tp.A - 1, 0LL);
        if (ROWS) {
            const RowLanes rl = row_lanes(tp.N, tp.npb, nb.lane);
            const int nn = min(blockIdx.x * tp.npb + rl.node, tp.N - 1);
            const int b0 = listed ? al.pre[tp.act_ptr[nn]] : tp.act_ptr[nn];
            const int cnt2 = rl.live ? (listed ? al.pre[tp.act_ptr[nn + 1]] : tp.act_ptr[nn + 1]) - b0 : 0;
            const int mx2 = wave_max(cnt2);
            const f4 zn0 = ld_blk(xq, nn, 3 * D::HP, t, nb.lane), zn1 = ld_blk(xq, nn, 3 * D::HP, HT + t, nb.lane),
                     zn2 = ld_blk(xq, nn, 3 * D::HP, 2 * HT + t, nb.lane);
            for (int k = 0; k < mx2; k += rl.L) {
                const int kk = k + rl.slot;
                const int ke = min(b0 + min(kk, max(cnt2 - 1, 0)), a_hi);
                const size_t a = cnt2 > 0 ? (size_t)row_of(ke) : 0;
                const int m = cnt2 > 0 ? src_of(ke) : 0;
                const float* gp = geo + a * GEO_STRIDE;
                const float gx = gp[2], gy = gp[3], gz = gp[4];
                const float cx = XC ? gp[5] : 0.f, cy = XC ? gp[6] : 0.f, cz = XC ? gp[7] : 0.f;
                const f4 q0 = ld_blk(qbuf, a, 3 * D::HP, t, nb.lane), q1 = ld_blk(qbuf, a, 3 * D::HP, HT + t, nb.lane),
                         q2 = ld_blk(qbuf, a, 3 * D::HP, 2 * HT + t, nb.lane);
                const f4 y0 = ld_blk(xq, m, 3 * D::HP, t, nb.lane), y1 = ld_blk(xq, m, 3 * D::HP, HT + t, nb.lane),
                         y2 = ld_blk(xq, m, 3 * D::HP, 2 * HT + t, nb.lane);
                const f4 w0 = ld_blk(vec_in, (size_t)m * 3 + 0, D::HP, t, nb.lane), w1 = ld_blk(vec_in, (size_t)m * 3 + 1, D::HP, t, nb.lane),
                         w2 = ld_blk(vec_in, (size_t)m * 3 + 2, D::HP, t, nb.lane);
                if (kk < cnt2) {
                    const f4 xm = (y0 + zn0) * q0;
                    dx += xm;
                    const f4 a2 = (y1 + zn1) * q1 * inv_sqrt3;
                    const f4 a3 = (y2 + zn2) * q2;
                    v0 += (XC ? w0 * a2 + a3 * gx + xm * cx : w0 * a2 + a3 * gx) * inv_sqrt_h;
                    v1 += (XC ? w1 * a2 + a3 * gy + xm * cy : w1 * a2 + a3 * gy) * inv_sqrt_h;
                    v2 += (XC ? w2 * a2 + a3 * gz + xm * cz : w2 * a2 + a3 * gz) * inv_sqrt_h;
                }
            }
            dx = rows_total4(dx, rl, nb.lane); v0 = rows_total4(v0, rl, nb.lane);
            v1 = rows_total4(v1, rl, nb.lane); v2 = rows_total4(v2, rl, nb.lane);
        }
        int mnext[2], rnext[2];
        auto entry = [&](int kk, int& m, int& r) {
            const int ke = min(a0 + min(kk, max(cnt - 1, 0)), a_hi);
            m = cnt > 0 ? src_of(ke) : 0;
            r = cnt > 0 ? row_of(ke) : 0;
        };
#pragma unroll
        for (int i = 0; i < 2; ++i) entry(i, mnext[i], rnext[i]);
        float zero1 = 0.f;
        if (L0) asm volatile("" : "+v"(zero1));
        const f4 zero4 = {zero1, zero1, zero1, zero1};
        for (int k = 0; !ROWS && k < mx; k += 2) {
            f4 q0[2], q1[2], q2[2], y0[2], y1[2], y2[2], w0[2], w1[2], w2[2];
            float gx[2], gy[2], gz[2], cx[2], cy[2], cz[2];
            const int mc[2] = {mnext[0], mnext[1]}, rc[2] = {rnext[0], rnext[1]};
#pragma unroll
            for (int i = 0; i < 2; ++i)
                entry(k + 2 + i, mnext[i], rnext[i]);
#pragma unroll
            for (int i = 0; i < 2; ++i) {
                const size_t a = (size_t)rc[i];
                const int m = mc[i];
                const float* g = geo + a * GEO_STRIDE;
                gx[i] = g[2]; gy[i] = g[3]; gz[i] = g[4];
                cx[i] = XC ? g[5] : 0.f; cy[i] = XC ? g[6] : 0.f; cz[i] = XC ? g[7] : 0.f;
                q0[i] = ld_blk(qbuf, a, 3 * D::HP, t, nb.lane); q1[i] = L0 ? zero4 : ld_blk(qbuf, a, 3 * D::HP, HT + t, nb.lane);
                q2[i] = ld_blk(qbuf, a, 3 * D::HP, 2 * HT + t, nb.lane);
                y0[i] = ld_blk(xq, m, 3 * D::HP, t, nb.lane); y1[i] = L0 ? zero4 : ld_blk(xq, m, 3 * D::HP, HT + t, nb.lane);
                y2[i] = ld_blk(xq, m, 3 * D::HP, 2 * HT + t, nb.lane);
                w0[i] = L0 ? zero4 : ld_blk(vec_in, (size_t)m * 3 + 0, D::HP, t, nb.lane);
                w1[i] = L0 ? zero4 : ld_blk(vec_in, (size_t)m * 3 + 1, D::HP, t, nb.lane);
                w2[i] = L0 ? zero4 : ld_blk(vec_in, (size_t)m * 3 + 2, D::HP, t, nb.lane);
            }
#pragma unroll
            for (int i = 0; i < 2; ++i)
                if (k + i < cnt) {
                    const f4 xm = (y0[i] + xn0) * q0[i];
                    dx += xm;
                    const f4 a2 = (y1[i] + xn1) * q1[i] * inv_sqrt3;
                    const f4 a3 = (y2[i] + xn2) * q2[i];
                    v0 += (XC ? w0[i] * a2 + a3 * gx[i] + xm * cx[i] : w0[i] * a2 + a3 * gx[i]) * inv_sqrt_h;
                    v1 += (XC ? w1[i] * a2 + a3 * gy[i] + xm * cy[i] : w1[i] * a2 + a3 * gy[i]) * inv_sqrt_h;
                    v2 += (XC ? w2[i] * a2 + a3 * gz[i] + xm * cz[i] : w2[i] * a2 + a3 * gz[i]) * inv_sqrt_h;
                }
        }
        const f4 sa = (ld_blk(s, n, D::HP, t, nb.lane) + dx) * inv_sqrt2;
        v0 += ld_blk(vec_in, (size_t)n * 3 + 0, D::HP, t, nb.lane);
        v1 += ld_blk(vec_in, (size_t)n * 3 + 1, D::HP, t, nb.lane);
        v2 += ld_blk(vec_in, (size_t)n * 3 + 2, D::HP, t, nb.lane);
        lds_st(in, t, nb.lane, sa);
        lds_st(vx + 0 * HT * 256, t, nb.lane, v0);
        lds_st(vx + 1 * HT * 256, t, nb.lane, v1);
        lds_st(vx + 2 * HT * 256, t, nb.lane, v2);
        if (sa_out != nullptr && nb.valid) {
            st_blk(sa_out, n, D::HP, t, nb.lane, sa);
            st_blk(va_out, (size_t)n * 3 + 0, D::HP, t, nb.lane, v0);
            st_blk(va_out, (size_t)n * 3 + 1, D::HP, t, nb.lane, v1);
            st_blk(va_out, (size_t)n * 3 + 2, D::HP, t, nb.lane, v2);
        }
    }
    TL(2);
    __syncthreads();
    TL(3);

    const float fx = x1[n * 3], fy = x1[n * 3 + 1], fz = x1[n * 3 + 2];
    const float* l3 = wb + lo.l3u;
    f4 v2k[TPW][3], vdk[TPW];
#pragma unroll
    for (int i = 0; i < TPW; ++i) {
        const int t = nb.wave + i * WAVES;
        if (t < HT) {
            TileJob job[2] = {tile_job<HT>(wb + lo.vp, t, vx), tile_job<HT>(wb + lo.vp, HT + t, vx)};
            f4 acc[6];
#pragma unroll
            for (int k = 0; k < 6; ++k) acc[k] = f4zero();
            dense_seq_xyz<HT, 2, HT * 256, (ROWS ? 5 : OARD_NODE_SEQ_G), ROWS>(job, nb.lane, acc);
            const f4 v1[3] = {acc[0], acc[1], acc[2]}, v2[3] = {acc[3], acc[4], acc[5]};
#pragma unroll
            for (int x = 0; x < 3; ++x) v2k[i][x] = v2[x];
            const f4 sc = v1[0] * fx + v1[1] * fy + v1[2] * fz;
            vdk[i] = (v1[0] * v2[0] + v1[1] * v2[1] + v1[2] * v2[2]) * inv_sqrt_h;
            f4 sca;
            const int f0 = 16 * t + 4 * nb.g;
            if (tp.npb <= 4) {
                float* blk = in + (HT + t) * 256;
                lds_st(in, HT + t, nb.lane, sc);
                __builtin_amdgcn_wave_barrier();
                const int f = nb.lane >> 2, c = nb.lane & 3;
                float* cell = blk + (16 * (f >> 2) + c) * 4 + (f & 3);
                const float y = (c < tp.npb && 16 * t + f < D::H) ? lin3u1(l3s, l3, *cell) : 0.f;
                *cell = y;
            } else {
                const bool in_tab = fabsf(sc.x) < L3T_X && fabsf(sc.y) < L3T_X && fabsf(sc.z) < L3T_X && fabsf(sc.w) < L3T_X;
                if (l3t_ok && !__any(!in_tab))
                    sca = (f4){lin3u_table_eval(l3t, sc.x), lin3u_table_eval(l3t, sc.y), lin3u_table_eval(l3t, sc.z), lin3u_table_eval(l3t, sc.w)};
                else
                    sca = lin3u4(l3s, l3, sc);
                sca.x = f0 + 0 < D::H ? sca.x : 0.f; sca.y = f0 + 1 < D::H ? sca.y : 0.f;
                sca.z = f0 + 2 < D::H ? sca.z : 0.f; sca.w = f0 + 3 < D::H ? sca.w : 0.f;
                lds_st(in, HT + t, nb.lane, sca);
            }
        }
    }
    TL(4);
    __syncthreads();
    TL(5);

    {
        TileJob job[TPW];
        f4 acc[TPW];
#pragma unroll
        for (int i = 0; i < TPW; ++i) { job[i] = tile_job<2 * HT>(wb + lo.xv0, min(nb.wave + i * WAVES, HT - 1), in); acc[i] = f4zero(); }
        dense_seq<2 * HT, TPW>(job, nb.lane, acc);
#pragma unroll
        for (int i = 0; i < TPW; ++i)
            if (nb.wave + i * WAVES < HT) lds_st(hx, nb.wave + i * WAVES, nb.lane, silu4(acc[i]));
    }
    TL(6);
    __syncthreads();
    TL(7);

    {
        TileJob job[3 * TPW];
        f4 acc[3 * TPW];
#pragma unroll
        for (int i = 0; i < TPW; ++i) {
            const int t = min(nb.wave + i * WAVES, HT - 1);
#pragma unroll
            for (int k = 0; k < 3; ++k) { job[3 * i + k] = tile_job<HT>(wb + lo.xv2, k * HT + t, hx); acc[3 * i + k] = f4zero(); }
        }
        dense_seq<HT, 3 * TPW>(job, nb.lane, acc);
#pragma unroll
        for (int i = 0; i < TPW; ++i) {
            const int t = nb.wave + i * WAVES;
            if (t < HT && nb.valid) {
                const f4 a = acc[3 * i], b = acc[3 * i + 1], c = acc[3 * i + 2];
                st_blk(s_out, n, D::HP, t, nb.lane, lds_blk(in, t, nb.lane) + (a + b + vdk[i]) * inv_sqrt2);
#pragma unroll
                for (int x = 0; x < 3; ++x)
                    st_blk(vec_out, (size_t)n * 3 + x, D::HP, t, nb.lane,
                           lds_blk(vx + x * HT * 256, t, nb.lane) + c * v2k[i][x]);
            }
        }
    }
    TL(0);
    TL_END();
}

template <class D, int WAVES>
__global__ __launch_bounds__(WAVES * 64) void k_neighbor_v1(TopoDev tp, const float* __restrict__ wb, PackOff po,
                                                            const float* __restrict__ zemb, const float* __restrict__ nbe,
                                                            const float* __restrict__ ew, float* __restrict__ s,
                                                            float* __restrict__ s1) {
    constexpr int HT = D::HT, TPW = (HT + WAVES - 1) / WAVES;
    __shared__ __attribute__((aligned(16))) float sm[2 * HT * 256];
    float* sv = sm;
    float* yv = sm + HT * 256;
    const NodeBlk nb = node_blk(tp.N, tp.npb);
    const int n = nb.n, smp = tp.node_sample[n], s0 = tp.sample_ptr[smp];
    const int ns = nb.valid ? tp.sample_ptr[smp + 1] - s0 : 0;
    const int mx = wave_max(ns);
    const int self = n - s0;
    const float* c0f = wb + po.c0row + 2 * D::H;
    for (int t = nb.wave; t < HT; t += WAVES) {
        f4 acc = f4zero();
// ... 206 lines not shown
```

Baseline: 3709 reaction-steps/s.

## Fuse equivariant message combine into edge kernel with per-target partial sums

Adds a new equivariant edge kernel that computes the messages and combines them with source/target features and geometry. It then segment-reduces the results per target node into seven partial-sum planes, and the node kernel sums these instead of re-gathering q/xq/vec per active edge. The goal is to remove the heavy per-edge gather and combine pass from the node stage. In exchange it adds a new column topology array, a larger vmsg workspace and extra LDS for the radial buffer. The path is enabled by default for inference when the large-batch shape is selected.

```diff
diff --git a/oareactdiff_amd/_capi.py b/oareactdiff_amd/_capi.py
--- a/oareactdiff_amd/_capi.py
+++ b/oareactdiff_amd/_capi.py
@@ -152,7 +152,7 @@
     L.oard_timing_reset.argtypes = []; L.oard_timing_reset.restype = C.c_int
     L.oard_timing_get.argtypes = [C.c_char_p, C.POINTER(C.c_double), C.POINTER(i64)]; L.oard_timing_get.restype = C.c_int
     for env, opt in (("OARD_GCL_VARIANT", b"gcl_variant"), ("OARD_EQUI_VARIANT", b"equi_variant"),
-                     ("OARD_NODE_VARIANT", b"node_variant"), ("OARD_GCL_SKIP", b"gcl_skip"), ("OARD_EQUI_SKIP", b"equi_skip"), ("OARD_EQUI_L0_SKIP", b"equi_l0_skip"), ("OARD_GCL_MSUM", b"gcl_msum"), ("OARD_GCL_PERSIST", b"gcl_persist"), ("OARD_GCL_GRID", b"gcl_grid"), ("OARD_PARTS", b"parts"), ("OARD_SEQUENTIAL", b"sequential"), ("OARD_POISON", b"poison"), ("OARD_AUTO_SMALL", b"auto_small"), ("OARD_AUTO_TINY", b"auto_tiny"), ("OARD_NPB", b"npb"),
+                     ("OARD_NODE_VARIANT", b"node_variant"), ("OARD_GCL_SKIP", b"gcl_skip"), ("OARD_EQUI_SKIP", b"equi_skip"), ("OARD_EQUI_L0_SKIP", b"equi_l0_skip"), ("OARD_GCL_MSUM", b"gcl_msum"), ("OARD_EQUI_TSUM", b"equi_tsum"), ("OARD_GCL_PERSIST", b"gcl_persist"), ("OARD_GCL_GRID", b"gcl_grid"), ("OARD_PARTS", b"parts"), ("OARD_SEQUENTIAL", b"sequential"), ("OARD_POISON", b"poison"), ("OARD_AUTO_SMALL", b"auto_small"), ("OARD_AUTO_TINY", b"auto_tiny"), ("OARD_NPB", b"npb"),
                      ("OARD_WGRAD_WGS", b"wgrad_wgs"), ("OARD_WGRAD_LDS", b"wgrad_lds"), ("OARD_WGRAD_T16", b"wgrad_t16"), ("OARD_WGRAD_QUEUE", b"wgrad_queue"), ("OARD_GATE_FOLD", b"gate_fold"), ("OARD_WGRAD_SHAPES", b"wgrad_shapes"), ("OARD_TRAIN_DUAL", b"train_dual"), ("OARD_SMALL_SPLIT", b"small_split"),
                      ("OARD_SKIP_FAMILIES", b"skip_families")):
         if os.environ.get(env) not in (None, ""):
diff --git a/oareactdiff_amd/csrc/oard_edge_v1.h b/oareactdiff_amd/csrc/oard_edge_v1.h
--- a/oareactdiff_amd/csrc/oard_edge_v1.h
+++ b/oareactdiff_amd/csrc/oard_edge_v1.h
@@ -83,8 +83,9 @@
 OARD_DEV f4 lds_a(const float* sl, int j) { return *reinterpret_cast<const f4*>(sl + j * 256); }
 
 struct NoHook { OARD_DEV void operator()() const {} };
-template <int KB, bool TAIL, class Hook>
-OARD_DEV f4 chain_tile(const float* sl, int j0, const f4 (&in)[KB], f4 init, float tail, Hook hook) {
+struct LdsB { const float* p; OARD_DEV f4 operator[](int b) const { return *reinterpret_cast<const f4*>(p + b * 256); } };
+template <int KB, bool TAIL, class Hook, class B>
+OARD_DEV f4 chain_tile(const float* sl, int j0, const B& in, f4 init, float tail, Hook hook) {
     static_assert(!TAIL || (KB & 1), "compact tail needs an odd number of chunks");
     f4 c0 = init, c1 = f4zero();
     f4 a0 = lds_a(sl, j0), a1 = KB > 1 ? lds_a(sl, j0 + 1) : f4zero();
@@ -107,8 +108,8 @@
 OARD_DEV f4 chain_tile(const float* sl, int j0, const f4 (&in)[KB], f4 init, Hook hook = Hook()) {
     return chain_tile<KB, false, Hook>(sl, j0, in, init, 0.f, hook);
 }
-template <int KB, class Hook = NoHook>
-OARD_DEV f4 chain_tile4(const float* sl, int j0, const f4 (&in)[KB], f4 init, Hook hook = Hook()) {
+template <int KB, class Hook = NoHook, class B = void>
+OARD_DEV f4 chain_tile4(const float* sl, int j0, const B& in, f4 init, Hook hook = Hook()) {
     f4 c0 = init, c1 = f4zero();
     f4 a0 = lds_a(sl, j0), a1 = KB > 1 ? lds_a(sl, j0 + 1) : f4zero();
 #pragma unroll
@@ -616,6 +617,146 @@
 }
 
 template <class D>
+struct EquiTsStream : EquiStream<D> {
+    static constexpr size_t LDS_BYTES = EquiStream<D>::LDS_BYTES + (size_t)8 * D::RB * 1024;
+};
+template <class D, bool L0>
+__global__ __launch_bounds__(8 * 64) void k_equi_edge_ts(TopoDev tp, const float* __restrict__ stream, const float* __restrict__ dp0b,
+                                                         const float* __restrict__ ew, const float* __restrict__ rbuf,
+                                                         const float* __restrict__ geo, const float* __restrict__ xq,
+                                                         const float* __restrict__ vec, float* __restrict__ esum) {
+    extern __shared__ __attribute__((aligned(16))) float smem[];
+    using S = EquiStream<D>;
+    constexpr int WAVES = 8, WB = D::WB, D1T = D::D1T, RB = D::RB, HT = D::HT, G1 = S::G1, G2 = S::G2;
+    constexpr int PS = OARD_TS_PARTS * D::HP;
+    const int lane = threadIdx.x & 63, g = lane >> 4;
+    const int wave = __builtin_amdgcn_readfirstlane(threadIdx.x >> 6);
+
+    const long long c = ((long long)blockIdx.x * WAVES + wave) * 16 + (lane & 15);
+    i4 ci = {0, 0, 0, -1};
+    if (c < tp.TC) ci = *reinterpret_cast<const i4*>(tp.tcol_info + 4 * c);
+    const int key = ci.w;
+    const SegLanes sg = seg_lanes(key);
+    float* ep = esum + (size_t)c * PS + 4 * g;
+    {
+        bool on = false;
+#pragma unroll
+        for (int h = 0; h < 2; ++h) {
+            const long long cc = (long long)blockIdx.x * WAVES * 16 + h * 64 + lane;
+            if (cc < tp.TC) {
+                const int r = tp.tcol_info[4 * cc], k = tp.tcol_info[4 * cc + 3];
+                on = on || (k > 0 && geo[(size_t)r * GEO_STRIDE + 11] > 0.f);
+            }
+        }
+        if (!__any(on)) {
+            if (sg.head) {
+#pragma unroll
+                for (int t = 0; t < HT; ++t)
+#pragma unroll
+                    for (int q = 0; q < OARD_TS_PARTS; ++q)
+                        if (!(L0 && q >= 1 && q <= 3)) st_f4(ep + q * D::HP + 16 * t, f4zero());
+            }
+            return;
+        }
+    }
+    if (key < 0) ci = *reinterpret_cast<const i4*>(tp.tcol_info);
+    const size_t a = (size_t)ci.x;
+    const float* erow = ew + a * D::WP + 4 * g;
+    const float* xs = xq + (size_t)ci.y * (3 * D::HP) + 4 * g;
+    const float* xt = xq + (size_t)ci.z * (3 * D::HP) + 4 * g;
+    const float* vs = vec + (size_t)ci.y * (3 * D::HP) + 4 * g;
+    const float inv_sqrt_h = 1.0f / sqrtf((float)D::H), a2_scale = 0.57735026918962576f * inv_sqrt_h;
+    float gs[3];
+#pragma unroll
+    for (int k = 0; k < 3; ++k) gs[k] = geo[a * GEO_STRIDE + 2 + k] * inv_sqrt_h;
+
+    SlabPrefetch<WAVES, S::SLAB, 0, 3> pf;
+    pf.wave = wave;
+    pf.lane_off = (unsigned)lane * 16u;
+    auto pf_begin = [&](int ph) { pf.begin(stream, smem, ph, ph * G1, G1); };
+    auto pf_begin_t2 = [&](int ph, int slot) { pf.begin(stream, smem, ph, S::C1 + slot * G2, slot < S::NG2 ? G2 : 0); };
+    auto hook = [&]() { pf.tick(); };
+    auto A = [&](int p, int j) -> f4 {
+        return *reinterpret_cast<const f4*>(smem + ((size_t)(p & 1) * S::SLAB + j) * 256 + lane * 4);
+    };
+    auto SL = [&](int p) -> const float* { return smem + (size_t)(p & 1) * S::SLAB * 256 + lane * 4; };
+
+    f4 d1[D1T];
+#pragma unroll
+    for (int t = 0; t < D1T; ++t) d1[t] = ld_vec(dp0b, t, lane);
+    float* rbl = smem + (size_t)2 * S::SLAB * 256 + (size_t)wave * RB * 256 + lane * 4;
+#pragma unroll
+    for (int b = 0; b < RB; ++b) *reinterpret_cast<f4*>(rbl + b * 256) = ld_blk(rbuf, a, D::RP, b, lane);
+    const LdsB rb{rbl};
+    f4 xn = ld_f4(erow);
+    pf_begin(0);
+    pf.flush();
+
+    int p = 0;
+    for (int b = 0; b < WB; ++b, ++p) {
+        phase_barrier();
+        const f4 x = xn;
+        if (b + 1 < WB) pf_begin(p + 1); else pf_begin_t2(p + 1, 0);
+        if (b + 1 < WB) xn = ld_f4(erow + 16 * (b + 1));
+        chain_kouter<D1T>(SL(p), 0, x, d1, hook);
+        pf.flush();
+    }
+#pragma unroll
+    for (int t = 0; t < D1T; ++t) d1[t] = silu4(d1[t]);
+
+    f4 pend[3] = {f4zero(), f4zero(), f4zero()};
+    float* pend_p = ep;
+    auto put = [&](int q, f4 v) __attribute__((always_inline)) {
+        v = seg_sum(v, sg);
+        if (sg.head) st_f4(pend_p + q * D::HP, v);
+    };
+    auto sum_store = [&](auto prev_) __attribute__((always_inline)) {
+        constexpr int prev = decltype(prev_)::value;
+        if constexpr (prev == 0) put(0, pend[0]);
+        if constexpr (prev == 1) { put(1, pend[0]); put(2, pend[1]); put(3, pend[2]); }
+        if constexpr (prev == 2) { put(4, pend[0] * gs[0]); put(5, pend[0] * gs[1]); put(6, pend[0] * gs[2]); }
+    };
+    auto t2_phase = [&](int tt, auto th_, bool pending, auto rows4) __attribute__((always_inline)) {
+        constexpr int th = decltype(th_)::value;
+        phase_barrier();
+        if (pending) sum_store(th_);
+        pf_begin_t2(p + 1, tt + 1 < HT ? 3 * (tt + 1) + th : (th == 2 ? S::NG2 : (L0 ? 2 : th + 1)));
+        const f4 ys = ld_f4(xs + th * D::HP + 16 * tt), yt = ld_f4(xt + th * D::HP + 16 * tt);
+        f4 w[3] = {f4zero(), f4zero(), f4zero()};
+        if (th == 1) {
+#pragma unroll
+            for (int k = 0; k < 3; ++k) w[k] = ld_f4(vs + k * D::HP + 16 * tt);
+        }
+        f4 cd, cr;
+        if (decltype(rows4)::value) {
+            cd = reduce_g(chain_tile4<D1T>(SL(p), 1, d1, A(p, 0), hook));
+            cr = reduce_g(chain_tile4<RB>(SL(p), 1 + D1T, rb, f4zero(), hook));
+            if (g != 0) { cd = f4zero(); cr = f4zero(); }
+        } else {
+            cd = chain_tile<D1T>(SL(p), 1, d1, A(p, 0), hook);
+            cr = chain_tile<RB, false>(SL(p), 1 + D1T, rb, f4zero(), 0.f, hook);
+        }
+        pf.flush();
+        const f4 msg = (ys + yt) * (cd * cr);
+        if (th == 1) {
+            const f4 a2 = msg * a2_scale;
+            pend[0] = w[0] * a2; pend[1] = w[1] * a2; pend[2] = w[2] * a2;
+        } else pend[0] = msg;
+        pend_p = ep + 16 * tt;
+        ++p;
+    };
+    constexpr int HT_FULL = S::ROWS4 ? HT - 1 : HT;
+    auto third = [&](auto th_) __attribute__((always_inline)) {
+        for (int tt = 0; tt < HT_FULL; ++tt) t2_phase(tt, th_, tt > 0, std::false_type{});
+        if (S::ROWS4) t2_phase(HT - 1, th_, HT_FULL > 0, std::true_type{});
+        sum_store(th_);
+    };
+    third(std::integral_constant<int, 0>{});
+    if (!L0) third(std::integral_constant<int, 1>{});
+    third(std::integral_constant<int, 2>{});
+}
+
+template <class D>
 __global__ __launch_bounds__(256) void k_equi_agg_v1(TopoDev tp, const float* __restrict__ wb, LayerOff lo,
                                                      const float* __restrict__ qbuf, const float* __restrict__ xq,
                                                      const float* __restrict__ geo, const float* __restrict__ x1,
diff --git a/oareactdiff_amd/csrc/oard_hip.hip b/oareactdiff_amd/csrc/oard_hip.hip
--- a/oareactdiff_amd/csrc/oard_hip.hip
+++ b/oareactdiff_amd/csrc/oard_hip.hip
@@ -70,6 +70,8 @@
 int g_poison = 0;
 int g_equi_l0_skip = 1;
 int g_gcl_msum = 1;
+int g_equi_tsum = 1;
+int g_equi_tsum_taken = 0;
 int g_gcl_msum_taken = 0;
 int g_equi_l0_taken = 0;
 int g_parts = 0;
@@ -306,7 +308,7 @@
     w.sc0 = take(N * d.HP * 4); w.vdot = take(N * d.HP * 4);
     w.geo = take(A * GEO_STRIDE * 4); w.d64 = take(A * 8); w.rbuf = take(A * d.RP * 4);
     w.ew = take(E * d.WP * 4); w.mbuf = take(std::max(E, (size_t)(td.CI + td.CX) + 1) * d.HP * 4);
-    w.xmsg = take(A * d.HP * 4); w.vmsg = take(A * 3 * d.HP * 4);
+    w.xmsg = take(A * d.HP * 4); w.vmsg = take(std::max(A * 3, ((size_t)td.TC + 1) * OARD_TS_PARTS) * d.HP * 4);
     w.dpos = take(N * 3 * 4); w.hout = take(N * 16 * 4);
     w.al_rows = take(A * 4); w.al_src = take(A * 4); w.al_pre = take(A * 4); w.al_cnt = take((size_t)cdiv((long long)td.A, 256) * 4 + 4); w.al_n = take(4);
     w.d1s = take((size_t)cdiv((long long)td.A, 128) * 8 * d.D1T * 1024);
@@ -510,6 +512,17 @@
     }
 }
 
+template <class D>
+int launch_equi_ts(const TopoDev& tp, const float* stream, const float* dp0b, const float* ew, const float* rbuf, const float* geo, const float* xq,
+                   const float* vec, float* esum, bool layer0, hipStream_t st) {
+    if (tp.TC <= 0) return OARD_OK;
+    if (layer0) LAUNCH_LDS(F_EQUI_EDGE, (k_equi_edge_ts<D, true>), cdiv(tp.TC, 16 * 8), 8 * 64, (EquiTsStream<D>::LDS_BYTES), st,
+                           tp, stream, dp0b, ew, rbuf, geo, xq, vec, esum);
+    else LAUNCH_LDS(F_EQUI_EDGE, (k_equi_edge_ts<D, false>), cdiv(tp.TC, 16 * 8), 8 * 64, (EquiTsStream<D>::LDS_BYTES), st,
+                    tp, stream, dp0b, ew, rbuf, geo, xq, vec, esum);
+    return OARD_OK;
+}
+
 struct TapeOff {
     size_t hin, geo, rbuf, pp0, x1;
     size_t s_in[OARD_MAX_LAYERS + 1], vec_in[OARD_MAX_LAYERS + 1];
@@ -618,6 +631,9 @@
                       (tp.CI == 0 || gcl_v1_throughput(c->precision, gcl_variant, topo->conc, tp.CI)) &&
                       (tp.CX == 0 || gcl_v1_throughput(c->precision, gcl_variant, topo->conc, tp.CX));
     g_gcl_msum_taken = msum;
+    const bool tsum = !train && g_equi_tsum && A > 0 && node_variant == 1 && equi_variant != 0 && tp.npb > 4 && !po.layer[0].xcross &&
+                      equi_v1_shape(c->precision, equi_variant, topo->conc, A, (const float*)(ws + w.d1s)) == 2;
+    g_equi_tsum_taken = tsum;
     for (int l = 0; l < c->num_layers; ++l) {
         const LayerOff lo = po.layer[l];
         const bool nv1 = node_variant == 1 && equi_variant != 0;
@@ -662,7 +678,10 @@
             const bool l0_skip = l == 0 && !train && g_equi_l0_skip && A > 0 && nv1 && !rows &&
                                  equi_v1_shape(c->precision, equi_variant, topo->conc, A, (const float*)(ws + w.d1s)) == 2;
             if (l == 0) g_equi_l0_taken = l0_skip;
-            if (A > 0) {
+            if (tsum) {
+                int rc = launch_equi_ts<D>(tp, wb + lo.equi_stream, wb + lo.dp0b, ew_out, rbuf, geo, xq, vcur, vmsg, l0_skip, st);
+                if (rc != OARD_OK) return rc;
+            } else if (A > 0) {
                 int rc = launch_equi_v1<D>(c->precision, equi_variant, topo->conc, tp, wb, lo, wb + lo.equi_stream, wb + lo.dp0b, ew_out, rbuf, vmsg,
                                            train ? (float*)(tape + to.zd1[l]) : nullptr, train ? (float*)(tape + to.cd[l]) : nullptr, st,
                                            (float*)(ws + w.d1s), al, l0_skip);
@@ -671,7 +690,14 @@
 #define EQUI_NODE_V1(D_, ROWS_, XC_) LAUNCH(F_NODE, (k_equi_node_v1<D_, NW, ROWS_, XC_>), gN16, NW * 64, st, tp, wb, lo, (const float*)vmsg, \
                        (const float*)xq, (const float*)geo, (const float*)x1, (const float*)s_mid_at(l), s_at(l + 1), (const float*)vcur, vnext, \
                        train ? (float*)(tape + to.s_a[l]) : nullptr, train ? (float*)(tape + to.vec_a[l]) : nullptr, al)
-            if (nv1 && rows) {
+            if (tsum) {
+                if (l0_skip) LAUNCH(F_NODE, (k_equi_node_v1<TSum<Layer0<D> >, NW, false, false>), gN16, NW * 64, st, tp, wb, lo, (const float*)vmsg,
+                                    (const float*)xq, (const float*)geo, (const float*)x1, (const float*)s_mid_at(l), s_at(l + 1), (const float*)vcur, vnext,
+                                    (float*)nullptr, (float*)nullptr, ActList{});
+                else LAUNCH(F_NODE, (k_equi_node_v1<TSum<D>, NW, false, false>), gN16, NW * 64, st, tp, wb, lo, (const float*)vmsg,
+                            (const float*)xq, (const float*)geo, (const float*)x1, (const float*)s_mid_at(l), s_at(l + 1), (const float*)vcur, vnext,
+                            (float*)nullptr, (float*)nullptr, ActList{});
+            } else if (nv1 && rows) {
                 if (lo.xcross) EQUI_NODE_V1(D, true, true); else EQUI_NODE_V1(D, true, false);
             } else if (nv1 && l0_skip) {
                 if (lo.xcross) EQUI_NODE_V1(Layer0<D>, false, true); else EQUI_NODE_V1(Layer0<D>, false, false);
@@ -1251,6 +1277,19 @@
         }
     }
 
+    std::vector<int> tcol_info, tnode_cols((size_t)N * 2, 0);
+    for (int b = 0; b < B; ++b) {
+        for (int n = sample_ptr[b]; n < sample_ptr[b + 1]; ++n) {
+            tnode_cols[2 * (size_t)n] = (int)(tcol_info.size() / 4);
+            for (int a = act_ptr[n]; a < act_ptr[n + 1]; ++a) { tcol_info.push_back(a); tcol_info.push_back(act_src[a]); tcol_info.push_back(n); tcol_info.push_back(n + 1); }
+            tnode_cols[2 * (size_t)n + 1] = (int)(tcol_info.size() / 4);
+        }
+        while ((tcol_info.size() / 4) % 16) { tcol_info.push_back((int)A); tcol_info.push_back(0); tcol_info.push_back(0); tcol_info.push_back(-1); }
+    }
+    const long long TC = (long long)(tcol_info.size() / 4);
+    if (TC > 0x7fffffffLL - 256) return OARD_EINVAL;
+    if (tcol_info.empty()) tcol_info.assign({(int)A, 0, 0, -1});
+
     std::vector<UploadItem> items;
     size_t cur = 0;
     auto add = [&](const void* p, size_t bytes) { UploadItem it{p, bytes, cur}; cur = align_up(cur + bytes, 256); items.push_back(it); return it.off; };
@@ -1263,7 +1302,8 @@
                  o_aedge = add(act_edge.data(), act_edge.size() * 4), o_rptr = add(ref_edge_ptr.data(), N * 8),
                  o_erow = add(edge_row.data(), edge_row.size() * 4), o_rsrc = add(row_src.data(), row_src.size() * 4),
                  o_rtgt = add(row_tgt.data(), row_tgt.size() * 4), o_reid = add(row_eid.data(), row_eid.size() * 4),
-                 o_crow = add(col_info.data(), col_info.size() * 4), o_ncol = add(node_cols.data(), node_cols.size() * 4);
+                 o_crow = add(col_info.data(), col_info.size() * 4), o_ncol = add(node_cols.data(), node_cols.size() * 4),
+                 o_tcol = add(tcol_info.data(), tcol_info.size() * 4), o_tncol = add(tnode_cols.data(), tnode_cols.size() * 4);
     size_t cap = 0;
     char* dev = (char*)pool_alloc(cur, &cap);
     if (!dev) return OARD_EHIP;
@@ -1281,6 +1321,7 @@
     d.edge_row = (const int*)(dev + o_erow); d.row_src = (const int*)(dev + o_rsrc); d.row_tgt = (const int*)(dev + o_rtgt);
     d.row_eid = (const int*)(dev + o_reid);
     d.CI = CI; d.CX = CX; d.col_info = (const int*)(dev + o_crow); d.node_cols = (const int*)(dev + o_ncol);
+    d.TC = TC; d.tcol_info = (const int*)(dev + o_tcol); d.tnode_cols = (const int*)(dev + o_tncol);
     return OARD_OK;
 }
 
@@ -2239,6 +2280,8 @@
     if (strcmp(name, "equi_skip") == 0) { g_equi_skip = value; return OARD_OK; }
     if (strcmp(name, "equi_l0_skip") == 0) { g_equi_l0_skip = value; return OARD_OK; }
     if (strcmp(name, "gcl_msum") == 0) { g_gcl_msum = value; return OARD_OK; }
+    if (strcmp(name, "equi_tsum") == 0) { g_equi_tsum = value; return OARD_OK; }
+    if (strcmp(name, "equi_tsum_taken") == 0) return g_equi_tsum_taken ? OARD_OK : OARD_EINVAL;
     if (strcmp(name, "gcl_msum_taken") == 0) return g_gcl_msum_taken ? OARD_OK : OARD_EINVAL;
     if (strcmp(name, "equi_l0_taken") == 0) return g_equi_l0_taken ? OARD_OK : OARD_EINVAL;
     if (strcmp(name, "gcl_persist") == 0) { g_gcl_persist = value; return OARD_OK; }
diff --git a/oareactdiff_amd/csrc/oard_inst.h b/oareactdiff_amd/csrc/oard_inst.h
--- a/oareactdiff_amd/csrc/oard_inst.h
+++ b/oareactdiff_amd/csrc/oard_inst.h
@@ -44,6 +44,7 @@
 
 #if !defined(OARD_INST_DEFINE) || defined(OARD_INST_UNIT_EQUI)
 #define OARD_A_EQUI (TopoDev, const float*, const float*, const float*, const float*, float*, float*, float*, ActList, int)
+#define OARD_A_EQUI_TS (TopoDev, const float*, const float*, const float*, const float*, const float*, const float*, const float*, float*)
 #define OARD_A_EQUI_NODE (TopoDev, const float*, LayerOff, const float*, const float*, const float*, const float*, const float*, float*, const float*, float*, float*, float*, ActList)
 #define X(h, r) \
     OARD_INST((k_equi_edge_v1<Dims<h, r>, 8, false>), OARD_A_EQUI) OARD_INST((k_equi_edge_v1<Dims<h, r>, 8, true>), OARD_A_EQUI) \
@@ -51,6 +52,9 @@
     OARD_INST((k_equi_node_v1<Dims<h, r>, OARD_NW(h), false, false>), OARD_A_EQUI_NODE) OARD_INST((k_equi_node_v1<Dims<h, r>, OARD_NW(h), false, true>), OARD_A_EQUI_NODE) \
     OARD_INST((k_equi_node_v1<Dims<h, r>, OARD_NW(h), true, false>), OARD_A_EQUI_NODE) OARD_INST((k_equi_node_v1<Dims<h, r>, OARD_NW(h), true, true>), OARD_A_EQUI_NODE) \
     OARD_INST((k_equi_node_v1<Layer0<Dims<h, r> >, OARD_NW(h), false, false>), OARD_A_EQUI_NODE) OARD_INST((k_equi_node_v1<Layer0<Dims<h, r> >, OARD_NW(h), false, true>), OARD_A_EQUI_NODE) \
+    OARD_INST((k_equi_edge_ts<Dims<h, r>, false>), OARD_A_EQUI_TS) OARD_INST((k_equi_edge_ts<Dims<h, r>, true>), OARD_A_EQUI_TS) \
+    OARD_INST((k_equi_node_v1<TSum<Dims<h, r> >, OARD_NW(h), false, false>), OARD_A_EQUI_NODE) \
+    OARD_INST((k_equi_node_v1<TSum<Layer0<Dims<h, r> > >, OARD_NW(h), false, false>), OARD_A_EQUI_NODE) \
     OARD_INST((k_gcl_edge_bwd<Dims<h, r>, 8, 2, true>), (TopoDev, const float*, long long, long long, GclBwdArgs)) \
     OARD_INST((k_gcl_edge_bwd<Dims<h, r>, 8, 2, false>), (TopoDev, const float*, long long, long long, GclBwdArgs)) \
     OARD_INST((k_equi_edge_bwd<Dims<h, r>, 8>), (TopoDev, const float*, const float*, const float*, float*, float*))
diff --git a/oareactdiff_amd/csrc/oard_layout.h b/oareactdiff_amd/csrc/oard_layout.h
--- a/oareactdiff_amd/csrc/oard_layout.h
+++ b/oareactdiff_amd/csrc/oard_layout.h
@@ -71,6 +71,9 @@
     long long CI, CX;
     const int *col_info;
     const int *node_cols;
+    long long TC;
+    const int *tcol_info;
+    const int *tnode_cols;
 };
 
 struct ActList {
@@ -114,6 +117,8 @@
     int N_ref = 0;
 };
 
+#define OARD_TS_PARTS 7
+
 struct WsOff {
     size_t pos, pf64, pf32, x1, pp0, labels, hin, zemb, nb, s, s1, ne1, xh, P, Q, xq, vec, vec2, v2buf, sc0, vdot,
         geo, d64, rbuf, ew, mbuf, xmsg, vmsg, dpos, hout, total;
diff --git a/oareactdiff_amd/csrc/oard_node_v1.h b/oareactdiff_amd/csrc/oard_node_v1.h
--- a/oareactdiff_amd/csrc/oard_node_v1.h
+++ b/oareactdiff_amd/csrc/oard_node_v1.h
@@ -472,6 +472,10 @@
 template <class D> struct Layer0 : D {};
 template <class D> struct is_layer0 { static constexpr bool value = false; };
 template <class D> struct is_layer0<Layer0<D> > { static constexpr bool value = true; };
+template <class D> struct TSum : D {};
+template <class D> struct is_tsum { static constexpr bool value = false; };
+template <class D> struct is_tsum<TSum<D> > { static constexpr bool value = true; };
+template <class D> struct is_layer0<TSum<Layer0<D> > > { static constexpr bool value = true; };
 template <class D, int WAVES, bool ROWS = false, bool XC = false>
 __global__ __launch_bounds__(WAVES * 64) void k_equi_node_v1(TopoDev tp, const float* __restrict__ wb, LayerOff lo,
                                                              const float* __restrict__ qbuf, const float* __restrict__ xq,
@@ -480,8 +484,9 @@
                                                              float* __restrict__ vec_out,
                                                              float* __restrict__ sa_out, float* __restrict__ va_out ,
                                                              ActList al ) {
-    constexpr bool L0 = is_layer0<D>::value;
+    constexpr bool L0 = is_layer0<D>::value, TS = is_tsum<D>::value;
     static_assert(!(L0 && ROWS), "the layer-0 form exists for the large-batch gather only");
+    static_assert(!(TS && (ROWS || XC)), "the partial sums exist for the large-batch stage without the coord_cross term");
     constexpr int HT = D::HT;
     constexpr int TPW = (HT + WAVES - 1) / WAVES;
     __shared__ __attribute__((aligned(16))) float sm[6 * HT * 256 + 48 * 12 + L3T_FLOATS];
@@ -555,6 +560,33 @@
             dx = rows_total4(dx, rl, nb.lane); v0 = rows_total4(v0, rl, nb.lane);
             v1 = rows_total4(v1, rl, nb.lane); v2 = rows_total4(v2, rl, nb.lane);
         }
+        if constexpr (TS) {
+            constexpr int PS = OARD_TS_PARTS * D::HP;
+            const int c_lo = tp.tnode_cols[2 * (size_t)n], c_hi = tp.tnode_cols[2 * (size_t)n + 1];
+            const int np = (nb.valid && c_hi > c_lo) ? 1 + ((c_hi - 1) >> 4) - (c_lo >> 4) : 0;
+            const int mxp = wave_max(np);
+            for (int k = 0; k < mxp; k += 2) {
+                f4 r[2][OARD_TS_PARTS];
+#pragma unroll
+                for (int i = 0; i < 2; ++i) {
+#pragma unroll
+                    for (int q = 0; q < OARD_TS_PARTS; ++q) r[i][q] = f4zero();
+                    if (k + i < np) {
+                        const size_t col = (size_t)(k + i == 0 ? c_lo : ((c_lo >> 4) + k + i) << 4);
+#pragma unroll
+                        for (int q = 0; q < OARD_TS_PARTS; ++q)
+                            if (!(L0 && q >= 1 && q <= 3)) r[i][q] = ld_blk(qbuf, col, PS, q * HT + t, nb.lane);
+                    }
+                }
+#pragma unroll
+                for (int i = 0; i < 2; ++i) {
+                    dx += r[i][0];
+                    v0 += L0 ? r[i][4] : r[i][1] + r[i][4];
+                    v1 += L0 ? r[i][5] : r[i][2] + r[i][5];
+                    v2 += L0 ? r[i][6] : r[i][3] + r[i][6];
+                }
+            }
+        }
         int mnext[2], rnext[2];
         auto entry = [&](int kk, int& m, int& r) {
             const int ke = min(a0 + min(kk, max(cnt - 1, 0)), a_hi);
@@ -562,11 +594,12 @@
             r = cnt > 0 ? row_of(ke) : 0;
         };
 #pragma unroll
-        for (int i = 0; i < 2; ++i) entry(i, mnext[i], rnext[i]);
+        for (int i = 0; i < 2; ++i)
+            if (!TS) entry(i, mnext[i], rnext[i]);
         float zero1 = 0.f;
         if (L0) asm volatile("" : "+v"(zero1));
         const f4 zero4 = {zero1, zero1, zero1, zero1};
-        for (int k = 0; !ROWS && k < mx; k += 2) {
+        for (int k = 0; !ROWS && !TS && k < mx; k += 2) {
             f4 q0[2], q1[2], q2[2], y0[2], y1[2], y2[2], w0[2], w1[2], w2[2];
             float gx[2], gy[2], gz[2], cx[2], cy[2], cz[2];
             const int mc[2] = {mnext[0], mnext[1]}, rc[2] = {rnext[0], rnext[1]};
```

After: 3740 reaction-steps/s, median of 6. Within noise of the previous version (+0.8%).
